# oscarknagg/voicemap

Measured on AMD Instinct MI355X. Metric: audio-sec/s embedded, 3s@16kHz siamese batch (training step), higher is better.
Workload: dtype f16; 1 GPU; siamese cfg-A train step (filters 128, embed 64, contrastive loss), 128 pairs/GPU of 3 s @ 16 kHz decimated x4 (L=12000), Adam(clipnorm 1), f16 storage; global_pairs=128, parallelism=dp1

## Files before the change

include/voicemap_hip.h:

```cpp
#ifndef VOICEMAP_HIP_H
#define VOICEMAP_HIP_H

#include <stdint.h>

#ifdef __cplusplus
extern "C" {
#endif

enum { VM_F32 = 0, VM_BF16 = 1, VM_F32S = 2, VM_F16 = 3 };
enum { VM_OK = 0, VM_ERR_ARG = -1, VM_ERR_LAUNCH = -2, VM_ERR_UNSUPPORTED = -3 };
enum { VM_LOSS_CONTRASTIVE = 0, VM_LOSS_BCE = 1 };
enum { VM_HEAD_UNIFORM_EUCLIDEAN = 0, VM_HEAD_WEIGHTED_L1 = 1 };
enum { VM_DIST_EUCLIDEAN = 0, VM_DIST_COSINE = 1, VM_DIST_DOT = 2 };
enum { VM_SCORE_WEIGHTED_L1 = 3, VM_SCORE_NEG_EUCLIDEAN = 4 };

const char* vm_last_error(void);
int vm_abi_version(void);
int vm_check_device(void);

int vm_fill_zero(void* ptr, int64_t bytes, void* stream);
int vm_event_create(void** event_out);
int vm_event_destroy(void* event);
int vm_event_record(void* event, void* stream);
int vm_stream_wait_event(void* stream, void* event);
// ... 19 lines not shown
                                    int noise_is_i16, const int64_t* noise_offsets, int K, const float* snr_lin, const float* gain,
                                    const float* rirs, int n_rirs, int R, const int32_t* rir_id, float* out, void* ws, void* stream);

int64_t vm_conv1_stat_rows(int64_t L);
int vm_conv1_fwd(const float* x, const float* w, const float* bias, int64_t n_windows, int64_t L, int F,
                 int dtype, void* z, float* stat_sum, float* stat_sq, void* stream);
int64_t vm_conv1_wgrad_workspace_bytes(int64_t n_windows, int F);
int vm_conv1_wgrad(const float* x, const void* du, int64_t n_windows, int64_t L, int F, int dtype,
                   float* ws, float* grad_w, void* stream);

int vm_conv1_fused_fwd(const float* x, const float* w, const float* bias, const float* gamma_or_scale, const float* shift,
                       int64_t n_windows, int64_t L, int F, int pool, int inference, int dtype, void* out, float* stat_sum,
                       float* stat_sq, void* stream);
int vm_conv1_fused_fwd_varlen(const float* x, const float* w, const float* bias, const float* scale, const float* shift,
                              const int32_t* lens, int64_t n_windows, int64_t L, int F, int pool, int dtype, void* out, void* stream);
int64_t vm_conv1_fused_bwd_workspace_bytes(int64_t n_windows, int64_t L, int F);
int vm_conv1_fused_bwd(const float* x, const float* w, const float* bias, const void* dp, const float* scale,
                       const float* mean, const float* invstd, const float* drop, const float* c1, const float* c2,
                       int64_t n_windows, int64_t windows_per_tower, int64_t L, int F, int pool, int dtype, void* ws,
                       float* grad_w, float* grad_b, void* stream);

int64_t vm_conv_stat_rows(int64_t L);
int vm_conv_fwd(const void* in, const void* wf, const float* bias, int64_t n_windows, int64_t L, int c_in,
                int c_out, int dtype, void* z, float* stat_sum, float* stat_sq, void* stream);
int64_t vm_conv_flat_stat_rows(int64_t n_windows, int64_t L);
int vm_conv_fwd_flat(const void* in, const void* wf, const float* bias, int64_t n_windows, int64_t L, int c_in, int c_out, int dtype,
                     void* z, float* stat_sum, float* stat_sq, void* stream);
int vm_conv_fwd_e_supported(int64_t n_windows, int64_t L, int c_in, int c_out, int dtype);
int vm_conv_fwd_e(const void* in, const void* wf, const float* bias, const float* gamma, int64_t n_windows, int64_t L,
                  int c_in, int c_out, int dtype, void* z, float* stat_sum, float* stat_sq, void* e, void* stream);
int vm_fold_bn_weights(const float* wt, const float* scale, const float* shift, const float* bias, int towers, int c_in, int c_out,
                       int dtype, void* wf_folded, void* wf_packed, float* hb, float* ctr_out, void* stream);
int vm_conv_fwd_fold_supported(int64_t n_windows, int64_t L, int c_in, int c_out, int dtype, int with_e);
int vm_conv_fwd_fold(const void* in_e, const void* wf_folded, const float* bias, const float* hb, const float* gamma,
                     int64_t n_windows, int64_t windows_per_tower, int64_t L, int c_in, int c_out, int dtype, void* z, float* stat_sum,
                     float* stat_sq, void* e, void* o, const void* wf_packed, const float* e_center, void* stream);
int vm_pack_nt_weights_supported(int n_rows, int a_c, int dtype);
int vm_pack_nt_weights(const void* bt, int towers, int n_rows, int a_c, int dtype, void* packed, void* stream);
int vm_pack_nt_weights_batch(int n, const void* const* bt, const int* towers, const int* n_rows, const int* a_c, int dtype,
                             void* const* packed, void* stream);
int vm_conv_fwd_pool_supported(int64_t n_windows, int64_t L, int c_in, int c_out, int dtype);
int vm_conv_fwd_pool(const void* in, const void* wf, const float* bias, const float* scale, const float* shift,
                     int64_t n_windows, int64_t L, int c_in, int c_out, int dtype, void* act, const void* wf_packed, void* stream);
int vm_conv_fwd_pool_varlen(const void* in, const void* wf, const float* bias, const float* scale, const float* shift,
                            const int32_t* lens, int64_t n_windows, int64_t L, int c_in, int c_out, int dtype, void* act,
                            const void* wf_packed, void* stream);
int vm_conv_dgrad(const void* du, const void* wd, int64_t n_windows, int64_t L, int c_in, int c_out, int dtype,
                  void* dx, void* stream);
int64_t vm_conv_dgrad_bnred_rows(int64_t L);
int vm_conv_dgrad_bnred_supported(int64_t n_windows, int64_t L, int c_in, int c_out, int dtype);
int vm_conv_dgrad_bnred(const void* du, const void* wd, int64_t n_windows, int64_t L, int c_in, int c_out, int dtype,
                        void* dx, const void* red_a, int red_a_padded, float* red_s0, float* red_s1, const void* wd_packed,
                        void* stream);
int vm_conv_wgrad_splits(int64_t n_windows, int64_t L, int c_in, int c_out);
int64_t vm_conv_wgrad_workspace_bytes(int64_t n_windows, int64_t L, int c_in, int c_out);
int vm_conv_wgrad(const void* in, const void* du, int64_t n_windows, int64_t L, int c_in, int c_out, int dtype,
                  void* ws, float* grad_w, void* stream);
int64_t vm_conv_wgrad_fold_workspace_bytes(int64_t n_windows, int64_t windows_per_tower, int64_t L, int c_in, int c_out);
int vm_conv_wgrad_fold(const void* in_e, const void* du, int64_t n_windows, int64_t windows_per_tower, int64_t L, int c_in, int c_out,
                       int dtype, const float* scale, const float* shift, const float* dsum, void* ws, float* grad_w, void* stream);
int vm_conv_wgrad_fold_finish(const void* ws, int64_t n_windows, int64_t windows_per_tower, int64_t L, int c_in, int c_out,
                              const float* scale, const float* shift, const float* dsum, float* grad_w, void* stream);
int vm_prep_conv_weights(const float* w, int c_in, int c_out, int dtype, void* wf, void* wd, void* stream);
int vm_prep_conv_weights_batch(int n_layers, const float* const* w, const int* c_in, const int* c_out, int dtype,
                               void* const* wf, void* const* wd, float* const* wt, void* stream);

// ... 69 lines not shown
int vm_bn_drop_pool_gmax_partials_e(const void* e, const float* scale, const float* shift, const float* drop, int64_t n_windows,
                                    int64_t windows_per_tower, int64_t Lq, int C, int dtype, float* part_v, int32_t* part_i,
                                    void* stream);
int vm_bn_bwd_gmax_finalize_e(const void* e, const float* dg, const int32_t* gidx, const float* scale, const float* shift,
                              const float* mean, const float* invstd, const float* drop, int64_t n_windows, int64_t windows_per_tower,
                              int64_t Lq, int C, int dtype, double count_per_tower, float* c1, float* c2, float* grad_gamma,
                              float* grad_beta, void* stream);
int vm_bn_pool_bwd_apply_pairs_gmax(const void* e, const void* o, const float* dg, const int32_t* gidx, const float* scale,
                                    const float* shift, const float* mean, const float* invstd, const float* drop, const float* c1,
                                    const float* c2, int64_t n_windows, int64_t windows_per_tower, int64_t L, int C, int dtype, void* du,
                                    float* part_du, void* stream);

int vm_global_maxpool_fwd(const void* act, int64_t n_windows, int64_t L, int C, int dtype, float* gmax,
                          int32_t* gidx, void* stream);
int vm_global_maxpool_fwd_varlen(const void* act, const int32_t* lens, int64_t n_windows, int64_t L, int C, int dtype, float* gmax,
                                 int32_t* gidx, void* ws, void* stream);
int vm_global_maxpool_bwd(const float* dg, const int32_t* gidx, int64_t n_windows, int64_t L, int C, int dtype,
                          void* dp, void* stream);
int vm_dense_fwd(const float* in, const float* w, const float* b, int64_t rows, int n_in, int n_out, float* out,
                 void* stream);
int vm_dense_bwd(const float* in, const float* w, const float* dout, int64_t rows, int n_in, int n_out,
                 float* grad_w, float* grad_b, float* din, void* stream);

int vm_siamese_head_loss(const float* emb, const float* head_w, const float* head_b, const float* y, int64_t pairs,
                         int E, int head_kind, int loss_kind, float grad_scale, float* pred, float* loss_acc, float* demb,
                         float* grad_hw, float* grad_hb, float* ws, void* stream);
int vm_siamese_head_reduce(const float* emb, const float* ws, int64_t pairs, int E, int head_kind, float* loss_acc, float* grad_hw,
                           float* grad_hb, void* stream);

int vm_tail_fwd_bwd_supported(int C, int E);
int vm_tail_fwd_bwd(const float* gmax_part_v, const int32_t* gmax_part_i, int seg_rows, float* gmax, int32_t* gidx, const float* dense_w, const float* dense_b,
                    const float* head_w, const float* head_b, const float* y, int64_t pairs, int C, int E, int head_kind,
                    int loss_kind, float grad_scale, float* emb, float* pred, float* demb, float* dgmax, float* ws, void* stream);
int vm_tail_param_grads(const float* gmax, const float* demb, const float* emb, const float* ws, int64_t pairs, int C, int E,
                        int head_kind, float* loss_acc, float* grad_dense_w, float* grad_dense_b, float* grad_hw, float* grad_hb,
                        void* stream);

int vm_softmax_cce(const float* logits, const int32_t* labels, int64_t rows, int n_classes, float grad_scale, float* prob,
                   float* loss_acc, float* dlogits, float* ws, void* stream);

int64_t vm_sqnorm_workspace_bytes(int64_t n);
int vm_grad_sqnorm(const float* g, int64_t n, void* ws, float* sqnorm, void* stream);
int vm_adam_clip_step(float* p, const float* g, float* m, float* v, int64_t n, float lr_t, float beta1, float beta2,
                      float eps, float clipnorm, float grad_prescale, float* sqnorm, const void* sqnorm_parts, int skip_nonfinite,
                      int32_t* skipped, void* stream);

int vm_nshot_distances(const float* query, const float* support, int64_t tasks, int k, int n, int E, int dist_kind,
                       float* pred, int32_t* argmin, void* stream);

int vm_nshot_indexed(const float* emb, int64_t n_rows, const int32_t* query_idx, const int32_t* support_idx, int64_t tasks, int k,
                     int n, int E, int dist_kind, float* pred, int32_t* argmin, void* stream);
int64_t vm_pairdist_workspace_bytes(int64_t M, int64_t N);
int vm_pairdist_argmin(const float* q, const float* ref, int64_t M, int64_t N, int E, int dist_kind, int64_t q_row0, float* dist,
                       float* best_val, int32_t* best_idx, void* ws, void* stream);
int64_t vm_pair_score_hist_workspace_bytes(int64_t N, int E);
int vm_pair_score_hist(const float* emb, const int32_t* label, int64_t N, int E, int score_kind, const float* weights, int64_t row_lo,
                       int64_t row_hi, const int64_t* host_windows, int n_windows, int bins, uint64_t* hist, void* ws, void* stream);
int64_t vm_cohort_stats_workspace_bytes(int64_t M, int64_t C, int E);
int vm_cohort_topk_stats(const float* q, int64_t M, const float* cohort, int64_t C, int E, int score_kind, const float* weights,
                         int64_t self_row0, int64_t K, float* mu, float* sigma, float* rsig, int32_t* count, int32_t* topk_idx, void* ws,
                         void* stream);
int vm_pair_score_hist_norm(const float* emb, const int32_t* label, int64_t N, int E, int score_kind, const float* weights, int64_t row_lo,
                            int64_t row_hi, const int64_t* host_windows, int n_windows, int bins, const float* mu, const float* rsig,
                            uint64_t* hist, void* ws, void* stream);
int64_t vm_speaker_sums_workspace_bytes(int64_t N, int E, int64_t S);
int vm_speaker_sums(const float* emb, const int32_t* label, int64_t N, int E, int64_t S, int kind, double* sums, double* msum, int32_t* count,
// ... 53 lines not shown
```

voicemap_amd/csrc/conv_common.hpp:

```cpp
#pragma once
#include <string.h>

#include <type_traits>

#include "common.hpp"

namespace vm {

constexpr int BM = 128, BN = 128;

template <int KB>
struct Geo {
    static constexpr int PITCH = KB + 16;
    static constexpr int TILE = BM * PITCH;
    static constexpr int CH = KB / 16;
    static constexpr int NCHUNK = BM * CH / 256;
};
constexpr int OUT_PITCH = BN * 4 + 16;

template <typename T> struct Mfma;
template <> struct Mfma<bf16> {
    static constexpr int KSTEP_BYTES = 32;
    using Frag = bf16x8;
    __device__ static inline Frag load(const char* row_ptr, int s, int kh) {
// ... 113 lines not shown
        acc[0][0] = M::run(b0h, a0h, acc[0][0]);
        acc[0][1] = M::run(b1h, a0h, acc[0][1]);
        acc[1][0] = M::run(b0h, a1h, acc[1][0]);
        acc[1][1] = M::run(b1h, a1h, acc[1][1]);
    }
}

__device__ inline void zero_acc(f32x16 (&acc)[2][2]) {
#pragma unroll
    for (int i = 0; i < 2; ++i)
#pragma unroll
        for (int j = 0; j < 2; ++j)
#pragma unroll
            for (int r = 0; r < 16; ++r) acc[i][j][r] = 0.f;
}

__device__ inline void acc_to_lds(char* out_tile, int wm, int wn, int lane, const f32x16 (&acc)[2][2]) {
    const int hi = lane >> 5;
#pragma unroll
    for (int im = 0; im < 2; ++im) {
        const int m = wm * 64 + im * 32 + (lane & 31);
#pragma unroll
        for (int in = 0; in < 2; ++in) {
#pragma unroll
            for (int g = 0; g < 4; ++g) {
                const int n = wn * 64 + in * 32 + 8 * g + 4 * hi;
                f32x4 v = {acc[im][in][4 * g], acc[im][in][4 * g + 1], acc[im][in][4 * g + 2], acc[im][in][4 * g + 3]};
                *reinterpret_cast<f32x4*>(out_tile + m * OUT_PITCH + n * 4) = v;
            }
        }
    }
}

enum { EPI_FWD = 0, EPI_DGRAD = 1, EPI_FWD_POOL = 2, EPI_FWD_FOLD = 3 };

template <typename T>
struct NtArgs {
    const T* a;
    const T* bt;
    const float* bias;
    T* out;
    float* stat_sum;
    float* stat_sq;
    int64_t a_win_stride;
    int a_c;
    int L, N, Ktot;
    int tilesL, tilesN;
    const T* red_a = nullptr;
    int64_t red_a_win_stride = 0;
    int red_a_row0 = 0;
    int split = 0;
    const float* aff_scale = nullptr;
    const float* aff_shift = nullptr;
    T* pool_e = nullptr;
    int pool_e_pad = 0;
    T* pool_o = nullptr;
    const float* fold_hb = nullptr;
    const float* fold_ctr = nullptr;
    int64_t tower_windows = 0, bt_tower_stride = 0;
    int flat_period = 0, flat_valid = 0;
    const T* bt_packed = nullptr;
    const int32_t* valid_len = nullptr;
};

template <int AUX = 0>
__device__ inline void glds16(const char* gsrc, char* lds_base) {
#if defined(__HIP_DEVICE_COMPILE__)
    __builtin_amdgcn_global_load_lds(gsrc, (__attribute__((address_space(3))) void*)lds_base, 16, 0, AUX);
#endif
}

template <int KB>
__device__ inline int swz(int row, int chunk) {
    return KB == 128 ? (chunk ^ ((row >> 1) & 7)) : (chunk ^ ((row >> 2) & 3));
}

template <int N>
__device__ inline void wait_vmcnt() {
    asm volatile("s_waitcnt vmcnt(%0)" ::"n"(N) : "memory");
}

}
```

voicemap_amd/csrc/conv_gemm.hip:

```cpp
#include "conv_common.hpp"

#ifndef VM_ABL
#define VM_ABL 0
#endif

namespace vm {

template <int KB>
constexpr int nt_lds_bytes() {
    return (2 * 2 * Geo<KB>::TILE > BM * OUT_PITCH + 4096) ? 2 * 2 * Geo<KB>::TILE : BM * OUT_PITCH + 4096;
}

template <typename T, int EPI, int KB, bool SPLIT = false>
__global__ __launch_bounds__(256) void conv_nt_kernel(NtArgs<T> p, int64_t n_groups) {
    static_assert(!SPLIT || (sizeof(T) == 4 && KB == 128), "split-bf16 arithmetic: fp32 storage, 128-byte slices");
    using G = Geo<KB>;
    constexpr int VEC = Elem<T>::kVec;
    constexpr int BK = KB / (int)sizeof(T);
    __shared__ __attribute__((aligned(16))) char lds[nt_lds_bytes<KB>()];

    const int tid = threadIdx.x, lane = tid & 63, w = tid >> 6, wm = w >> 1, wn = w & 1;
    const int nk = (p.Ktot + BK - 1) / BK;

    int lds_off[G::NCHUNK], kch[G::NCHUNK], srow[G::NCHUNK];
// ... 416 lines not shown
        for (int g = 0; g < 4; ++g)
#pragma unroll
            for (int i = 0; i < 4; ++i)
#pragma unroll
                for (int e = 0; e < 4; ++e) acc[i][j][4 * g + e] = b4[j][g][e];
}
#if defined(VM_EXPERIMENT_PROFILE_EPI)
extern __device__ unsigned int g_prof[];
__device__ inline void vm_epi_mark(int k) {
    const long long t = __builtin_amdgcn_s_memtime();
    if ((threadIdx.x & 63) == 0 && blockIdx.x < 8192) g_prof[((int64_t)blockIdx.x * 4 + (threadIdx.x >> 6)) * 8 + k] = (unsigned int)t;
}
#if VM_EXPERIMENT_PROFILE_EPI + 0 == 2
#define VM_EPI_MARK(k)
#define VM_RED_MARK(k) vm_epi_mark(k)
#else
#define VM_EPI_MARK(k) vm_epi_mark(k)
#define VM_RED_MARK(k)
#endif
#else
#define VM_EPI_MARK(k)
#define VM_RED_MARK(k)
#endif
struct N2DrainSync {
    __device__ inline void sync() { __syncthreads(); }
    __device__ inline void point() {}
};

template <typename T, int EPI>
__device__ inline void n2_tile_write(const NtArgs<T>& p, char* lds, const f32x16 (&acc)[4][2], int t0, int n0, int trows, int lane, int wm, int wn,
                                     const f32x4 (&negc)[2][4]) {
    using namespace n2;
    const int r = lane & 31, kh = lane >> 5;
    constexpr bool FWD = EPI == EPI_FWD || EPI == EPI_FWD_FOLD;
    const bool red = EPI == EPI_DGRAD && p.red_a != nullptr;
    const int valid = (p.L - t0) < trows ? (p.L - t0) : trows;
    constexpr bool CAN_CENTRE = EPI == EPI_FWD_FOLD && std::is_same<T, f16>::value;
    const bool ctrd = CAN_CENTRE && p.fold_ctr != nullptr;
    auto body = [&](auto ctrd_c) {
        constexpr bool CTRD = decltype(ctrd_c)::value;
        uint32_t nc16[2][4][2];
        if constexpr (CTRD) {
            typedef _Float16 h2 __attribute__((ext_vector_type(2)));
#pragma unroll
            for (int j = 0; j < 2; ++j)
#pragma unroll
                for (int g = 0; g < 4; ++g) {
                    nc16[j][g][0] = __builtin_bit_cast(uint32_t, h2{(_Float16)negc[j][g][0], (_Float16)negc[j][g][1]});
                    nc16[j][g][1] = __builtin_bit_cast(uint32_t, h2{(_Float16)negc[j][g][2], (_Float16)negc[j][g][3]});
                }
        }
#pragma unroll
        for (int i = 0; i < 4; ++i) {
#pragma unroll
            for (int j = 0; j < 2; ++j) {
                const int mb = wm * 128 + i * 32;
                const int m = mb + r;
                const bool partial = mb + 32 > valid;
                const bool zero = (FWD || red) && partial && m >= valid;
#pragma unroll
                for (int g = 0; g < 4; ++g) {
                    const int nl = wn * 64 + j * 32 + 8 * g + 4 * kh;
                    T o[4];
#pragma unroll
                    for (int e = 0; e < 4; ++e) o[e] = Elem<T>::from_f(acc[i][j][4 * g + e]);
                    u32x2 pk = *reinterpret_cast<const u32x2*>(o);
                    if constexpr (CTRD) {
                        uint32_t lo = pk[0], hi = pk[1];
                        asm("v_pk_max_f16 %0, %1, %2" : "=v"(lo) : "v"(lo), "v"(nc16[j][g][0]));
                        asm("v_pk_max_f16 %0, %1, %2" : "=v"(hi) : "v"(hi), "v"(nc16[j][g][1]));
                        pk[0] = lo;
                        pk[1] = hi;
                    } else if constexpr (EPI != EPI_DGRAD) {
                        uint32_t lo = pk[0], hi = pk[1];
                        asm("v_pk_max_i16 %0, %1, 0" : "=v"(lo) : "v"(lo));
                        asm("v_pk_max_i16 %0, %1, 0" : "=v"(hi) : "v"(hi));
                        pk[0] = lo;
                        pk[1] = hi;
                    }
                    pk[0] = zero ? 0u : pk[0];
                    pk[1] = zero ? 0u : pk[1];
                    *reinterpret_cast<u32x2*>(lds + m * TP + nl * 2) = pk;
                }
            }
        }
    };
    if constexpr (CAN_CENTRE) {
        if (ctrd) body(std::true_type{});
        else body(std::false_type{});
    } else {
        body(std::false_type{});
    }
}

template <typename T, int EPI, typename BarT>
__device__ inline void n2_tile_drain(const NtArgs<T>& p, char* lds, int64_t n, int tl, int t0, int n0, int trows, int tid, int lane, int w,
                                     BarT& bar) {
    using namespace n2;
    using V8 = typename Mfma<T>::Frag;
    const int kh = lane >> 5;
    constexpr bool FWD = EPI == EPI_FWD || EPI == EPI_FWD_FOLD;
    const bool stats = FWD && p.stat_sum != nullptr && !(VM_ABL & 8);
    const bool red = EPI == EPI_DGRAD && p.red_a != nullptr;
    const int valid = (p.L - t0) < trows ? (p.L - t0) : trows;
    const int c8 = tid & 15, rg = tid >> 4;
    if (EPI == EPI_FWD_POOL) {
        float sc[8], sh[8];
        {
            const f32x4 s0 = *reinterpret_cast<const f32x4*>(p.aff_scale + n0 + c8 * 8), s1 = *reinterpret_cast<const f32x4*>(p.aff_scale + n0 + c8 * 8 + 4);
            const f32x4 h0 = *reinterpret_cast<const f32x4*>(p.aff_shift + n0 + c8 * 8), h1 = *reinterpret_cast<const f32x4*>(p.aff_shift + n0 + c8 * 8 + 4);
#pragma unroll
            for (int e = 0; e < 4; ++e) {
                sc[e] = s0[e];
                sc[4 + e] = s1[e];
                sh[e] = h0[e];
                sh[4 + e] = h1[e];
            }
        }
        const int vq = valid >> 1;
        int dq = vq;
        if (p.valid_len != nullptr) {
            const int d = (p.valid_len[n] >> 1) - (t0 >> 1);
            dq = d < vq ? d : vq;
        }
        T* pbase = p.out + (n * (int64_t)(p.L / 2 + 2) + 1 + (t0 >> 1)) * (int64_t)p.N + n0 + c8 * 8;
        V8 r0[8], r1[8];
#pragma unroll
        for (int jj = 0; jj < 8; ++jj) {
            const int q = rg + 16 * jj;
            r0[jj] = *reinterpret_cast<const V8*>(lds + (2 * q) * TP + c8 * 16);
            r1[jj] = *reinterpret_cast<const V8*>(lds + (2 * q + 1) * TP + c8 * 16);
        }
#pragma unroll
        for (int jj = 0; jj < 8; ++jj) {
// ... 18 lines not shown
    auto half = [&](int h, auto interior_c) {
        constexpr bool INTERIOR = decltype(interior_c)::value;
        u32x4 v[8];
#pragma unroll
        for (int jj = 0; jj < 8; ++jj) v[jj] = *reinterpret_cast<const u32x4*>(lds + (h * 128 + rg + 16 * jj) * TP + c8 * 16);
#pragma unroll
        for (int jj = 0; jj < 8; ++jj) {
            const int row = h * 128 + rg + 16 * jj;
            const bool ok = INTERIOR ? (h == 0 || jj < 7 || row < trows) : row < valid;
            if (ok && !((VM_ABL & 4) && row > 0)) *reinterpret_cast<u32x4*>(obase + (int64_t)row * p.N) = v[jj];
        }
    };
    if (FWD && p.pool_o != nullptr) {
    } else if (interior) {
        half(0, std::true_type{});
        bar.point();
        half(1, std::true_type{});
        bar.point();
    } else {
        half(0, std::false_type{});
        bar.point();
        half(1, std::false_type{});
        bar.point();
    }
    if (FWD && p.pool_e != nullptr) {
        u32x4 neg;
        {
            const f32x4 g0 = *reinterpret_cast<const f32x4*>(p.aff_scale + n0 + c8 * 8), g1 = *reinterpret_cast<const f32x4*>(p.aff_scale + n0 + c8 * 8 + 4);
            neg[0] = (g0[0] < 0.f ? 0xFFFFu : 0u) | (g0[1] < 0.f ? 0xFFFF0000u : 0u);
            neg[1] = (g0[2] < 0.f ? 0xFFFFu : 0u) | (g0[3] < 0.f ? 0xFFFF0000u : 0u);
            neg[2] = (g1[0] < 0.f ? 0xFFFFu : 0u) | (g1[1] < 0.f ? 0xFFFF0000u : 0u);
            neg[3] = (g1[2] < 0.f ? 0xFFFFu : 0u) | (g1[3] < 0.f ? 0xFFFF0000u : 0u);
        }
        constexpr bool CAN_CENTRE = EPI == EPI_FWD_FOLD && std::is_same<T, f16>::value;
        const bool ctrd = CAN_CENTRE && p.fold_ctr != nullptr;
        u32x4 c16 = {0u, 0u, 0u, 0u};
        if (CAN_CENTRE && ctrd) {
            const f32x4 q0 = *reinterpret_cast<const f32x4*>(p.fold_ctr + n0 + c8 * 8), q1 = *reinterpret_cast<const f32x4*>(p.fold_ctr + n0 + c8 * 8 + 4);
            typedef _Float16 h2 __attribute__((ext_vector_type(2)));
            c16[0] = __builtin_bit_cast(uint32_t, h2{(_Float16)q0[0], (_Float16)q0[1]});
            c16[1] = __builtin_bit_cast(uint32_t, h2{(_Float16)q0[2], (_Float16)q0[3]});
            c16[2] = __builtin_bit_cast(uint32_t, h2{(_Float16)q1[0], (_Float16)q1[1]});
            c16[3] = __builtin_bit_cast(uint32_t, h2{(_Float16)q1[2], (_Float16)q1[3]});
        }
        const int vq = valid >> 1;
        T* ebase = p.pool_e + (n * (int64_t)(p.L / 2 + 2 * p.pool_e_pad) + p.pool_e_pad + (t0 >> 1)) * (int64_t)p.N + n0 + c8 * 8;
        T* obase2 = p.pool_o + (n * (int64_t)(p.L / 2) + (t0 >> 1)) * (int64_t)p.N + n0 + c8 * 8;
        u32x4 r0[8], r1[8];
#pragma unroll
        for (int jj = 0; jj < 8; ++jj) {
            const int q = rg + 16 * jj;
            r0[jj] = *reinterpret_cast<const u32x4*>(lds + (2 * q) * TP + c8 * 16);
            r1[jj] = *reinterpret_cast<const u32x4*>(lds + (2 * q + 1) * TP + c8 * 16);
        }
        auto pairs = [&](auto ctrd_c, auto other_c) {
            constexpr bool CTRD = decltype(ctrd_c)::value, OTHER = decltype(other_c)::value;
#pragma unroll
            for (int jj = 0; jj < 8; ++jj) {
                const int q = rg + 16 * jj;
                u32x4 o, oth;
#pragma unroll
                for (int d = 0; d < 4; ++d) {
                    uint32_t a = r0[jj][d], b = r1[jj][d];
                    const uint32_t m = neg[d];
                    if constexpr (CTRD) {
                        uint32_t mx, mn;
                        asm("v_pk_max_f16 %0, %1, %2" : "=v"(mx) : "v"(a), "v"(b));
// ... 7 lines not shown
                    if constexpr (!CTRD || OTHER) {
                        const uint32_t fl = m & 0x7FFF7FFFu;
                        const uint32_t af = a ^ fl, bf = b ^ fl;
                        uint32_t mx, mn;
                        asm("v_pk_max_i16 %0, %1, %2" : "=v"(mx) : "v"(af), "v"(bf));
                        if constexpr (!CTRD) o[d] = mx ^ fl;
                        if constexpr (OTHER) {
                            uint32_t df;
                            asm("v_pk_min_i16 %0, %1, %2" : "=v"(mn) : "v"(af), "v"(bf));
                            asm("v_pk_sub_i16 %0, %1, %2" : "=v"(df) : "v"(af), "v"(bf));
                            oth[d] = (mn ^ fl) | (df & 0x80008000u);
                        }
                    }
                }
                if (q < vq) {
                    *reinterpret_cast<u32x4*>(ebase + (int64_t)q * p.N) = o;
                    if constexpr (OTHER) *reinterpret_cast<u32x4*>(obase2 + (int64_t)q * p.N) = oth;
                }
                bar.point();
            }
        };
        const bool other = p.pool_o != nullptr;
        if constexpr (CAN_CENTRE) {
            if (ctrd && other) pairs(std::true_type{}, std::true_type{});
            else if (ctrd) pairs(std::true_type{}, std::false_type{});
            else if (other) pairs(std::false_type{}, std::true_type{});
            else pairs(std::false_type{}, std::false_type{});
        } else {
            if (other) pairs(std::false_type{}, std::true_type{});
            else pairs(std::false_type{}, std::false_type{});
        }
    }
    VM_EPI_MARK(5);
    if (stats) {
#if defined(__HIP_DEVICE_COMPILE__)
        const uint32_t lds0 = (uint32_t)(uintptr_t)(__attribute__((address_space(3))) const char*)lds;
#else
        const uint32_t lds0 = 0;
#endif
        const int li = lane & 15, lg = (lane >> 4) & 1;
        const uint32_t xoff = lds0 + (4 * (li >> 2) + 2 * kh) * TP + (32 * w + 16 * lg + 4 * (li & 3)) * 2;
        const u32x2 ones = ones4<T>();
        const int srows = (p.L + 127) / 128;
        const int cn = lane & 31;
#pragma unroll
        for (int h = 0; h < 2; ++h) {
            f32x4 d1a = {0.f, 0.f, 0.f, 0.f}, d1b = d1a, d2a = d1a, d2b = d1a;
            u32x2 lo[8], hi[8];
#pragma unroll
            for (int rs = 0; rs < 8; ++rs) {
                const uint32_t a = xoff + (h * 128 + rs * 16) * TP;
                asm volatile("ds_read_b64_tr_b16 %0, %1" : "=v"(lo[rs]) : "v"(a));
                asm volatile("ds_read_b64_tr_b16 %0, %1 offset:272" : "=v"(hi[rs]) : "v"(a));
            }
#pragma unroll
            for (int rs = 0; rs < 8; ++rs) {
                if (rs == 0) {
                    asm volatile("s_waitcnt lgkmcnt(14)" : "+v"(lo[0]), "+v"(hi[0]));
                } else if (rs == 1) {
                    asm volatile("s_waitcnt lgkmcnt(12)" : "+v"(lo[1]), "+v"(hi[1]));
                } else if (rs == 2) {
                    asm volatile("s_waitcnt lgkmcnt(10)" : "+v"(lo[2]), "+v"(hi[2]));
                } else if (rs == 3) {
                    asm volatile("s_waitcnt lgkmcnt(8)" : "+v"(lo[3]), "+v"(hi[3]));
                } else if (rs == 4) {
                    asm volatile("s_waitcnt lgkmcnt(6)" : "+v"(lo[4]), "+v"(hi[4]));
                } else if (rs == 5) {
                    asm volatile("s_waitcnt lgkmcnt(4)" : "+v"(lo[5]), "+v"(hi[5]));
                } else if (rs == 6) {
                    asm volatile("s_waitcnt lgkmcnt(2)" : "+v"(lo[6]), "+v"(hi[6]));
                } else {
                    asm volatile("s_waitcnt lgkmcnt(0)" : "+v"(lo[7]), "+v"(hi[7]));
                }
                d2a = Mfma4<T>::run(lo[rs], lo[rs], d2a);
                d2b = Mfma4<T>::run(hi[rs], hi[rs], d2b);
                d1a = Mfma4<T>::run(ones, lo[rs], d1a);
                d1b = Mfma4<T>::run(ones, hi[rs], d1b);
                __builtin_amdgcn_sched_barrier(0);
            }
            float ds = d1a[0] + d1b[0], dq = 0.f;
#pragma unroll
            for (int e = 0; e < 4; ++e) dq = e == (lane & 3) ? d2a[e] + d2b[e] : dq;
            ds += __shfl_xor(ds, 32, 64);
            dq += __shfl_xor(dq, 32, 64);
            if (2 * tl + h < srows && kh == 0) {
                const int64_t srow = n * srows + 2 * tl + h;
                p.stat_sum[srow * p.N + n0 + 32 * w + cn] = ds;
                p.stat_sq[srow * p.N + n0 + 32 * w + cn] = dq;
            }
            bar.point();
        }
    }
    VM_EPI_MARK(6);
    VM_RED_MARK(1);
    if (red) {
#if defined(__HIP_DEVICE_COMPILE__)
        const uint32_t lds0 = (uint32_t)(uintptr_t)(__attribute__((address_space(3))) const char*)lds;
#else
        const uint32_t lds0 = 0;
#endif
        const int li = lane & 15, lg = (lane >> 4) & 1;
        const uint32_t xoff = lds0 + (4 * (li >> 2) + 2 * kh) * TP + (32 * w + 16 * lg + 4 * (li & 3)) * 2;
        const u32x2 ones = ones4<T>();
        u32x2 dlo[16], dhi[16];
        f32x4 d1[2][2], d2[2][2];
#pragma unroll
        for (int h = 0; h < 2; ++h)
#pragma unroll
            for (int u = 0; u < 2; ++u) d1[h][u] = d2[h][u] = f32x4{0.f, 0.f, 0.f, 0.f};
#pragma unroll
        for (int q = 0; q < 16; ++q) {
            const uint32_t a = xoff + (q * 16) * TP;
            asm volatile("ds_read_b64_tr_b16 %0, %1" : "=v"(dlo[q]) : "v"(a));
            asm volatile("ds_read_b64_tr_b16 %0, %1 offset:272" : "=v"(dhi[q]) : "v"(a));
            if (q == 7) asm volatile("s_waitcnt lgkmcnt(0)" : "+v"(dlo[0]), "+v"(dhi[0]), "+v"(dlo[1]), "+v"(dhi[1]), "+v"(dlo[2]), "+v"(dhi[2]),
                                     "+v"(dlo[3]), "+v"(dhi[3]), "+v"(dlo[4]), "+v"(dhi[4]), "+v"(dlo[5]), "+v"(dhi[5]), "+v"(dlo[6]), "+v"(dhi[6]),
                                     "+v"(dlo[7]), "+v"(dhi[7]));
        }
        asm volatile("s_waitcnt lgkmcnt(0)" : "+v"(dlo[8]), "+v"(dhi[8]), "+v"(dlo[9]), "+v"(dhi[9]), "+v"(dlo[10]), "+v"(dhi[10]), "+v"(dlo[11]),
                     "+v"(dhi[11]), "+v"(dlo[12]), "+v"(dhi[12]), "+v"(dlo[13]), "+v"(dhi[13]), "+v"(dlo[14]), "+v"(dhi[14]), "+v"(dlo[15]),
                     "+v"(dhi[15]));
        VM_RED_MARK(2);
        bar.sync();
// ... 33 lines not shown
            }
            asm volatile("s_waitcnt lgkmcnt(0)" : "+v"(alo[0]), "+v"(ahi[0]), "+v"(alo[1]), "+v"(ahi[1]), "+v"(alo[2]), "+v"(ahi[2]), "+v"(alo[3]),
                         "+v"(ahi[3]), "+v"(alo[4]), "+v"(ahi[4]), "+v"(alo[5]), "+v"(ahi[5]), "+v"(alo[6]), "+v"(ahi[6]), "+v"(alo[7]), "+v"(ahi[7]));
#pragma unroll
            for (int rs = 0; rs < 8; ++rs) {
                const int q = h * 8 + rs;
                d2[h][0] = Mfma4<T>::run(dlo[q], alo[rs], d2[h][0]);
                d2[h][1] = Mfma4<T>::run(dhi[q], ahi[rs], d2[h][1]);
            }
        }
        const int cn = lane & 31;
        const int rows2 = 2 * p.tilesL;
#pragma unroll
        for (int h = 0; h < 2; ++h) {
            float ds = d1[h][0][0] + d1[h][1][0], dq = 0.f;
#pragma unroll
            for (int e = 0; e < 4; ++e) dq = e == (lane & 3) ? d2[h][0][e] + d2[h][1][e] : dq;
            ds += __shfl_xor(ds, 32, 64);
            dq += __shfl_xor(dq, 32, 64);
            const int64_t srow = n * rows2 + 2 * tl + h;
            if (kh == 0) {
                p.stat_sum[srow * p.N + n0 + 32 * w + cn] = ds;
                p.stat_sq[srow * p.N + n0 + 32 * w + cn] = dq;
            }
        }
    }
}


template <typename T, int EPI>
__device__ inline void n2_epilogue(const NtArgs<T>& p, char* lds, const f32x16 (&acc)[4][2], int64_t n, int tl, int t0, int n0, int trows,
                                   int tid, int lane, int w, int wm, int wn) {
    f32x4 negc[2][4];
    if constexpr (EPI == EPI_FWD_FOLD && std::is_same<T, f16>::value) {
        if (p.fold_ctr != nullptr) {
#pragma unroll
            for (int j = 0; j < 2; ++j)
#pragma unroll
                for (int g = 0; g < 4; ++g) {
                    const f32x4 c = *reinterpret_cast<const f32x4*>(p.fold_ctr + n0 + (wn * 64 + j * 32) + 8 * g + 4 * (lane >> 5));
                    negc[j][g] = f32x4{-c[0], -c[1], -c[2], -c[3]};
                }
        }
    }
    VM_EPI_MARK(1);
    __syncthreads();
    VM_EPI_MARK(2);
    n2_tile_write<T, EPI>(p, lds, acc, t0, n0, trows, lane, wm, wn, negc);
    VM_EPI_MARK(3);
    __syncthreads();
    VM_EPI_MARK(4);
    N2DrainSync bar;
    n2_tile_drain<T, EPI>(p, lds, n, tl, t0, n0, trows, tid, lane, w, bar);
}

namespace n2r {
constexpr int TROWS = 254;
constexpr int A_BLK = 256 * 64, B_STG = 128 * 64;
constexpr int B0 = 3 * A_BLK;
constexpr int OPER = 3 * A_BLK + 3 * B_STG;
static_assert(OPER <= n2::LDS_BYTES, "operand rings fit under the epilogue tile");
}

__device__ inline void wait_vm_0246(int n) {
    if (n >= 6) {
        asm volatile("s_waitcnt vmcnt(6)" ::: "memory");
    } else if (n == 4) {
// ... 31 lines not shown
    }
}

template <typename T, int EPI>
__global__ __launch_bounds__(256, 2) void conv_nt2r_kernel(NtArgs<T> p, int64_t n_groups) {
    VM_PROF(const long long pt_start = __builtin_amdgcn_s_memtime(); long long pt_first = 0, pt_bar = 0;)
    using namespace n2;
    using namespace n2r;
    using V8 = typename Mfma<T>::Frag;
    __shared__ __attribute__((aligned(1024))) char lds[LDS_BYTES];
    const int tid = threadIdx.x, lane = tid & 63;
    const int w = __builtin_amdgcn_readfirstlane(tid >> 6), wm = w >> 1, wn = w & 1;
    const int chunks = p.a_c / 32, nk = chunks * 3;
    const int row_bytes = p.a_c * 2;

    unsigned group;
    int tn;
    {
        const unsigned v = blockIdx.x, tiles_n = (unsigned)p.tilesN;
        if ((n_groups & 7) == 0) {
            const unsigned j = v >> 3, q = j / tiles_n;
            tn = (int)(j - q * tiles_n);
            group = q * 8 + (v & 7);
        } else {
            group = v / tiles_n;
            tn = (int)(v - group * tiles_n);
        }
    }
    const unsigned nw = group / (unsigned)p.tilesL;
    const int tl = (int)(group - nw * (unsigned)p.tilesL);
    const int64_t n = nw;
    const int t0 = tl * TROWS, n0 = tn * TN;
    if (n2_pool_dead_tile<T, EPI>(p, n, t0, n0, tid)) return;
    if constexpr (EPI == EPI_FWD_FOLD) {
        const unsigned tw = nw / (unsigned)p.tower_windows;
        p.bt += tw * p.bt_tower_stride;
        p.fold_hb += tw * 4 * p.N;
        if (p.fold_ctr != nullptr) p.fold_ctr += tw * p.N;
    }
    f32x4 bias4[2][4];
    if constexpr (EPI == EPI_FWD_FOLD) p.bias = p.fold_hb + 3 * p.N;
    n2_load_bias<T, EPI>(p, bias4, n0 + wn * 64 + 4 * (lane >> 5));

    const int lrow = lane >> 2, lchunk = lane & 3;
    const char* a_src[4];
    const char* b_src[2];
#pragma unroll
    for (int i = 0; i < 4; ++i) {
        const int row = (w + 4 * i) * 16 + lrow;
        int pr = t0 + row;
        pr = pr < p.L + 2 ? pr : p.L + 1;
        a_src[i] = reinterpret_cast<const char*>(p.a + n * p.a_win_stride + (int64_t)pr * p.a_c) + ((lchunk ^ ((row >> 2) & 3)) << 4);
    }
#pragma unroll
    for (int i = 0; i < 2; ++i) {
        const int row = (w + 4 * i) * 16 + lrow;
        b_src[i] = reinterpret_cast<const char*>(p.bt + (int64_t)(n0 + row) * p.Ktot) + ((lchunk ^ ((row >> 2) & 3)) << 4);
    }
    auto issue_a = [&](int blk, int chunk, int i0) {
        char* base = lds + blk * A_BLK;
#pragma unroll
        for (int i = 0; i < 2; ++i) glds16(a_src[i0 + i] + chunk * KB, base + __builtin_amdgcn_readfirstlane((w + 4 * (i0 + i)) * 1024));
    };
    auto issue_b = [&](int stg, int ko) {
        char* base = lds + B0 + stg * B_STG;
#pragma unroll
        for (int i = 0; i < 2; ++i) glds16(b_src[i] + ko, base + __builtin_amdgcn_readfirstlane((w + 4 * i) * 1024));
    };

    const int r = lane & 31, kh = lane >> 5;
    int a_addr[3][2], b_addr[2];
#pragma unroll
    for (int tap = 0; tap < 3; ++tap) {
        const int row = wm * 128 + r + tap;
// ... 82 lines not shown
            VM_MM(a0[1], b0[1], 1, 1);
            __builtin_amdgcn_sched_barrier(0);
            asm volatile("s_waitcnt lgkmcnt(7)" : "+v"(a0[2]));
            VM_MM(a0[2], b0[0], 2, 0);
            VM_MM(a0[2], b0[1], 2, 1);
            __builtin_amdgcn_sched_barrier(0);
            asm volatile("s_waitcnt lgkmcnt(6)" : "+v"(a0[3]));
            VM_MM(a0[3], b0[0], 3, 0);
            VM_MM(a0[3], b0[1], 3, 1);
            __builtin_amdgcn_sched_barrier(0);
            asm volatile("s_waitcnt lgkmcnt(3)" : "+v"(b1[0]), "+v"(b1[1]), "+v"(a1[0]));
            VM_MM(a1[0], b1[0], 0, 0);
            VM_MM(a1[0], b1[1], 0, 1);
            __builtin_amdgcn_sched_barrier(0);
            asm volatile("s_waitcnt lgkmcnt(2)" : "+v"(a1[1]));
            VM_MM(a1[1], b1[0], 1, 0);
            VM_MM(a1[1], b1[1], 1, 1);
            __builtin_amdgcn_sched_barrier(0);
            asm volatile("s_waitcnt lgkmcnt(1)" : "+v"(a1[2]));
            VM_MM(a1[2], b1[0], 2, 0);
            VM_MM(a1[2], b1[1], 2, 1);
            __builtin_amdgcn_sched_barrier(0);
            asm volatile("s_waitcnt lgkmcnt(0)" : "+v"(a1[3]));
            VM_MM(a1[3], b1[0], 3, 0);
            VM_MM(a1[3], b1[1], 3, 1);
            __builtin_amdgcn_sched_barrier(0);
#undef VM_MM
            __builtin_amdgcn_sched_barrier(0);
            VM_PROF(if (kt == 0) pt_first = __builtin_amdgcn_s_memtime();)
        }
        a_blk = a_blk == 2 ? 0 : a_blk + 1;
    }
    VM_PROF(const long long pt_loop = __builtin_amdgcn_s_memtime();)
    if constexpr (EPI == EPI_FWD_FOLD) {
        const int c0 = n0 + wn * 64 + 4 * (lane >> 5), rl = p.L - 1 - t0;
        if (t0 == 0) n2_fold_edge<T>(p, acc, 0, 0, wm, lane & 31, c0);
        if (rl >= 0 && rl < TROWS) n2_fold_edge<T>(p, acc, rl, 1, wm, lane & 31, c0);
    }
    n2_epilogue<T, EPI>(p, lds, acc, n, tl, t0, n0, TROWS, tid, lane, w, wm, wn);
#if defined(VM_EXPERIMENT_PROFILE)
    {
        asm volatile("s_waitcnt vmcnt(0)" ::: "memory");
        const long long pt_end = __builtin_amdgcn_s_memtime();
        if (lane == 0 && blockIdx.x < 8192) {
            unsigned int* q = g_prof + ((int64_t)blockIdx.x * 4 + w) * 8;
            q[0] = (unsigned int)(pt_end - pt_start);
            q[1] = (unsigned int)(pt_first - pt_start);
            q[2] = (unsigned int)(pt_loop - pt_first);
            q[3] = (unsigned int)(pt_end - pt_loop);
            q[4] = (unsigned int)(pt_s2 - pt_start);
            q[5] = (unsigned int)(pt_s3 - pt_s2);
            q[6] = (unsigned int)(pt_bar - pt_s3);
            q[7] = (unsigned int)(pt_first - pt_bar);
        }
    }
#endif
}


#ifndef VM_NT3_ABL
#define VM_NT3_ABL 0
#endif
namespace n3 {
constexpr int NBLK = 4;
constexpr int A_BLK = 256 * 64;
static_assert(NBLK * A_BLK <= n2::LDS_BYTES, "the input ring fits under the epilogue tile");
constexpr int KT_BYTES = 4096;
// ... 47 lines not shown
              n3_nwait(5, 8, false) == 8, "conv_nt3_kernel wait schedule");
static_assert(n3_nwait(0, 4, true) == 8 && n3_nwait(1, 4, true) == 12 && n3_nwait(2, 4, true) == 12 && n3_nwait(3, 4, true) == 8 &&
              n3_nwait(4, 8, true) == 6 && n3_nwait(11, 4, true) == 0, "conv_nt3_kernel wait schedule (lean prologue)");

template <typename T, int EPI, int CHUNKS, bool LEAN>
__global__ __launch_bounds__(256, 2) void conv_nt3_kernel(NtArgs<T> p, int64_t n_groups) {
    VM_PROF(const long long pt_start = __builtin_amdgcn_s_memtime(); long long pt_first = 0, pt_bar = 0;)
    using namespace n2;
    using V8 = typename Mfma<T>::Frag;
    constexpr int A_BLK = n3::A_BLK, NK = 3 * CHUNKS;
    __shared__ __attribute__((aligned(1024))) char lds[LDS_BYTES];
    const int tid = threadIdx.x, lane = tid & 63;
    const int w = __builtin_amdgcn_readfirstlane(tid >> 6), wm = w >> 1, wn = w & 1;

    unsigned group;
    int tn;
    {
        const unsigned v = blockIdx.x, tiles_n = (unsigned)p.tilesN;
        if ((n_groups & 7) == 0) {
            const unsigned j = v >> 3, q = j / tiles_n;
            tn = (int)(j - q * tiles_n);
            group = q * 8 + (v & 7);
        } else {
            group = v / tiles_n;
            tn = (int)(v - group * tiles_n);
        }
    }
    const unsigned nw = group / (unsigned)p.tilesL;
    const int tl = (int)(group - nw * (unsigned)p.tilesL);
    const int64_t n = nw;
    const int t0 = tl * n2r::TROWS, n0 = tn * TN;
    if (n2_pool_dead_tile<T, EPI>(p, n, t0, n0, tid)) return;
    unsigned tw = 0;
    if constexpr (EPI == EPI_FWD_FOLD) {
        tw = nw / (unsigned)p.tower_windows;
        p.fold_hb += tw * 4 * p.N;
        if (p.fold_ctr != nullptr) p.fold_ctr += tw * p.N;
    }
    if constexpr (EPI == EPI_FWD_FOLD) p.bias = p.fold_hb + 3 * p.N;
    f32x4 bias_lo[2][4], bias_hi[2][4];
    if constexpr (EPI != EPI_DGRAD) {
        const float* bp = p.bias + n0 + wn * 64;
#pragma unroll
        for (int j = 0; j < 2; ++j)
#pragma unroll
            for (int g = 0; g < 4; ++g) {
                bias_lo[j][g] = *reinterpret_cast<const f32x4*>(bp + 32 * j + 8 * g);
                bias_hi[j][g] = *reinterpret_cast<const f32x4*>(bp + 32 * j + 8 * g + 4);
            }
    }

    const int lrow = lane >> 2, lchunk = lane & 3;
    const char* a_src[4];
#pragma unroll
    for (int i = 0; i < 4; ++i) {
        const int row = (w + 4 * i) * 16 + lrow;
        int pr = t0 + row;
        pr = pr < p.L + 2 ? pr : p.L + 1;
        a_src[i] = reinterpret_cast<const char*>(p.a + n * p.a_win_stride + (int64_t)pr * p.a_c) + ((lchunk ^ ((row >> 2) & 3)) << 4);
    }
    auto issue_a = [&](int blk, int chunk, int i0) {
        char* base = lds + blk * A_BLK;
#pragma unroll
        for (int i = 0; i < 2; ++i) glds16(a_src[i0 + i] + chunk * KB, base + __builtin_amdgcn_readfirstlane((w + 4 * (i0 + i)) * 1024));
    };
    auto issue_a1 = [&](int blk, int chunk, int i) {
        glds16(a_src[i] + chunk * KB, lds + blk * A_BLK + __builtin_amdgcn_readfirstlane((w + 4 * i) * 1024));
    };
    uint64_t bbase;
    {
        const uint64_t q = (uint64_t)(uintptr_t)p.bt_packed +
                           ((uint64_t)tw * (unsigned)(p.N >> 6) + (unsigned)((n0 >> 6) + wn)) * (uint64_t)(NK * n3::KT_BYTES);
// ... 97 lines not shown
        constexpr int kt_ = (KT), c_ = kt_ / 3, tap_ = kt_ - 3 * c_, cur_ = kt_ % 3, nxt_ = (kt_ + 2) % 3, ablk_ = c_ % 4;             \
        constexpr int nc_ = (kt_ + 1) / 3, ntap_ = (kt_ + 1) - 3 * nc_;                             \
        n3_wait_b<n3_nwait(kt_, CHUNKS, LEAN)>(bs[cur_]);                                                                             \
        if constexpr (kt_ == 0) {                                                                                                     \
            __builtin_amdgcn_s_barrier();                                                                                             \
            VM_PROF(pt_bar = __builtin_amdgcn_s_memtime();)                                                                           \
            const uint32_t a00_ = lds0 + a_addr[0][0];                                                                                \
            VM_FRAG_READ(f0[0], a00_, 0) VM_FRAG_READ(f0[1], a00_, 1) VM_FRAG_READ(f0[2], a00_, 2) VM_FRAG_READ(f0[3], a00_, 3)         \
        }                                                                                                                             \
        const uint32_t aa1_ = lds0 + ablk_ * A_BLK + a_addr[tap_][1];                                                                  \
        const uint32_t an0_ = lds0 + (nc_ % 4) * A_BLK + a_addr[ntap_][0];                                                             \
        const uint64_t sb_ = bbase + (uint64_t)((kt_ + 2) * n3::KT_BYTES);                                                            \
        __builtin_amdgcn_sched_barrier(0);                                                                                            \
        VM_P_STEP0(0) VM_P_STEP0(1) VM_P_STEP0(2) VM_P_STEP0(3)                                                                       \
        if constexpr (tap_ == 2 && kt_ + 1 < NK) {                                                                                    \
            asm volatile("s_waitcnt lgkmcnt(0)" : "+v"(f1[0]), "+v"(f1[1]), "+v"(f1[2]), "+v"(f1[3]));                                 \
            __builtin_amdgcn_s_barrier();                                                                                             \
            __builtin_amdgcn_sched_barrier(0);                                                                                        \
        }                                                                                                                             \
        VM_P_STEP1(0) VM_P_STEP1(1) VM_P_STEP1(2) VM_P_STEP1(3)                                                                       \
        VM_PROF(if (kt_ == 0) pt_first = __builtin_amdgcn_s_memtime();)                                                               \
    }
#define VM_CHUNK(C) VM_KTILE_P(3 * (C)) VM_KTILE_P(3 * (C) + 1) VM_KTILE_P(3 * (C) + 2)
    VM_CHUNK(0) VM_CHUNK(1) VM_CHUNK(2) VM_CHUNK(3) VM_CHUNK(4) VM_CHUNK(5) VM_CHUNK(6) VM_CHUNK(7)
    VM_CHUNK(8) VM_CHUNK(9) VM_CHUNK(10) VM_CHUNK(11) VM_CHUNK(12) VM_CHUNK(13) VM_CHUNK(14) VM_CHUNK(15)
    static_assert(CHUNKS <= 16, "conv_nt3_kernel: at most 16 channel chunks are written out");
#undef VM_CHUNK
#undef VM_KTILE_P
#undef VM_P_STEP0
#undef VM_P_STEP1
#undef VM_FRAG_READ
#undef VM_MM
#undef VM_LOAD_SET
    if constexpr (EPI == EPI_FWD_FOLD) {
        const int c0 = n0 + wn * 64 + 4 * (lane >> 5), rl = p.L - 1 - t0;
        if (t0 == 0) n2_fold_edge<T>(p, acc, 0, 0, wm, lane & 31, c0);
        if (rl >= 0 && rl < n2r::TROWS) n2_fold_edge<T>(p, acc, rl, 1, wm, lane & 31, c0);
    }
    VM_PROF(const long long pt_loop = __builtin_amdgcn_s_memtime();)
#if VM_NT3_ABL & 8
    if (acc[0][0][0] == 123.456f && acc[3][1][15] == 1.5f) n2_epilogue<T, EPI>(p, lds, acc, n, tl, t0, n0, n2r::TROWS, tid, lane, w, wm, wn);
#else
    n2_epilogue<T, EPI>(p, lds, acc, n, tl, t0, n0, n2r::TROWS, tid, lane, w, wm, wn);
#endif
#if defined(VM_EXPERIMENT_PROFILE)
    {
        asm volatile("s_waitcnt vmcnt(0)" ::: "memory");
        const long long pt_end = __builtin_amdgcn_s_memtime();
#if defined(VM_EXPERIMENT_PROFILE_HW)
        if (lane == 0 && blockIdx.x < 8192) {
            unsigned int* q = g_prof + ((int64_t)blockIdx.x * 4 + w) * 8;
            q[0] = (unsigned int)pt_start;
            q[1] = (unsigned int)pt_end;
            q[2] = __builtin_amdgcn_s_getreg((31 << 11) | 4);
            q[3] = __builtin_amdgcn_s_getreg((31 << 11) | 20);
            q[4] = (unsigned int)pt_bar;
            q[5] = (unsigned int)pt_loop;
            q[6] = (unsigned int)(pt_start >> 32);
            q[7] = (unsigned int)pt_s3;
        }
        (void)pt_first; (void)pt_s2;
#elif defined(VM_EXPERIMENT_PROFILE_EPI)
        if (lane == 0 && blockIdx.x < 8192) {
            unsigned int* q = g_prof + ((int64_t)blockIdx.x * 4 + w) * 8;
            q[0] = (unsigned int)pt_start;
            q[7] = (unsigned int)pt_end;
        }
// ... 87 lines not shown
}

static bool nt3_chunks(int a_c) { return a_c == 128 || a_c == 256 || a_c == 384 || a_c == 512; }

template <typename T, int EPI>
static void launch_n2r(const NtArgs<T>& a, int64_t n_windows, hipStream_t stream) {
    if constexpr (sizeof(T) == 2) {
        NtArgs<T> b = a;
        b.tilesN = a.N / n2::TN;
        b.tilesL = (a.L + n2r::TROWS - 1) / n2r::TROWS;
        const int64_t n_groups = n_windows * b.tilesL;
        if constexpr (EPI != EPI_FWD) {
            if (b.bt_packed != nullptr && (g_nt3 & (EPI == EPI_DGRAD ? 2 : 1)) && nt3_chunks(a.a_c)) {
                const dim3 grid((unsigned)(n_groups * b.tilesN));
#define VM_NT3(CH, PIPE) hipLaunchKernelGGL((conv_nt3_kernel<T, EPI, CH, PIPE>), grid, dim3(256), 0, stream, b, n_groups)
                const bool pipe = (g_nt3_lean & (EPI == EPI_DGRAD ? 2 : 1)) != 0;
                switch (a.a_c / 32) {
                    case 4: if (pipe) VM_NT3(4, true); else VM_NT3(4, false); break;
                    case 8: if (pipe) VM_NT3(8, true); else VM_NT3(8, false); break;
                    case 12: if (pipe) VM_NT3(12, true); else VM_NT3(12, false); break;
                    default: if (pipe) VM_NT3(16, true); else VM_NT3(16, false); break;
                }
#undef VM_NT3
                return;
            }
        }
        hipLaunchKernelGGL((conv_nt2r_kernel<T, EPI>), dim3((unsigned)(n_groups * b.tilesN)), dim3(256), 0, stream, b, n_groups);
    }
}

template <typename T, int EPI>
static void launch_nt(const NtArgs<T>& a, int64_t n_windows, hipStream_t stream) {
    if constexpr (sizeof(T) == 2) {
        if (!a.flat_period && (g_nt_n2 & (EPI == EPI_DGRAD ? 2 : 1)) && a.Ktot == 3 * a.a_c && n2r_shape(n_windows, a.L, a.a_c, a.N, EPI == EPI_FWD || EPI == EPI_FWD_FOLD)) {
            launch_n2r<T, EPI>(a, n_windows, stream);
            return;
        }
    }
    const int64_t n_groups = n_windows * a.tilesL;
    const int64_t grid = n_groups < g_nt_blocks ? n_groups : g_nt_blocks;
    const int64_t kbytes = (int64_t)a.Ktot * (int64_t)sizeof(T);
    if constexpr (sizeof(T) == 4) {
        if (a.split) {
            hipLaunchKernelGGL((conv_nt_kernel<T, EPI, 128, true>), dim3((unsigned)grid), dim3(256), 0, stream, a, n_groups);
            return;
        }
    }
    if (g_nt_glds && kbytes % 128 == 0) {
        hipLaunchKernelGGL((conv_nt_glds_kernel<T, EPI, 128>), dim3((unsigned)grid), dim3(256), 0, stream, a, n_groups);
    } else if (g_nt_glds && kbytes % 64 == 0) {
        hipLaunchKernelGGL((conv_nt_glds_kernel<T, EPI, 64>), dim3((unsigned)grid), dim3(256), 0, stream, a, n_groups);
    } else {
        hipLaunchKernelGGL((conv_nt_kernel<T, EPI, 128>), dim3((unsigned)grid), dim3(256), 0, stream, a, n_groups);
    }
}

template <typename T>
static NtArgs<T> fwd_args(const void* in, const void* wf, const float* bias, void* out, float* stat_sum, float* stat_sq, int64_t L,
                          int c_in, int c_out, int dtype) {
    NtArgs<T> a;
    a.a = (const T*)in;
    a.bt = (const T*)wf;
    a.bias = bias;
    a.out = (T*)out;
    a.stat_sum = stat_sum;
    a.stat_sq = stat_sq;
    a.a_win_stride = (L + 2) * (int64_t)c_in;
// ... 102 lines not shown
extern "C" int vm_conv_fwd_fold(const void* in_e, const void* wf_folded, const float* bias, const float* hb, const float* gamma,
                                int64_t n_windows, int64_t windows_per_tower, int64_t L, int c_in, int c_out, int dtype, void* z,
                                float* stat_sum, float* stat_sq, void* e, void* o, const void* wf_packed, const float* e_center,
                                void* stream) {
    VM_REQUIRE(in_e && wf_folded && bias && hb && stat_sum && stat_sq, "vm_conv_fwd_fold: null pointer");
    VM_REQUIRE(e_center == nullptr || (dtype == VM_F16 && e != nullptr && o != nullptr),
               "vm_conv_fwd_fold: a centred tile (e_center) needs VM_F16 storage and the (e, o) pair output");
    VM_REQUIRE(e == nullptr || gamma != nullptr, "vm_conv_fwd_fold: the pool extreme needs gamma (its sign picks max / min)");
    VM_REQUIRE(o == nullptr || e != nullptr, "vm_conv_fwd_fold: o (the other element of each pair) goes with e");
    VM_REQUIRE(z != nullptr || o != nullptr, "vm_conv_fwd_fold: z may only be NULL when (e, o) carry the output");
    VM_REQUIRE(n_windows > 0 && L > 0 && windows_per_tower > 0 && n_windows % windows_per_tower == 0,
               "vm_conv_fwd_fold: n_windows must be a positive multiple of windows_per_tower");
    VM_REQUIRE((L + 2) * (int64_t)c_in < (1LL << 31) && 3LL * c_in * c_out < (1LL << 31), "vm_conv_fwd_fold: window too large");
    if (!vm_conv_fwd_fold_supported(n_windows, L, c_in, c_out, dtype, e != nullptr)) {
        set_error("vm_conv_fwd_fold: shape/dtype/tuning not served by the 256 x 128 input-resident kernel (ask vm_conv_fwd_fold_supported)");
        return VM_ERR_UNSUPPORTED;
    }
    VM_DISPATCH_16(dtype, {
        NtArgs<T> a = fwd_args<T>(in_e, wf_folded, bias, z, stat_sum, stat_sq, L, c_in, c_out, dtype);
        a.fold_hb = hb;
        a.tower_windows = windows_per_tower;
        a.bt_tower_stride = 3LL * c_in * c_out;
        a.aff_scale = gamma;
        a.pool_e = (T*)e;
        a.pool_o = (T*)o;
        a.pool_e_pad = 1;
        a.bt_packed = (const T*)wf_packed;
        a.fold_ctr = e_center;
        launch_n2r<T, EPI_FWD_FOLD>(a, n_windows, (hipStream_t)stream);
    });
    return check_launch("vm_conv_fwd_fold");
}

extern "C" int vm_conv_fwd_pool_supported(int64_t n_windows, int64_t L, int c_in, int c_out, int dtype) {
    return (is16(dtype) && (g_nt_n2 & 1) && L >= 2 && !(L & 1) && n2r_shape(n_windows, L, c_in, c_out, false)) ? 1 : 0;
}

extern "C" int vm_conv_fwd_pool(const void* in, const void* wf, const float* bias, const float* scale, const float* shift,
                                int64_t n_windows, int64_t L, int c_in, int c_out, int dtype, void* act, const void* wf_packed,
                                void* stream) {
    VM_REQUIRE(in && wf && bias && scale && shift && act, "vm_conv_fwd_pool: null pointer");
    VM_REQUIRE(n_windows > 0 && L > 0, "vm_conv_fwd_pool: bad sizes");
    VM_REQUIRE((L + 2) * (int64_t)c_in < (1LL << 31) && 3LL * c_in * c_out < (1LL << 31), "vm_conv_fwd_pool: window too large");
    if (!vm_conv_fwd_pool_supported(n_windows, L, c_in, c_out, dtype)) {
        set_error("vm_conv_fwd_pool: shape/dtype/tuning not served by the 256 x 128 input-resident kernel (ask vm_conv_fwd_pool_supported)");
        return VM_ERR_UNSUPPORTED;
    }
    VM_DISPATCH_16(dtype, {
        NtArgs<T> a = fwd_args<T>(in, wf, bias, act, nullptr, nullptr, L, c_in, c_out, dtype);
        a.aff_scale = scale;
        a.aff_shift = shift;
        a.bt_packed = (const T*)wf_packed;
        launch_n2r<T, EPI_FWD_POOL>(a, n_windows, (hipStream_t)stream);
    });
    return check_launch("vm_conv_fwd_pool");
}

extern "C" int vm_conv_fwd_pool_varlen(const void* in, const void* wf, const float* bias, const float* scale, const float* shift,
                                       const int32_t* lens, int64_t n_windows, int64_t L, int c_in, int c_out, int dtype, void* act,
                                       const void* wf_packed, void* stream) {
    VM_REQUIRE(in && wf && bias && scale && shift && lens && act, "vm_conv_fwd_pool_varlen: null pointer");
    VM_REQUIRE(n_windows > 0 && L > 0, "vm_conv_fwd_pool_varlen: bad sizes");
    VM_REQUIRE((L + 2) * (int64_t)c_in < (1LL << 31) && 3LL * c_in * c_out < (1LL << 31), "vm_conv_fwd_pool_varlen: window too large");
    if (!vm_conv_fwd_pool_supported(n_windows, L, c_in, c_out, dtype)) {
        set_error("vm_conv_fwd_pool_varlen: shape/dtype/tuning not served by the 256 x 128 input-resident kernel (ask vm_conv_fwd_pool_supported)");
        return VM_ERR_UNSUPPORTED;
// ... 161 lines not shown
```

voicemap_amd/csrc/program_run.hip:

```cpp
#include <cstdint>
#include <cstring>

extern "C" {
int vm_abi_version(void);
int vm_adam_clip_step(const void*, const void*, const void*, const void*, int64_t, float, float, float, float, float, float, const void*, const void*, int, const void*, const void*);
int vm_bn_bwd_finalize(const void*, const void*, int64_t, int64_t, int, double, const void*, const void*, const void*, const void*, const void*, const void*);
int vm_bn_bwd_from_sums(const void*, const void*, int64_t, const void*, const void*, const void*, const void*, const void*, const void*, const void*, int64_t, int64_t, int64_t, int, int, int, int, const void*, const void*, const void*);
int vm_bn_bwd_from_sums_finalize(const void*, const void*, int64_t, const void*, const void*, const void*, const void*, const void*, const void*, const void*, int64_t, int64_t, int64_t, int, int, int, int, double, const void*, const void*, const void*, const void*, const void*, const void*);
int vm_bn_bwd_gmax_finalize(const void*, const void*, const void*, const void*, const void*, const void*, const void*, const void*, int64_t, int64_t, int64_t, int, int, int, double, const void*, const void*, const void*, const void*, const void*);
int vm_bn_bwd_gmax_finalize_e(const void*, const void*, const void*, const void*, const void*, const void*, const void*, const void*, int64_t, int64_t, int64_t, int, int, double, const void*, const void*, const void*, const void*, const void*);
int vm_bn_drop_pool_fwd(const void*, const void*, const void*, const void*, int64_t, int64_t, int64_t, int, int, int, const void*, const void*);
int vm_bn_drop_pool_fwd_varlen(const void*, const void*, const void*, const void*, int64_t, int64_t, int, int, int, const void*, const void*);
int vm_bn_drop_pool_gmax_fwd(const void*, const void*, const void*, const void*, int64_t, int64_t, int64_t, int, int, int, const void*, const void*, const void*, const void*);
int vm_bn_drop_pool_gmax_fwd_varlen(const void*, const void*, const void*, const void*, int64_t, int64_t, int, int, int, const void*, const void*, const void*, const void*);
int vm_bn_drop_pool_gmax_partials(const void*, const void*, const void*, const void*, int64_t, int64_t, int64_t, int, int, int, const void*, const void*, const void*);
int vm_bn_drop_pool_gmax_partials_e(const void*, const void*, const void*, const void*, int64_t, int64_t, int64_t, int, int, const void*, const void*, const void*);
int vm_bn_finalize(const void*, const void*, int64_t, int, int, double, const void*, const void*, float, float, int, const void*, const void*, const void*, const void*, const void*, const void*, const void*, const void*, float, const void*, const void*, const void*, const void*, const void*);
int vm_bn_infer_affine(const void*, const void*, const void*, const void*, float, int, const void*, const void*, const void*);
int vm_bn_part_rows(void);
int vm_bn_part_rows_used(int64_t, int, int, int);
int vm_bn_pool2d_stack_fwd(const void*, const void*, const void*, const void*, int64_t, int, int64_t, int64_t, int, int, int, const void*, const void*, const void*);
int vm_bn_pool2d_stack_fwd_split(const void*, const void*, const void*, const void*, const void*, int64_t, int, int64_t, int64_t, int, int, int, const void*, const void*, const void*);
int vm_bn_pool_bwd_apply(const void*, const void*, const void*, const void*, const void*, const void*, const void*, const void*, const void*, int64_t, int64_t, int64_t, int, int, int, const void*, const void*, const void*);
int vm_bn_pool_bwd_apply_gmax(const void*, const void*, const void*, const void*, const void*, const void*, const void*, const void*, const void*, const void*, int64_t, int64_t, int64_t, int, int, int, const void*, const void*, const void*);
int vm_bn_pool_bwd_apply_pairs(const void*, const void*, const void*, const void*, const void*, const void*, const void*, const void*, const void*, const void*, int64_t, int64_t, int64_t, int, int, const void*, const void*, const void*, const void*);
int vm_bn_pool_bwd_apply_pairs_gmax(const void*, const void*, const void*, const void*, const void*, const void*, const void*, const void*, const void*, const void*, const void*, int64_t, int64_t, int64_t, int, int, const void*, const void*, const void*);
int vm_bn_pool_bwd_reduce(const void*, const void*, const void*, const void*, const void*, const void*, const void*, int64_t, int64_t, int64_t, int, int, int, const void*, const void*, const void*);
int vm_bn_pool_bwd_reduce_gmax(const void*, const void*, const void*, const void*, const void*, const void*, const void*, const void*, int64_t, int64_t, int64_t, int, int, int, const void*, const void*, const void*);
int vm_bn_pool_bwd_reduce_pooled(const void*, const void*, const void*, const void*, const void*, const void*, const void*, const void*, int64_t, int64_t, int64_t, int, int, int, const void*, const void*, const void*);
int vm_check_device(void);
int vm_clip_max_bwd(const void*, const void*, int64_t, int, int, const void*, const void*);
int vm_clip_max_fwd(const void*, int64_t, int, int, int, const void*, const void*, const void*);
int vm_cohort_topk_stats(const void*, int64_t, const void*, int64_t, int, int, const void*, int64_t, int64_t, const void*, const void*, const void*, const void*, const void*, const void*, const void*);
int vm_colsum(const void*, int64_t, int, const void*, const void*, const void*);
int vm_colsum_strided(const void*, int64_t, int, int, const void*, const void*, const void*);
int vm_conv1_fused_bwd(const void*, const void*, const void*, const void*, const void*, const void*, const void*, const void*, const void*, const void*, int64_t, int64_t, int64_t, int, int, int, const void*, const void*, const void*, const void*);
int vm_conv1_fused_fwd(const void*, const void*, const void*, const void*, const void*, int64_t, int64_t, int, int, int, int, const void*, const void*, const void*, const void*);
int vm_conv1_fused_fwd_varlen(const void*, const void*, const void*, const void*, const void*, const void*, int64_t, int64_t, int, int, int, const void*, const void*);
int vm_conv1_fwd(const void*, const void*, const void*, int64_t, int64_t, int, int, const void*, const void*, const void*, const void*);
int vm_conv1_wgrad(const void*, const void*, int64_t, int64_t, int, int, const void*, const void*, const void*);
int vm_conv2d_first_bn_pool_stack(const void*, const void*, const void*, const void*, const void*, const void*, const void*, int64_t, int, int64_t, int64_t, int, int, int, int, const void*, const void*, const void*);
int vm_conv2d_first_fwd(const void*, const void*, const void*, int64_t, int, int64_t, int, int, int, const void*, const void*, const void*, const void*);
int vm_conv2d_first_fwd_split(const void*, const void*, const void*, const void*, int64_t, int, int64_t, int, int, int, const void*, const void*, const void*, const void*, const void*);
int vm_conv2d_first_supported(int, int);
int vm_conv2d_first_wgrad(const void*, const void*, int64_t, int, int64_t, int, int, int, const void*, const void*, const void*);
int vm_conv_dgrad(const void*, const void*, int64_t, int64_t, int, int, int, const void*, const void*);
int vm_conv_dgrad_bnred(const void*, const void*, int64_t, int64_t, int, int, int, const void*, const void*, int, const void*, const void*, const void*, const void*);
int vm_conv_dgrad_bnred_supported(int64_t, int64_t, int, int, int);
int vm_conv_fwd(const void*, const void*, const void*, int64_t, int64_t, int, int, int, const void*, const void*, const void*, const void*);
int vm_conv_fwd_e(const void*, const void*, const void*, const void*, int64_t, int64_t, int, int, int, const void*, const void*, const void*, const void*, const void*);
int vm_conv_fwd_e_supported(int64_t, int64_t, int, int, int);
int vm_conv_fwd_flat(const void*, const void*, const void*, int64_t, int64_t, int, int, int, const void*, const void*, const void*, const void*);
int vm_conv_fwd_fold(const void*, const void*, const void*, const void*, const void*, int64_t, int64_t, int64_t, int, int, int, const void*, const void*, const void*, const void*, const void*, const void*, const void*, const void*);
int vm_conv_fwd_fold_supported(int64_t, int64_t, int, int, int, int);
int vm_conv_fwd_pool(const void*, const void*, const void*, const void*, const void*, int64_t, int64_t, int, int, int, const void*, const void*, const void*);
int vm_conv_fwd_pool_supported(int64_t, int64_t, int, int, int);
int vm_conv_fwd_pool_varlen(const void*, const void*, const void*, const void*, const void*, const void*, int64_t, int64_t, int, int, int, const void*, const void*, const void*);
int vm_conv_wgrad(const void*, const void*, int64_t, int64_t, int, int, int, const void*, const void*, const void*);
int vm_conv_wgrad_fold(const void*, const void*, int64_t, int64_t, int64_t, int, int, int, const void*, const void*, const void*, const void*, const void*, const void*);
int vm_conv_wgrad_fold_finish(const void*, int64_t, int64_t, int64_t, int, int, const void*, const void*, const void*, const void*, const void*);
int vm_conv_wgrad_splits(int64_t, int64_t, int, int);
int vm_crop_augment_decimate_whiten(const void*, int, const void*, int64_t, int64_t, int, int, float, int64_t, const void*, int, const void*, int, const void*, const void*, const void*, int, int, const void*, const void*, const void*, const void*);
int vm_crop_decimate_whiten(const void*, int, const void*, int64_t, int64_t, int, int, float, int64_t, const void*, const void*, const void*);
int vm_crop_decimate_whiten_varlen(const void*, int, const void*, const void*, int64_t, int64_t, int, int, float, const void*, const void*, const void*);
int vm_decimate_whiten(const void*, int, int64_t, int64_t, int, int, float, int64_t, const void*, const void*, const void*);
int vm_dense_bwd(const void*, const void*, const void*, int64_t, int, int, const void*, const void*, const void*, const void*);
int vm_dense_fwd(const void*, const void*, const void*, int64_t, int, int, const void*, const void*);
int vm_du_tower_sums(const void*, const void*, int64_t, int64_t, int64_t, int, int, const void*, const void*, const void*, const void*);
int vm_event_destroy(const void*);
int vm_event_record(const void*, const void*);
int vm_fill_zero(const void*, int64_t, const void*);
int vm_fold_bn_weights(const void*, const void*, const void*, const void*, int, int, int, int, const void*, const void*, const void*, const void*, const void*);
int vm_fold_pool_windows_bwd(const void*, const void*, int64_t, int, int64_t, int, int, int, int, const void*, const void*, const void*, const void*);
int vm_fold_windows(const void*, int64_t, int, int64_t, int, int, int, int, const void*, const void*);
int vm_global_maxpool_bwd(const void*, const void*, int64_t, int64_t, int, int, const void*, const void*);
int vm_global_maxpool_fwd(const void*, int64_t, int64_t, int, int, const void*, const void*, const void*);
int vm_global_maxpool_fwd_varlen(const void*, const void*, int64_t, int64_t, int, int, const void*, const void*, const void*, const void*);
int vm_grad_sqnorm(const void*, int64_t, const void*, const void*, const void*);
int vm_mfma_rate_probe(int, int, const void*, const void*);
int vm_mine_pairs(const void*, const void*, int64_t, int, int, int64_t, int64_t, int, int, const void*, const void*, const void*, const void*, const void*, const void*, const void*);
int vm_nshot_distances(const void*, const void*, int64_t, int, int, int, int, const void*, const void*, const void*);
int vm_nshot_indexed(const void*, int64_t, const void*, const void*, int64_t, int, int, int, int, const void*, const void*, const void*);
int vm_pack_nt_weights(const void*, int, int, int, int, const void*, const void*);
int vm_pack_nt_weights_batch(int, const void*, const void*, const void*, const void*, int, const void*, const void*);
int vm_pack_nt_weights_supported(int, int, int);
int vm_pair_score_hist(const void*, const void*, int64_t, int, int, const void*, int64_t, int64_t, const void*, int, int, const void*, const void*, const void*);
int vm_pair_score_hist_norm(const void*, const void*, int64_t, int, int, const void*, int64_t, int64_t, const void*, int, int, const void*, const void*, const void*, const void*, const void*);
int vm_pairdist_argmin(const void*, const void*, int64_t, int64_t, int, int, int64_t, const void*, const void*, const void*, const void*, const void*);
int vm_pool_windows_bwd(const void*, const void*, int64_t, int, int64_t, int, int, const void*, const void*);
int vm_pool_windows_fwd(const void*, int64_t, int, int64_t, int, int, const void*, const void*);
int vm_prep_conv_weights(const void*, int, int, int, const void*, const void*, const void*);
int vm_prep_conv_weights_batch(int, const void*, const void*, const void*, int, const void*, const void*, const void*, const void*);
int vm_siamese_head_loss(const void*, const void*, const void*, const void*, int64_t, int, int, int, float, const void*, const void*, const void*, const void*, const void*, const void*, const void*);
int vm_siamese_head_reduce(const void*, const void*, int64_t, int, int, const void*, const void*, const void*, const void*);
int vm_softmax_cce(const void*, const void*, int64_t, int, float, const void*, const void*, const void*, const void*, const void*);
int vm_speaker_identify(const void*, const void*, int64_t, int, const void*, const void*, const void*, int64_t, int, int, const void*, const void*, const void*, const void*, const void*, const void*, const void*);
int vm_speaker_sums(const void*, const void*, int64_t, int, int64_t, int, const void*, const void*, const void*, const void*, const void*);
int vm_speaker_trial_hist(const void*, const void*, int64_t, int, const void*, const void*, const void*, int64_t, int, int, const void*, int, int, const void*, const void*, const void*);
int vm_stack_windows(const void*, int64_t, int, int64_t, int, int, int, const void*, const void*);
int vm_stft_logmel(const void*, int, int64_t, int64_t, int, int, const void*, const void*, int, float, int, const void*, const void*);
int vm_stft_logmel_f16s(const void*, int, int64_t, int64_t, int, int, const void*, const void*, int, float, int, const void*, const void*);
int vm_stft_logmel_f16s_split(const void*, int, int64_t, int64_t, int, int, const void*, const void*, int, float, int, const void*, const void*, const void*);
int vm_stft_split_basis(const void*, int, const void*, const void*);
int vm_stream_wait_event(const void*, const void*);
int vm_tail_fwd_bwd(const void*, const void*, int, const void*, const void*, const void*, const void*, const void*, const void*, const void*, int64_t, int, int, int, int, float, const void*, const void*, const void*, const void*, const void*, const void*);
int vm_tail_fwd_bwd_supported(int, int);
int vm_tail_param_grads(const void*, const void*, const void*, const void*, int64_t, int, int, int, const void*, const void*, const void*, const void*, const void*, const void*);
}

static inline float w2f(int64_t w) {
    const uint32_t u = (uint32_t)w;
    float f;
    memcpy(&f, &u, 4);
    return f;
}
static inline double w2d(int64_t w) {
    double d;
    memcpy(&d, &w, 8);
    return d;
}

extern "C" int64_t vm_program_table_hash(void) { return 1570090092LL; }

extern "C" int vm_program_run(const int64_t* w, int64_t n_words, int64_t* fail_at) {
    int64_t i = 0;
    while (i + 1 < n_words) {
        const int64_t id = w[i], argc = w[i + 1];
        const int64_t* a = w + i + 2;
        int rc = -1;
        if (argc >= 0 && i + 2 + argc <= n_words) {
            switch (id) {
                case 0: if (argc == 0) rc = vm_abi_version(); break;
                case 1: if (argc == 16) rc = vm_adam_clip_step((const void*)a[0], (const void*)a[1], (const void*)a[2], (const void*)a[3], a[4], w2f(a[5]), w2f(a[6]), w2f(a[7]), w2f(a[8]), w2f(a[9]), w2f(a[10]), (const void*)a[11], (const void*)a[12], (int)a[13], (const void*)a[14], (const void*)a[15]); break;
                case 2: if (argc == 12) rc = vm_bn_bwd_finalize((const void*)a[0], (const void*)a[1], a[2], a[3], (int)a[4], w2d(a[5]), (const void*)a[6], (const void*)a[7], (const void*)a[8], (const void*)a[9], (const void*)a[10], (const void*)a[11]); break;
                case 3: if (argc == 20) rc = vm_bn_bwd_from_sums((const void*)a[0], (const void*)a[1], a[2], (const void*)a[3], (const void*)a[4], (const void*)a[5], (const void*)a[6], (const void*)a[7], (const void*)a[8], (const void*)a[9], a[10], a[11], a[12], (int)a[13], (int)a[14], (int)a[15], (int)a[16], (const void*)a[17], (const void*)a[18], (const void*)a[19]); break;
                case 4: if (argc == 24) rc = vm_bn_bwd_from_sums_finalize((const void*)a[0], (const void*)a[1], a[2], (const void*)a[3], (const void*)a[4], (const void*)a[5], (const void*)a[6], (const void*)a[7], (const void*)a[8], (const void*)a[9], a[10], a[11], a[12], (int)a[13], (int)a[14], (int)a[15], (int)a[16], w2d(a[17]), (const void*)a[18], (const void*)a[19], (const void*)a[20], (const void*)a[21], (const void*)a[22], (const void*)a[23]); break;
                case 5: if (argc == 20) rc = vm_bn_bwd_gmax_finalize((const void*)a[0], (const void*)a[1], (const void*)a[2], (const void*)a[3], (const void*)a[4], (const void*)a[5], (const void*)a[6], (const void*)a[7], a[8], a[9], a[10], (int)a[11], (int)a[12], (int)a[13], w2d(a[14]), (const void*)a[15], (const void*)a[16], (const void*)a[17], (const void*)a[18], (const void*)a[19]); break;
                case 6: if (argc == 19) rc = vm_bn_bwd_gmax_finalize_e((const void*)a[0], (const void*)a[1], (const void*)a[2], (const void*)a[3], (const void*)a[4], (const void*)a[5], (const void*)a[6], (const void*)a[7], a[8], a[9], a[10], (int)a[11], (int)a[12], w2d(a[13]), (const void*)a[14], (const void*)a[15], (const void*)a[16], (const void*)a[17], (const void*)a[18]); break;
                case 7: if (argc == 12) rc = vm_bn_drop_pool_fwd((const void*)a[0], (const void*)a[1], (const void*)a[2], (const void*)a[3], a[4], a[5], a[6], (int)a[7], (int)a[8], (int)a[9], (const void*)a[10], (const void*)a[11]); break;
                case 8: if (argc == 11) rc = vm_bn_drop_pool_fwd_varlen((const void*)a[0], (const void*)a[1], (const void*)a[2], (const void*)a[3], a[4], a[5], (int)a[6], (int)a[7], (int)a[8], (const void*)a[9], (const void*)a[10]); break;
                case 9: if (argc == 14) rc = vm_bn_drop_pool_gmax_fwd((const void*)a[0], (const void*)a[1], (const void*)a[2], (const void*)a[3], a[4], a[5], a[6], (int)a[7], (int)a[8], (int)a[9], (const void*)a[10], (const void*)a[11], (const void*)a[12], (const void*)a[13]); break;
                case 10: if (argc == 13) rc = vm_bn_drop_pool_gmax_fwd_varlen((const void*)a[0], (const void*)a[1], (const void*)a[2], (const void*)a[3], a[4], a[5], (int)a[6], (int)a[7], (int)a[8], (const void*)a[9], (const void*)a[10], (const void*)a[11], (const void*)a[12]); break;
                case 11: if (argc == 13) rc = vm_bn_drop_pool_gmax_partials((const void*)a[0], (const void*)a[1], (const void*)a[2], (const void*)a[3], a[4], a[5], a[6], (int)a[7], (int)a[8], (int)a[9], (const void*)a[10], (const void*)a[11], (const void*)a[12]); break;
                case 12: if (argc == 12) rc = vm_bn_drop_pool_gmax_partials_e((const void*)a[0], (const void*)a[1], (const void*)a[2], (const void*)a[3], a[4], a[5], a[6], (int)a[7], (int)a[8], (const void*)a[9], (const void*)a[10], (const void*)a[11]); break;
                case 13: if (argc == 25) rc = vm_bn_finalize((const void*)a[0], (const void*)a[1], a[2], (int)a[3], (int)a[4], w2d(a[5]), (const void*)a[6], (const void*)a[7], w2f(a[8]), w2f(a[9]), (int)a[10], (const void*)a[11], (const void*)a[12], (const void*)a[13], (const void*)a[14], (const void*)a[15], (const void*)a[16], (const void*)a[17], (const void*)a[18], w2f(a[19]), (const void*)a[20], (const void*)a[21], (const void*)a[22], (const void*)a[23], (const void*)a[24]); break;
                case 14: if (argc == 9) rc = vm_bn_infer_affine((const void*)a[0], (const void*)a[1], (const void*)a[2], (const void*)a[3], w2f(a[4]), (int)a[5], (const void*)a[6], (const void*)a[7], (const void*)a[8]); break;
                case 15: if (argc == 0) rc = vm_bn_part_rows(); break;
                case 16: if (argc == 4) rc = vm_bn_part_rows_used(a[0], (int)a[1], (int)a[2], (int)a[3]); break;
                case 17: if (argc == 14) rc = vm_bn_pool2d_stack_fwd((const void*)a[0], (const void*)a[1], (const void*)a[2], (const void*)a[3], a[4], (int)a[5], a[6], a[7], (int)a[8], (int)a[9], (int)a[10], (const void*)a[11], (const void*)a[12], (const void*)a[13]); break;
                case 18: if (argc == 15) rc = vm_bn_pool2d_stack_fwd_split((const void*)a[0], (const void*)a[1], (const void*)a[2], (const void*)a[3], (const void*)a[4], a[5], (int)a[6], a[7], a[8], (int)a[9], (int)a[10], (int)a[11], (const void*)a[12], (const void*)a[13], (const void*)a[14]); break;
                case 19: if (argc == 18) rc = vm_bn_pool_bwd_apply((const void*)a[0], (const void*)a[1], (const void*)a[2], (const void*)a[3], (const void*)a[4], (const void*)a[5], (const void*)a[6], (const void*)a[7], (const void*)a[8], a[9], a[10], a[11], (int)a[12], (int)a[13], (int)a[14], (const void*)a[15], (const void*)a[16], (const void*)a[17]); break;
                case 20: if (argc == 19) rc = vm_bn_pool_bwd_apply_gmax((const void*)a[0], (const void*)a[1], (const void*)a[2], (const void*)a[3], (const void*)a[4], (const void*)a[5], (const void*)a[6], (const void*)a[7], (const void*)a[8], (const void*)a[9], a[10], a[11], a[12], (int)a[13], (int)a[14], (int)a[15], (const void*)a[16], (const void*)a[17], (const void*)a[18]); break;
                case 21: if (argc == 19) rc = vm_bn_pool_bwd_apply_pairs((const void*)a[0], (const void*)a[1], (const void*)a[2], (const void*)a[3], (const void*)a[4], (const void*)a[5], (const void*)a[6], (const void*)a[7], (const void*)a[8], (const void*)a[9], a[10], a[11], a[12], (int)a[13], (int)a[14], (const void*)a[15], (const void*)a[16], (const void*)a[17], (const void*)a[18]); break;
                case 22: if (argc == 19) rc = vm_bn_pool_bwd_apply_pairs_gmax((const void*)a[0], (const void*)a[1], (const void*)a[2], (const void*)a[3], (const void*)a[4], (const void*)a[5], (const void*)a[6], (const void*)a[7], (const void*)a[8], (const void*)a[9], (const void*)a[10], a[11], a[12], a[13], (int)a[14], (int)a[15], (const void*)a[16], (const void*)a[17], (const void*)a[18]); break;
                case 23: if (argc == 16) rc = vm_bn_pool_bwd_reduce((const void*)a[0], (const void*)a[1], (const void*)a[2], (const void*)a[3], (const void*)a[4], (const void*)a[5], (const void*)a[6], a[7], a[8], a[9], (int)a[10], (int)a[11], (int)a[12], (const void*)a[13], (const void*)a[14], (const void*)a[15]); break;
                case 24: if (argc == 17) rc = vm_bn_pool_bwd_reduce_gmax((const void*)a[0], (const void*)a[1], (const void*)a[2], (const void*)a[3], (const void*)a[4], (const void*)a[5], (const void*)a[6], (const void*)a[7], a[8], a[9], a[10], (int)a[11], (int)a[12], (int)a[13], (const void*)a[14], (const void*)a[15], (const void*)a[16]); break;
                case 25: if (argc == 17) rc = vm_bn_pool_bwd_reduce_pooled((const void*)a[0], (const void*)a[1], (const void*)a[2], (const void*)a[3], (const void*)a[4], (const void*)a[5], (const void*)a[6], (const void*)a[7], a[8], a[9], a[10], (int)a[11], (int)a[12], (int)a[13], (const void*)a[14], (const void*)a[15], (const void*)a[16]); break;
                case 26: if (argc == 0) rc = vm_check_device(); break;
                case 27: if (argc == 7) rc = vm_clip_max_bwd((const void*)a[0], (const void*)a[1], a[2], (int)a[3], (int)a[4], (const void*)a[5], (const void*)a[6]); break;
                case 28: if (argc == 8) rc = vm_clip_max_fwd((const void*)a[0], a[1], (int)a[2], (int)a[3], (int)a[4], (const void*)a[5], (const void*)a[6], (const void*)a[7]); break;
                case 29: if (argc == 16) rc = vm_cohort_topk_stats((const void*)a[0], a[1], (const void*)a[2], a[3], (int)a[4], (int)a[5], (const void*)a[6], a[7], a[8], (const void*)a[9], (const void*)a[10], (const void*)a[11], (const void*)a[12], (const void*)a[13], (const void*)a[14], (const void*)a[15]); break;
                case 30: if (argc == 6) rc = vm_colsum((const void*)a[0], a[1], (int)a[2], (const void*)a[3], (const void*)a[4], (const void*)a[5]); break;
                case 31: if (argc == 7) rc = vm_colsum_strided((const void*)a[0], a[1], (int)a[2], (int)a[3], (const void*)a[4], (const void*)a[5], (const void*)a[6]); break;
                case 32: if (argc == 20) rc = vm_conv1_fused_bwd((const void*)a[0], (const void*)a[1], (const void*)a[2], (const void*)a[3], (const void*)a[4], (const void*)a[5], (const void*)a[6], (const void*)a[7], (const void*)a[8], (const void*)a[9], a[10], a[11], a[12], (int)a[13], (int)a[14], (int)a[15], (const void*)a[16], (const void*)a[17], (const void*)a[18], (const void*)a[19]); break;
                case 33: if (argc == 15) rc = vm_conv1_fused_fwd((const void*)a[0], (const void*)a[1], (const void*)a[2], (const void*)a[3], (const void*)a[4], a[5], a[6], (int)a[7], (int)a[8], (int)a[9], (int)a[10], (const void*)a[11], (const void*)a[12], (const void*)a[13], (const void*)a[14]); break;
                case 34: if (argc == 13) rc = vm_conv1_fused_fwd_varlen((const void*)a[0], (const void*)a[1], (const void*)a[2], (const void*)a[3], (const void*)a[4], (const void*)a[5], a[6], a[7], (int)a[8], (int)a[9], (int)a[10], (const void*)a[11], (const void*)a[12]); break;
                case 35: if (argc == 11) rc = vm_conv1_fwd((const void*)a[0], (const void*)a[1], (const void*)a[2], a[3], a[4], (int)a[5], (int)a[6], (const void*)a[7], (const void*)a[8], (const void*)a[9], (const void*)a[10]); break;
                case 36: if (argc == 9) rc = vm_conv1_wgrad((const void*)a[0], (const void*)a[1], a[2], a[3], (int)a[4], (int)a[5], (const void*)a[6], (const void*)a[7], (const void*)a[8]); break;
                case 37: if (argc == 18) rc = vm_conv2d_first_bn_pool_stack((const void*)a[0], (const void*)a[1], (const void*)a[2], (const void*)a[3], (const void*)a[4], (const void*)a[5], (const void*)a[6], a[7], (int)a[8], a[9], a[10], (int)a[11], (int)a[12], (int)a[13], (int)a[14], (const void*)a[15], (const void*)a[16], (const void*)a[17]); break;
                case 38: if (argc == 13) rc = vm_conv2d_first_fwd((const void*)a[0], (const void*)a[1], (const void*)a[2], a[3], (int)a[4], a[5], (int)a[6], (int)a[7], (int)a[8], (const void*)a[9], (const void*)a[10], (const void*)a[11], (const void*)a[12]); break;
                case 39: if (argc == 15) rc = vm_conv2d_first_fwd_split((const void*)a[0], (const void*)a[1], (const void*)a[2], (const void*)a[3], a[4], (int)a[5], a[6], (int)a[7], (int)a[8], (int)a[9], (const void*)a[10], (const void*)a[11], (const void*)a[12], (const void*)a[13], (const void*)a[14]); break;
                case 40: if (argc == 2) rc = vm_conv2d_first_supported((int)a[0], (int)a[1]); break;
                case 41: if (argc == 11) rc = vm_conv2d_first_wgrad((const void*)a[0], (const void*)a[1], a[2], (int)a[3], a[4], (int)a[5], (int)a[6], (int)a[7], (const void*)a[8], (const void*)a[9], (const void*)a[10]); break;
                case 42: if (argc == 9) rc = vm_conv_dgrad((const void*)a[0], (const void*)a[1], a[2], a[3], (int)a[4], (int)a[5], (int)a[6], (const void*)a[7], (const void*)a[8]); break;
                case 43: if (argc == 14) rc = vm_conv_dgrad_bnred((const void*)a[0], (const void*)a[1], a[2], a[3], (int)a[4], (int)a[5], (int)a[6], (const void*)a[7], (const void*)a[8], (int)a[9], (const void*)a[10], (const void*)a[11], (const void*)a[12], (const void*)a[13]); break;
                case 44: if (argc == 5) rc = vm_conv_dgrad_bnred_supported(a[0], a[1], (int)a[2], (int)a[3], (int)a[4]); break;
                case 45: if (argc == 12) rc = vm_conv_fwd((const void*)a[0], (const void*)a[1], (const void*)a[2], a[3], a[4], (int)a[5], (int)a[6], (int)a[7], (const void*)a[8], (const void*)a[9], (const void*)a[10], (const void*)a[11]); break;
                case 46: if (argc == 14) rc = vm_conv_fwd_e((const void*)a[0], (const void*)a[1], (const void*)a[2], (const void*)a[3], a[4], a[5], (int)a[6], (int)a[7], (int)a[8], (const void*)a[9], (const void*)a[10], (const void*)a[11], (const void*)a[12], (const void*)a[13]); break;
                case 47: if (argc == 5) rc = vm_conv_fwd_e_supported(a[0], a[1], (int)a[2], (int)a[3], (int)a[4]); break;
                case 48: if (argc == 12) rc = vm_conv_fwd_flat((const void*)a[0], (const void*)a[1], (const void*)a[2], a[3], a[4], (int)a[5], (int)a[6], (int)a[7], (const void*)a[8], (const void*)a[9], (const void*)a[10], (const void*)a[11]); break;
                case 49: if (argc == 19) rc = vm_conv_fwd_fold((const void*)a[0], (const void*)a[1], (const void*)a[2], (const void*)a[3], (const void*)a[4], a[5], a[6], a[7], (int)a[8], (int)a[9], (int)a[10], (const void*)a[11], (const void*)a[12], (const void*)a[13], (const void*)a[14], (const void*)a[15], (const void*)a[16], (const void*)a[17], (const void*)a[18]); break;
                case 50: if (argc == 6) rc = vm_conv_fwd_fold_supported(a[0], a[1], (int)a[2], (int)a[3], (int)a[4], (int)a[5]); break;
                case 51: if (argc == 13) rc = vm_conv_fwd_pool((const void*)a[0], (const void*)a[1], (const void*)a[2], (const void*)a[3], (const void*)a[4], a[5], a[6], (int)a[7], (int)a[8], (int)a[9], (const void*)a[10], (const void*)a[11], (const void*)a[12]); break;
                case 52: if (argc == 5) rc = vm_conv_fwd_pool_supported(a[0], a[1], (int)a[2], (int)a[3], (int)a[4]); break;
                case 53: if (argc == 14) rc = vm_conv_fwd_pool_varlen((const void*)a[0], (const void*)a[1], (const void*)a[2], (const void*)a[3], (const void*)a[4], (const void*)a[5], a[6], a[7], (int)a[8], (int)a[9], (int)a[10], (const void*)a[11], (const void*)a[12], (const void*)a[13]); break;
                case 54: if (argc == 10) rc = vm_conv_wgrad((const void*)a[0], (const void*)a[1], a[2], a[3], (int)a[4], (int)a[5], (int)a[6], (const void*)a[7], (const void*)a[8], (const void*)a[9]); break;
                case 55: if (argc == 14) rc = vm_conv_wgrad_fold((const void*)a[0], (const void*)a[1], a[2], a[3], a[4], (int)a[5], (int)a[6], (int)a[7], (const void*)a[8], (const void*)a[9], (const void*)a[10], (const void*)a[11], (const void*)a[12], (const void*)a[13]); break;
                case 56: if (argc == 11) rc = vm_conv_wgrad_fold_finish((const void*)a[0], a[1], a[2], a[3], (int)a[4], (int)a[5], (const void*)a[6], (const void*)a[7], (const void*)a[8], (const void*)a[9], (const void*)a[10]); break;
                case 57: if (argc == 4) rc = vm_conv_wgrad_splits(a[0], a[1], (int)a[2], (int)a[3]); break;
                case 58: if (argc == 22) rc = vm_crop_augment_decimate_whiten((const void*)a[0], (int)a[1], (const void*)a[2], a[3], a[4], (int)a[5], (int)a[6], w2f(a[7]), a[8], (const void*)a[9], (int)a[10], (const void*)a[11], (int)a[12], (const void*)a[13], (const void*)a[14], (const void*)a[15], (int)a[16], (int)a[17], (const void*)a[18], (const void*)a[19], (const void*)a[20], (const void*)a[21]); break;
                case 59: if (argc == 12) rc = vm_crop_decimate_whiten((const void*)a[0], (int)a[1], (const void*)a[2], a[3], a[4], (int)a[5], (int)a[6], w2f(a[7]), a[8], (const void*)a[9], (const void*)a[10], (const void*)a[11]); break;
                case 60: if (argc == 12) rc = vm_crop_decimate_whiten_varlen((const void*)a[0], (int)a[1], (const void*)a[2], (const void*)a[3], a[4], a[5], (int)a[6], (int)a[7], w2f(a[8]), (const void*)a[9], (const void*)a[10], (const void*)a[11]); break;
                case 61: if (argc == 11) rc = vm_decimate_whiten((const void*)a[0], (int)a[1], a[2], a[3], (int)a[4], (int)a[5], w2f(a[6]), a[7], (const void*)a[8], (const void*)a[9], (const void*)a[10]); break;
                case 62: if (argc == 10) rc = vm_dense_bwd((const void*)a[0], (const void*)a[1], (const void*)a[2], a[3], (int)a[4], (int)a[5], (const void*)a[6], (const void*)a[7], (const void*)a[8], (const void*)a[9]); break;
                case 63: if (argc == 8) rc = vm_dense_fwd((const void*)a[0], (const void*)a[1], (const void*)a[2], a[3], (int)a[4], (int)a[5], (const void*)a[6], (const void*)a[7]); break;
                case 64: if (argc == 11) rc = vm_du_tower_sums((const void*)a[0], (const void*)a[1], a[2], a[3], a[4], (int)a[5], (int)a[6], (const void*)a[7], (const void*)a[8], (const void*)a[9], (const void*)a[10]); break;
                case 65: if (argc == 1) rc = vm_event_destroy((const void*)a[0]); break;
                case 66: if (argc == 2) rc = vm_event_record((const void*)a[0], (const void*)a[1]); break;
                case 67: if (argc == 3) rc = vm_fill_zero((const void*)a[0], a[1], (const void*)a[2]); break;
                case 68: if (argc == 13) rc = vm_fold_bn_weights((const void*)a[0], (const void*)a[1], (const void*)a[2], (const void*)a[3], (int)a[4], (int)a[5], (int)a[6], (int)a[7], (const void*)a[8], (const void*)a[9], (const void*)a[10], (const void*)a[11], (const void*)a[12]); break;
                case 69: if (argc == 13) rc = vm_fold_pool_windows_bwd((const void*)a[0], (const void*)a[1], a[2], (int)a[3], a[4], (int)a[5], (int)a[6], (int)a[7], (int)a[8], (const void*)a[9], (const void*)a[10], (const void*)a[11], (const void*)a[12]); break;
                case 70: if (argc == 10) rc = vm_fold_windows((const void*)a[0], a[1], (int)a[2], a[3], (int)a[4], (int)a[5], (int)a[6], (int)a[7], (const void*)a[8], (const void*)a[9]); break;
                case 71: if (argc == 8) rc = vm_global_maxpool_bwd((const void*)a[0], (const void*)a[1], a[2], a[3], (int)a[4], (int)a[5], (const void*)a[6], (const void*)a[7]); break;
                case 72: if (argc == 8) rc = vm_global_maxpool_fwd((const void*)a[0], a[1], a[2], (int)a[3], (int)a[4], (const void*)a[5], (const void*)a[6], (const void*)a[7]); break;
                case 73: if (argc == 10) rc = vm_global_maxpool_fwd_varlen((const void*)a[0], (const void*)a[1], a[2], a[3], (int)a[4], (int)a[5], (const void*)a[6], (const void*)a[7], (const void*)a[8], (const void*)a[9]); break;
                case 74: if (argc == 5) rc = vm_grad_sqnorm((const void*)a[0], a[1], (const void*)a[2], (const void*)a[3], (const void*)a[4]); break;
                case 75: if (argc == 4) rc = vm_mfma_rate_probe((int)a[0], (int)a[1], (const void*)a[2], (const void*)a[3]); break;
                case 76: if (argc == 16) rc = vm_mine_pairs((const void*)a[0], (const void*)a[1], a[2], (int)a[3], (int)a[4], a[5], a[6], (int)a[7], (int)a[8], (const void*)a[9], (const void*)a[10], (const void*)a[11], (const void*)a[12], (const void*)a[13], (const void*)a[14], (const void*)a[15]); break;
                case 77: if (argc == 10) rc = vm_nshot_distances((const void*)a[0], (const void*)a[1], a[2], (int)a[3], (int)a[4], (int)a[5], (int)a[6], (const void*)a[7], (const void*)a[8], (const void*)a[9]); break;
                case 78: if (argc == 12) rc = vm_nshot_indexed((const void*)a[0], a[1], (const void*)a[2], (const void*)a[3], a[4], (int)a[5], (int)a[6], (int)a[7], (int)a[8], (const void*)a[9], (const void*)a[10], (const void*)a[11]); break;
                case 79: if (argc == 7) rc = vm_pack_nt_weights((const void*)a[0], (int)a[1], (int)a[2], (int)a[3], (int)a[4], (const void*)a[5], (const void*)a[6]); break;
                case 80: if (argc == 8) rc = vm_pack_nt_weights_batch((int)a[0], (const void*)a[1], (const void*)a[2], (const void*)a[3], (const void*)a[4], (int)a[5], (const void*)a[6], (const void*)a[7]); break;
                case 81: if (argc == 3) rc = vm_pack_nt_weights_supported((int)a[0], (int)a[1], (int)a[2]); break;
                case 82: if (argc == 14) rc = vm_pair_score_hist((const void*)a[0], (const void*)a[1], a[2], (int)a[3], (int)a[4], (const void*)a[5], a[6], a[7], (const void*)a[8], (int)a[9], (int)a[10], (const void*)a[11], (const void*)a[12], (const void*)a[13]); break;
                case 83: if (argc == 16) rc = vm_pair_score_hist_norm((const void*)a[0], (const void*)a[1], a[2], (int)a[3], (int)a[4], (const void*)a[5], a[6], a[7], (const void*)a[8], (int)a[9], (int)a[10], (const void*)a[11], (const void*)a[12], (const void*)a[13], (const void*)a[14], (const void*)a[15]); break;
                case 84: if (argc == 12) rc = vm_pairdist_argmin((const void*)a[0], (const void*)a[1], a[2], a[3], (int)a[4], (int)a[5], a[6], (const void*)a[7], (const void*)a[8], (const void*)a[9], (const void*)a[10], (const void*)a[11]); break;
                case 85: if (argc == 9) rc = vm_pool_windows_bwd((const void*)a[0], (const void*)a[1], a[2], (int)a[3], a[4], (int)a[5], (int)a[6], (const void*)a[7], (const void*)a[8]); break;
                case 86: if (argc == 8) rc = vm_pool_windows_fwd((const void*)a[0], a[1], (int)a[2], a[3], (int)a[4], (int)a[5], (const void*)a[6], (const void*)a[7]); break;
                case 87: if (argc == 7) rc = vm_prep_conv_weights((const void*)a[0], (int)a[1], (int)a[2], (int)a[3], (const void*)a[4], (const void*)a[5], (const void*)a[6]); break;
                case 88: if (argc == 9) rc = vm_prep_conv_weights_batch((int)a[0], (const void*)a[1], (const void*)a[2], (const void*)a[3], (int)a[4], (const void*)a[5], (const void*)a[6], (const void*)a[7], (const void*)a[8]); break;
                case 89: if (argc == 16) rc = vm_siamese_head_loss((const void*)a[0], (const void*)a[1], (const void*)a[2], (const void*)a[3], a[4], (int)a[5], (int)a[6], (int)a[7], w2f(a[8]), (const void*)a[9], (const void*)a[10], (const void*)a[11], (const void*)a[12], (const void*)a[13], (const void*)a[14], (const void*)a[15]); break;
                case 90: if (argc == 9) rc = vm_siamese_head_reduce((const void*)a[0], (const void*)a[1], a[2], (int)a[3], (int)a[4], (const void*)a[5], (const void*)a[6], (const void*)a[7], (const void*)a[8]); break;
                case 91: if (argc == 10) rc = vm_softmax_cce((const void*)a[0], (const void*)a[1], a[2], (int)a[3], w2f(a[4]), (const void*)a[5], (const void*)a[6], (const void*)a[7], (const void*)a[8], (const void*)a[9]); break;
                case 92: if (argc == 17) rc = vm_speaker_identify((const void*)a[0], (const void*)a[1], a[2], (int)a[3], (const void*)a[4], (const void*)a[5], (const void*)a[6], a[7], (int)a[8], (int)a[9], (const void*)a[10], (const void*)a[11], (const void*)a[12], (const void*)a[13], (const void*)a[14], (const void*)a[15], (const void*)a[16]); break;
                case 93: if (argc == 11) rc = vm_speaker_sums((const void*)a[0], (const void*)a[1], a[2], (int)a[3], a[4], (int)a[5], (const void*)a[6], (const void*)a[7], (const void*)a[8], (const void*)a[9], (const void*)a[10]); break;
                case 94: if (argc == 16) rc = vm_speaker_trial_hist((const void*)a[0], (const void*)a[1], a[2], (int)a[3], (const void*)a[4], (const void*)a[5], (const void*)a[6], a[7], (int)a[8], (int)a[9], (const void*)a[10], (int)a[11], (int)a[12], (const void*)a[13], (const void*)a[14], (const void*)a[15]); break;
                case 95: if (argc == 9) rc = vm_stack_windows((const void*)a[0], a[1], (int)a[2], a[3], (int)a[4], (int)a[5], (int)a[6], (const void*)a[7], (const void*)a[8]); break;
                case 96: if (argc == 13) rc = vm_stft_logmel((const void*)a[0], (int)a[1], a[2], a[3], (int)a[4], (int)a[5], (const void*)a[6], (const void*)a[7], (int)a[8], w2f(a[9]), (int)a[10], (const void*)a[11], (const void*)a[12]); break;
                case 97: if (argc == 13) rc = vm_stft_logmel_f16s((const void*)a[0], (int)a[1], a[2], a[3], (int)a[4], (int)a[5], (const void*)a[6], (const void*)a[7], (int)a[8], w2f(a[9]), (int)a[10], (const void*)a[11], (const void*)a[12]); break;
                case 98: if (argc == 14) rc = vm_stft_logmel_f16s_split((const void*)a[0], (int)a[1], a[2], a[3], (int)a[4], (int)a[5], (const void*)a[6], (const void*)a[7], (int)a[8], w2f(a[9]), (int)a[10], (const void*)a[11], (const void*)a[12], (const void*)a[13]); break;
                case 99: if (argc == 4) rc = vm_stft_split_basis((const void*)a[0], (int)a[1], (const void*)a[2], (const void*)a[3]); break;
                case 100: if (argc == 2) rc = vm_stream_wait_event((const void*)a[0], (const void*)a[1]); break;
                case 101: if (argc == 22) rc = vm_tail_fwd_bwd((const void*)a[0], (const void*)a[1], (int)a[2], (const void*)a[3], (const void*)a[4], (const void*)a[5], (const void*)a[6], (const void*)a[7], (const void*)a[8], (const void*)a[9], a[10], (int)a[11], (int)a[12], (int)a[13], (int)a[14], w2f(a[15]), (const void*)a[16], (const void*)a[17], (const void*)a[18], (const void*)a[19], (const void*)a[20], (const void*)a[21]); break;
                case 102: if (argc == 2) rc = vm_tail_fwd_bwd_supported((int)a[0], (int)a[1]); break;
                case 103: if (argc == 14) rc = vm_tail_param_grads((const void*)a[0], (const void*)a[1], (const void*)a[2], (const void*)a[3], a[4], (int)a[5], (int)a[6], (int)a[7], (const void*)a[8], (const void*)a[9], (const void*)a[10], (const void*)a[11], (const void*)a[12], (const void*)a[13]); break;
                default: break;
            }
        }
        if (rc != 0) {
            if (fail_at != nullptr) *fail_at = i;
            return rc;
        }
        i += 2 + argc;
    }
    return 0;
}
```

voicemap_amd/csrc/tail.hip:

```cpp
#include "common.hpp"

namespace vm {

template <typename T>
__global__ __launch_bounds__(256) void global_maxpool_fwd_kernel(const T* __restrict__ act, int64_t L, int C, int P,
                                                                 float* __restrict__ gmax, int32_t* __restrict__ gidx) {
    constexpr int VEC = Elem<T>::kVec;
    __shared__ float rv[256][VEC];
    __shared__ int ri[256][VEC];
    const int tid = threadIdx.x, RP = 256 / P, pl = tid % P, rl = tid / P;
    const int CV = C / VEC;
    const int64_t n = blockIdx.x;
    for (int cvb = 0; cvb < CV; cvb += P) {
        const int cv = cvb + pl;
        const bool cok = cv < CV;
        const int c0 = cv * VEC;
        float best[VEC];
        int bi[VEC];
#pragma unroll
        for (int i = 0; i < VEC; ++i) {
            best[i] = -INFINITY;
            bi[i] = 0x7fffffff;
        }
        if (cok) {
// ... 242 lines not shown
                                                                  int64_t pairs, int E, int head_kind,
                                                                  float* __restrict__ loss_acc, float* __restrict__ grad_hw,
                                                                  float* __restrict__ grad_hb) {
    __shared__ float red[4];
    const int tid = threadIdx.x;
    float l = 0.f, h = 0.f, gb = 0.f, gw = 0.f;
    for (int64_t b = tid; b < pairs; b += 256) {
        l += pair_ws[b * 4 + 0];
        h += pair_ws[b * 4 + 1];
        gb += pair_ws[b * 4 + 2];
        gw += pair_ws[b * 4 + 3];
    }
    const float ls = block_sum_256(l, red);
    const float hs = block_sum_256(h, red);
    const float gbs = block_sum_256(gb, red);
    const float gws = block_sum_256(gw, red);
    if (tid == 0) {
        loss_acc[0] = ls / (float)pairs;
        loss_acc[1] = hs / (float)pairs;
        grad_hb[0] = gbs;
        if (head_kind == VM_HEAD_UNIFORM_EUCLIDEAN) grad_hw[0] = gws;
    }
    if (head_kind == VM_HEAD_WEIGHTED_L1) {
        for (int j = tid; j < E; j += 256) {
            float acc = 0.f;
            for (int64_t b = 0; b < pairs; ++b) acc = fmaf(pair_ws[b * 4 + 2], fabsf(emb[b * E + j] - emb[(pairs + b) * E + j]), acc);
            grad_hw[j] = acc;
        }
    }
}

constexpr int TAIL_MAX_C = 1024, TAIL_MAX_E = 256;

__global__ __launch_bounds__(64 * DENSE_KS) void tail_pair_kernel(const float* __restrict__ part_v, const int32_t* __restrict__ part_i,
                                                                  int seg_rows, float* __restrict__ gmax, int32_t* __restrict__ gidx,
                                                                  const float* __restrict__ dw, const float* __restrict__ db,
                                                                  const float* __restrict__ hw, const float* __restrict__ hb,
                                                                  const float* __restrict__ y, int64_t pairs, int C, int E, int head_kind,
                                                                  int loss_kind, float grad_scale, float* __restrict__ emb,
                                                                  float* __restrict__ pred, float* __restrict__ demb,
                                                                  float* __restrict__ dgmax, float* __restrict__ pair_ws) {
    __shared__ float g[2][TAIL_MAX_C];
    __shared__ float ev[2][TAIL_MAX_E];
    __shared__ float de[2][TAIL_MAX_E];
    __shared__ float red[DENSE_KS][64];
    const int tid = threadIdx.x;
    const int64_t b = blockIdx.x;
    const int64_t win[2] = {b, pairs + b};
    for (int idx = tid; idx < 2 * C; idx += 64 * DENSE_KS) {
        const int w = idx >= C ? 1 : 0, c = idx - w * C;
        const int64_t n = win[w];
        float bv;
        if (part_v != nullptr) {
            bv = -INFINITY;
            int k = 0x7fffffff;
            for (int s = 0; s < seg_rows; ++s) {
                const float yv = part_v[(n * seg_rows + s) * C + c];
                const int kk = part_i[(n * seg_rows + s) * C + c];
                if (kk != 0x7fffffff && (k == 0x7fffffff || yv > bv || (yv == bv && kk < k))) {
                    bv = yv;
                    k = kk;
                }
            }
            gmax[n * C + c] = bv;
            gidx[n * C + c] = k;
        } else {
            bv = gmax[n * C + c];
        }
        g[w][c] = bv;
    }
    __syncthreads();
    {
        const int ol = tid & 63, kq = tid >> 6;
        const int per = (C + DENSE_KS - 1) / DENSE_KS;
        const int i0 = kq * per, i1 = min(C, i0 + per);
        for (int w = 0; w < 2; ++w) {
            for (int ob = 0; ob * 64 < E; ++ob) {
                const int o = ob * 64 + ol;
                const float* ir = g[w];
                float a[4] = {0.f, 0.f, 0.f, 0.f};
                if (o < E) {
                    int i = i0;
                    for (; i + 8 <= i1; i += 8) {
                        float x[8], yv[8];
#pragma unroll
                        for (int u = 0; u < 8; ++u) {
// ... 296 lines not shown
    hipLaunchKernelGGL(siamese_head_reduce_kernel, dim3(1), dim3(256), 0, (hipStream_t)stream, emb, ws, pairs, E, head_kind, loss_acc,
                       grad_hw, grad_hb);
    return check_launch("vm_siamese_head_reduce");
}

extern "C" int vm_softmax_cce(const float* logits, const int32_t* labels, int64_t rows, int n_classes, float grad_scale, float* prob,
                              float* loss_acc, float* dlogits, float* ws, void* stream) {
    VM_REQUIRE(logits && prob && rows > 0 && n_classes > 0, "vm_softmax_cce: bad argument");
    VM_REQUIRE(labels == nullptr || (loss_acc && ws), "vm_softmax_cce: loss_acc and ws (2*rows floats) required with labels");
    hipLaunchKernelGGL(softmax_cce_kernel, dim3((unsigned)rows), dim3(256), 0, (hipStream_t)stream, logits, labels, rows,
                       n_classes, prob, ws, ws ? ws + rows : nullptr, dlogits, grad_scale);
    int rc = check_launch("vm_softmax_cce");
    if (rc || labels == nullptr) return rc;
    hipLaunchKernelGGL(mean2_kernel, dim3(1), dim3(256), 0, (hipStream_t)stream, (const float*)ws, (const float*)(ws + rows),
                       rows, loss_acc);
    return check_launch("vm_softmax_cce(mean)");
}

extern "C" int vm_tail_fwd_bwd_supported(int C, int E) { return C > 0 && E > 0 && C <= TAIL_MAX_C && E <= TAIL_MAX_E; }

extern "C" int vm_tail_fwd_bwd(const float* gmax_part_v, const int32_t* gmax_part_i, int seg_rows, float* gmax, int32_t* gidx, const float* dense_w, const float* dense_b,
                               const float* head_w, const float* head_b, const float* y, int64_t pairs, int C, int E, int head_kind,
                               int loss_kind, float grad_scale, float* emb, float* pred, float* demb, float* dgmax, float* ws, void* stream) {
    VM_REQUIRE(gmax && gidx && dense_w && head_w && head_b && y && emb && pred && demb && dgmax && ws, "vm_tail_fwd_bwd: null pointer");
    VM_REQUIRE(pairs > 0 && vm_tail_fwd_bwd_supported(C, E), "vm_tail_fwd_bwd: needs pairs > 0, 0 < C <= %d, 0 < E <= %d (got %d, %d)",
               TAIL_MAX_C, TAIL_MAX_E, C, E);
    VM_REQUIRE((gmax_part_v == nullptr) == (gmax_part_i == nullptr) && (gmax_part_v == nullptr || seg_rows > 0),
               "vm_tail_fwd_bwd: gmax_part_v / gmax_part_i go together, with seg_rows > 0");
    VM_REQUIRE(head_kind == VM_HEAD_UNIFORM_EUCLIDEAN || head_kind == VM_HEAD_WEIGHTED_L1,
               "vm_tail_fwd_bwd: head_kind %d not implemented (the reference raises NotImplementedError too)", head_kind);
    VM_REQUIRE(loss_kind == VM_LOSS_CONTRASTIVE || loss_kind == VM_LOSS_BCE, "vm_tail_fwd_bwd: unknown loss %d", loss_kind);
    const float* part_v = gmax_part_v;
    const int32_t* part_i = gmax_part_i;
    hipLaunchKernelGGL(tail_pair_kernel, dim3((unsigned)pairs), dim3(64 * DENSE_KS), 0, (hipStream_t)stream, part_v, part_i, seg_rows, gmax,
                       gidx, dense_w, dense_b, head_w, head_b, y, pairs, C, E, head_kind, loss_kind, grad_scale, emb, pred, demb, dgmax, ws);
    return check_launch("vm_tail_fwd_bwd");
}

extern "C" int vm_tail_param_grads(const float* gmax, const float* demb, const float* emb, const float* ws, int64_t pairs, int C, int E,
                                   int head_kind, float* loss_acc, float* grad_dense_w, float* grad_dense_b, float* grad_hw, float* grad_hb,
                                   void* stream) {
    VM_REQUIRE(gmax && demb && emb && ws && loss_acc && grad_dense_w && grad_dense_b && grad_hw && grad_hb, "vm_tail_param_grads: null pointer");
    VM_REQUIRE(pairs > 0 && C > 0 && E > 0 && C < 65534, "vm_tail_param_grads: bad sizes");
    VM_REQUIRE(head_kind == VM_HEAD_UNIFORM_EUCLIDEAN || head_kind == VM_HEAD_WEIGHTED_L1, "vm_tail_param_grads: head_kind %d", head_kind);
    hipLaunchKernelGGL(tail_reduce_kernel, dim3((E + 63) / 64, C + 2), dim3(64 * DENSE_KS), 0, (hipStream_t)stream, gmax, demb, emb, ws, pairs,
                       C, E, head_kind, loss_acc, grad_dense_w, grad_dense_b, grad_hw, grad_hb);
    return check_launch("vm_tail_param_grads");
}
```

voicemap_amd/engine.py:

```python
from __future__ import annotations

import ctypes
import functools
import math
from collections import OrderedDict
from typing import Dict, List, Optional, Sequence, Tuple

import numpy as np
import torch

from . import _lib
from ._lib import VM_BF16, VM_F16, VM_F32, VM_F32S
from .program import DynF, DynI, Program, ProgramStore

_DT = {"f32": VM_F32, "fp32": VM_F32, "float32": VM_F32, "bf16": VM_BF16, "bfloat16": VM_BF16, "f32s": VM_F32S,
       "f16": VM_F16, "fp16": VM_F16, "float16": VM_F16}
_TORCH_DT = {VM_F32: torch.float32, VM_BF16: torch.bfloat16, VM_F32S: torch.float32, VM_F16: torch.float16}
DEFAULT_F16_LOSS_SCALE = 4096.0
DEFAULT_DTYPE = "f16"
HEADS = {"uniform_euclidean": _lib.VM_HEAD_UNIFORM_EUCLIDEAN, "weighted_l1": _lib.VM_HEAD_WEIGHTED_L1}
LOSSES = {"contrastive": _lib.VM_LOSS_CONTRASTIVE, "contrastive_loss": _lib.VM_LOSS_CONTRASTIVE,
          "bce": _lib.VM_LOSS_BCE, "binary_crossentropy": _lib.VM_LOSS_BCE}
CONV1_HALO_L, CONV1_HALO = 15, 31

# ... 35 lines not shown
    for i, (_, c, _) in enumerate(blocks):
        nt_off[f"bn{i+1}.moving_mean"] = (off, c)
        off += _align(c)
        nt_off[f"bn{i+1}.moving_variance"] = (off, c)
        off += _align(c)
    return spec, offsets, n_flat, nt_off, off


class FlatState:

    def __init__(self, blocks, embedding_dimension, head, num_classes, device):
        self.spec, self.offsets, self.n_flat, self.nt_off, n_nt = flat_layout(blocks, embedding_dimension, head, num_classes)
        self.n_params = sum(n for _, n, _ in self.offsets.values())
        self.P = torch.zeros(self.n_flat, dtype=torch.float32, device=device)
        self.G = torch.zeros_like(self.P)
        self.M = torch.zeros_like(self.P)
        self.V = torch.zeros_like(self.P)
        self.NT = torch.zeros(n_nt, dtype=torch.float32, device=device)
        self.iterations = 0

    def view(self, name: str, buf: Optional[torch.Tensor] = None) -> torch.Tensor:
        if name in self.nt_off:
            o, n = self.nt_off[name]
            return self.NT[o:o + n]
        o, n, shape = self.offsets[name]
        return (self.P if buf is None else buf)[o:o + n].view(shape)

    def refresh_weights(self):
        pass


_TIMED_AS = {"vm_conv_dgrad_bnred": ("vm_conv_dgrad", ()), "vm_conv_fwd_e": ("vm_conv_fwd", (3,)),
             "vm_conv_fwd_fold": ("vm_conv_fwd", (3, 4, 6, 15)), "vm_conv_wgrad_fold": ("vm_conv_wgrad", (3,)),
             "vm_bn_pool_bwd_apply_pairs": ("vm_bn_pool_bwd_apply", (1,))}


try:
    _raw_stream = torch._C._cuda_getCurrentRawStream
except AttributeError:
    def _raw_stream(index):
        return torch.cuda.current_stream(index).cuda_stream


_SHARED_STREAMS: Dict[tuple, "torch.cuda.Stream"] = {}


def _shared_stream(device: torch.device, role: str) -> "torch.cuda.Stream":
    idx = device.index if device.index is not None else torch.cuda.current_device()
    st = _SHARED_STREAMS.get((idx, role))
    if st is None:
        st = _SHARED_STREAMS[(idx, role)] = torch.cuda.Stream(device=device)
    return st


class HipEncoderEngine:

    _rec = None
    _stream_stack = ()
    replay = False
    native_replay = True
    fused_tail = False
    _packed_weights = False

    def __init__(self, blocks: Sequence[Tuple[int, int, int]], embedding_dimension: int, dropout: float = 0.05,
                 head: Optional[str] = None, num_classes: int = 0, dtype: str = DEFAULT_DTYPE, device="cuda",
                 bn_eps: float = 1e-3, bn_momentum: float = 0.99, unbiased_moving_variance: bool = True,
                 seed: Optional[int] = None):
# ... 41 lines not shown
            if self.is16 and self.nb - 1 <= 8:
                self.wt[i] = torch.empty(cout * 3 * cin, dtype=torch.float32, device=dev)
        self.packed_weights = self.is16
        self.wfp: Dict[int, torch.Tensor] = {}
        self.wdp: Dict[int, torch.Tensor] = {}
        for i in range(1, self.nb):
            cin, cout = self.blocks[i - 1][1], self.blocks[i][1]
            if self.is16 and self.lib.query("vm_pack_nt_weights_supported", cout, cin, self.dtype):
                self.wfp[i] = torch.empty(cout * 3 * cin, dtype=self.tdt, device=dev)
            if self.is16 and self.lib.query("vm_pack_nt_weights_supported", cin, cout, self.dtype):
                self.wdp[i] = torch.empty(cin * 3 * cout, dtype=self.tdt, device=dev)
        self._sq_ws = torch.empty(self.lib.query("vm_sqnorm_workspace_bytes", self.n_flat) // 8, dtype=torch.float64, device=dev)
        self._sqnorm = torch.zeros(1, dtype=torch.float32, device=dev)
        self.lr, self.beta_1, self.beta_2, self.adam_eps, self.decay, self.clipnorm = 1e-3, 0.9, 0.999, 1e-7, 0.0, 1.0
        self.iterations = 0
        self.last_infer_l0 = 0
        self.overlap_wgrad = True
        self.pooled_reduce = self.is16
        self.fused_bn_reduce = self.is16
        self.fused_sums_finalize = True
        self.wgrad_after_dgrad = False
        self.defer_wgrad_tail = 0
        self.misc_stream = _shared_stream(self.device, "misc")
        self.fused_pool_extreme = False
        self.fold_affine = self.is16
        self.fold_pairs = True
        self.center_blocks = (1,)
        import os as _os
        if _os.environ.get("VOICEMAP_CENTER_BLOCKS") is not None:
            self.center_blocks = tuple(int(v) for v in _os.environ["VOICEMAP_CENTER_BLOCKS"].split(",") if v.strip())
        self._fold = {}
        self.fused_infer_pool = self.is16
        self.last_pairs = False
        self.tower_swap = False
        self.tower_stagger = 0
        self.side_stream = _shared_stream(self.device, "tower")
        self._side_priority = 0
        self.split_towers = True
        self.tower_stream = _shared_stream(self.device, "tower")
        self.pre_overlap = True
        self.fused_tail = True
        self._seg_rows = self.lib.query("vm_bn_part_rows")
        self.defer_head_reduce = True
        self.grad_sync = None
        self.grad_prescale = 1.0
        self.sync_bn = False
        self.sync_bn_world = 1
        self._sync_bufs = {}
        self._plans: Dict[Tuple, dict] = {}
        self.replay = True
        self._rec: Optional[Program] = None
        self._programs = ProgramStore(self.lib, functools.partial(torch.cuda.synchronize, self.device))
        self._stream_stack: List[int] = []
        self._drop_bufs: Dict[int, tuple] = {}
        self.init_params(seed)

    def _init_loss_scale(self):
        self.loss_scaled = (self.dtype == VM_F16)
        self.loss_scale = DEFAULT_F16_LOSS_SCALE if self.loss_scaled else 1.0
        self._skipped = torch.zeros(1, dtype=torch.int32, device=self.device)
        self._skip_seen, self._clean_checks = 0, 0
        self.scale_poll_every, self.scale_poll_lag = 16, 8
        self.scale_grow_after, self.scale_max, self.scale_min = 2000, 2.0 ** 24, 1.0
        self.scale_norm_low = 64.0
        self.scale_norm_hold_polls, self._norm_growth_hold = 8, 0
        self._opt_calls, self._clean_steps, self._poll = 0, 0, None
# ... 475 lines not shown

    def _fold_plan(self, pl: dict):
        if "fold_ready" in pl:
            return
        n, ls, wpt = pl["n"], pl["L"], pl["wpt"]
        for i in range(self.nb - 1 if not (self.last_pairs and self.nb > 1) else self.nb):
            c = self.blocks[i][1]
            pl[i]["ep"] = torch.zeros(n, ls[i + 1] + 2, c, dtype=self.tdt, device=self.device)
            if i > 0:
                pl[i]["o"] = torch.empty(n, ls[i + 1], c, dtype=self.tdt, device=self.device)
        for i in range(1, self.nb):
            cin, c = self.blocks[i - 1][1], self.blocks[i][1]
            pl[i]["dsum"] = torch.empty(2, 3, c, dtype=torch.float32, device=self.device)
            ws = self.lib.query("vm_conv_wgrad_fold_workspace_bytes", n, wpt, ls[i], cin, c)
            pl[i]["wgrad_ws_fold"] = torch.empty(ws // 4 + 16, dtype=torch.float32, device=self.device)
        pl["fold_ready"] = wpt

    def forward(self, pl: dict, windows_per_tower: int, drop_masks: Optional[Sequence[Optional[torch.Tensor]]] = None,
                defer_tail: bool = False):
        n = pl["n"]
        training = pl["training"]
        n_towers = n // windows_per_tower if training else 1
        assert (not training) or n % windows_per_tower == 0
        assert n_towers <= 2 or not training, "at most two towers per call"
        wpt = windows_per_tower if training else n
        pl["wpt"], pl["drop"] = wpt, drop_masks
        split = training and n_towers == 2 and self.split_towers
        fold = training and self._fold_ok(pl, wpt, drop_masks)
        pl["fold_now"] = fold
        cl = self.blocks[-1][1]
        tail = bool(defer_tail and training and n_towers == 2 and self.fused_tail and self.head in HEADS
                    and self.lib.query("vm_tail_fwd_bwd_supported", cl, self.E))
        pl["tail_pending"] = tail
        pl["tail_parts"] = tail
        if fold:
            if pl.get("fold_ready", wpt) != wpt:
                del pl["fold_ready"]
                self._programs.drop_all()
            self._fold_plan(pl)
        if training:
            self.bn_steps += 1
            self._bn_t = self.bn_steps
        else:
            self._ensure_wfp()
        if split:
            if "cr_ws_t2" not in pl:
                pl["cr_ws_t2"] = torch.empty_like(pl["cr_ws"])
                pl["gmax_ws_t2"] = torch.empty_like(pl["gmax_ws"])
                pl["mov_scratch"] = torch.empty(2 * max(b[1] for b in self.blocks), dtype=torch.float32, device=self.device)
                pl["tower_ev"] = [torch.cuda.Event() for _ in self.blocks]
            cur = torch.cuda.current_stream(self.device)
            self._join(self.tower_stream, cur)
            pl["t2_stream"] = cur if self.tower_swap else self.tower_stream
            if self.tower_swap:
                with self._on(self.tower_stream):
                    self._forward_range(pl, 0, wpt, 0, 1, wpt, drop_masks, pl["cr_ws"], pl["gmax_ws"], first_of_two=True, fold=fold)
                self._forward_range(pl, wpt, wpt, 1, 1, wpt, drop_masks, pl["cr_ws_t2"], pl["gmax_ws_t2"], second_of_two=True, fold=fold)
            else:
                self._forward_range(pl, 0, wpt, 0, 1, wpt, drop_masks, pl["cr_ws"], pl["gmax_ws"], first_of_two=True, fold=fold)
                if self.tower_stagger and "stagger_ev" in pl:
                    self._wait(self.tower_stream, pl["stagger_ev"])
                with self._on(self.tower_stream):
                    self._forward_range(pl, wpt, wpt, 1, 1, wpt, drop_masks, pl["cr_ws_t2"], pl["gmax_ws_t2"], second_of_two=True, fold=fold)
            self._join(cur, self.tower_stream)
        else:
            self._forward_range(pl, 0, n, 0, n_towers, wpt, drop_masks, pl["cr_ws"], pl["gmax_ws"], fold=fold)
# ... 64 lines not shown
                    if first_of_two and self.tower_stagger == 2:
                        if "stagger_ev" not in pl:
                            pl["stagger_ev"] = torch.cuda.Event()
                        self._record(pl["stagger_ev"])
                else:
                    self._call("vm_bn_infer_affine", gam, bet, mm, mv, self.bn_eps, c, _p(b["scale"]), _p(b["shift"]), st)
                    self._call("vm_conv1_fused_fwd", W(pl["x0"]), w1, bias, _p(b["scale"]), _p(b["shift"]), nw, L, c, pool, 1, dt,
                               W(b["act"]), None, None, st)
                continue
            if i == 0:
                self._call("vm_conv1_fwd", W(pl["x0"]), _p(self.view("conv1.kernel")), bias, nw, L, c, dt, W(b["z"]), ssum, ssq, st)
            else:
                cin = self.blocks[i - 1][1]
                if (not training and self.fused_infer_pool and pool == 2
                        and self.lib.query("vm_conv_fwd_pool_supported", nw, L, cin, c, dt)):
                    self._call("vm_bn_infer_affine", gam, bet, mm, mv, self.bn_eps, c, _p(b["scale"]), _p(b["shift"]), st)
                    self._call("vm_conv_fwd_pool", W(pl[i - 1]["act"]), _p(self.wf[i]), bias, _p(b["scale"]), _p(b["shift"]), nw, L, cin,
                               c, dt, W(b["act"]), _p(self.wfp.get(i)) if self.packed_weights else None, st)
                    continue
                b["e_now"] = b["pairs_now"] = b["ctr_now"] = False
                if fold:
                    lo = pl[i - 1]
                    wfo, hbo, wfp = self._fold_bufs(i)
                    last_pairs = (i == self.nb - 1 and self.last_pairs and self.fold_pairs and pool == 2 and L % 2 == 0 and c % 8 == 0
                                  and bool(pl.get("tail_parts")) and self.fused_sums_finalize and not self.sync_bn and "o" in b)
                    with_e = i < self.nb - 1 or last_pairs
                    use_packed = wfp is not None and self.packed_weights
                    lo_c = (i == 1 and self.fuse_block1) or bool(lo.get("ctr_now"))
                    pairs = with_e and self.fold_pairs
                    ctr = T(b["ctr"]) if (pairs and dt == VM_F16 and i in self.center_blocks) else None
                    self._call("vm_fold_bn_weights", _p(self.wt[i]), T(lo["scale"]), T(lo["shift_c" if lo_c else "shift"]),
                               bias, ntw, cin, c, dt,
                               wfo[tw0].data_ptr(), wfp[tw0].data_ptr() if use_packed else None, hbo[tw0].data_ptr(), ctr, st)
                    self._call("vm_conv_fwd_fold", W(lo["ep"]), wfo[tw0].data_ptr(), bias, hbo[tw0].data_ptr(), gam if with_e else None,
                               nw, wpt, L, cin, c, dt, None if pairs else W(b["z"]), ssum, ssq, W(b["ep"]) if with_e else None,
                               W(b["o"]) if pairs else None, wfp[tw0].data_ptr() if use_packed else None, ctr, st)
                    b["e_now"], b["pairs_now"], b["ctr_now"] = with_e, pairs, ctr is not None
                    if last_pairs:
                        finalize()
                        parts, seg = pl["gmax_ws"], self._seg_rows
                        self._call("vm_bn_drop_pool_gmax_partials_e", W(b["ep"]), T(b["scale"]), T(b["shift"]), dm, nw, wpt, L // 2, c, dt,
                                   parts.data_ptr() + w0 * seg * c * 4, parts.data_ptr() + (pl["n"] + w0) * seg * c * 4, st)
                        fused_tail = True
                        continue
                    if with_e:
                        finalize()
                        continue
                elif (training and self.fused_pool_extreme and pool == 2 and i < self.nb - 1
                        and self.lib.query("vm_conv_fwd_e_supported", nw, L, cin, c, dt)):
                    if "e" not in b:
                        b["e"] = torch.empty(pl["n"], L // 2, c, dtype=self.tdt, device=self.device)
                    self._call("vm_conv_fwd_e", W(pl[i - 1]["act"]), _p(self.wf[i]), bias, gam, nw, L, cin, c, dt, W(b["z"]), ssum, ssq,
                               W(b["e"]), st)
                    finalize()
                    self._call("vm_bn_drop_pool_fwd", W(b["e"]), T(b["scale"]), T(b["shift"]), dm, nw, wpt, L // 2, c, 1, dt,
                               W(b["act"]), st)
                    b["e_now"] = True
                    continue
                else:
                    self._call("vm_conv_fwd", W(pl[i - 1]["act"]), _p(self.wf[i]), bias, nw, L, cin, c, dt, W(b["z"]), ssum, ssq, st)
            if training:
                finalize()
            else:
                self._call("vm_bn_infer_affine", gam, bet, mm, mv, self.bn_eps, c, _p(b["scale"]), _p(b["shift"]), st)
            sc, sh = (T(b["scale"]), T(b["shift"])) if training else (_p(b["scale"]), _p(b["shift"]))
            if i == self.nb - 1:
# ... 194 lines not shown
                else:
                    self._call("vm_conv_dgrad", _p(b["du"]), _p(self.wd[i]), n, L, cin, c, dt, _p(lo["dp"]), st)
                if late:
                    side_wgrad()
        if self.overlap_wgrad:
            self._join(torch.cuda.current_stream(self.device), self.side_stream)

    def _bnred_plan(self, pl: dict, i: int) -> bool:
        if not self.fused_bn_reduce or i < 1:
            return False
        lo, n, L = pl[i - 1], pl["n"], pl["L"][i]
        cin, c = self.blocks[i - 1][1], self.blocks[i][1]
        if not (i == 1 and self.fuse_block1) and not lo.get("e_now"):
            if not (self.pooled_reduce and pl["L"][i - 1] % self.blocks[i - 1][2] == 0):
                return False
        if not self.lib.query("vm_conv_dgrad_bnred_supported", n, L, cin, c, self.dtype):
            return False
        if "rs0" not in lo:
            lo["rs_rows"] = self.lib.query("vm_conv_dgrad_bnred_rows", L)
            for nm in ("rs0", "rs1"):
                lo[nm] = torch.empty(n * lo["rs_rows"], cin, dtype=torch.float32, device=self.device)
        return True

    def siamese_head(self, pl: dict, y: Optional[torch.Tensor], loss: str = "contrastive"):
        assert self.head in HEADS, "engine was built without a siamese head"
        pairs = pl["n"] // 2
        G = self.G
        train = y is not None
        if pl.get("tail_pending"):
            assert train, "forward(defer_tail=True) must be followed by siamese_head with labels"
            cl, parts, seg = self.blocks[-1][1], pl["gmax_ws"], self._seg_rows
            pv = parts.data_ptr() if pl["tail_parts"] else None
            pi = parts.data_ptr() + pl["n"] * seg * cl * 4 if pl["tail_parts"] else None
            self._call("vm_tail_fwd_bwd", pv, pi, seg, _p(pl["gmax"]), _p(pl["gidx"]), _p(self.view("dense.kernel")), _p(self.view("dense.bias")),
                       _p(self.view("head.kernel")), _p(self.view("head.bias")), self._dyn("y", _p(y)), pairs, cl, self.E, HEADS[self.head],
                       LOSSES[loss], self._dyn("loss_scale", float(self.loss_scale)), _p(pl["emb"]), _p(pl["pred"]), _p(pl["demb"]), _p(pl["dgmax"]), _p(pl["head_ws"]), self.stream())
            pl["tail_pending"], pl["tail_grads_pending"], pl["head_pending"] = False, True, False
            return pl["pred"][:pairs]
        defer = train and self.overlap_wgrad and pl["training"] and getattr(self, "defer_head_reduce", False)
        self._call("vm_siamese_head_loss", _p(pl["emb"]), _p(self.view("head.kernel")), _p(self.view("head.bias")),
                      self._dyn("y", _p(y)), pairs, self.E, HEADS[self.head], LOSSES[loss], self._dyn("loss_scale", float(self.loss_scale)),
                      _p(pl["pred"]),
                      _p(pl["loss_acc"]) if (train and not defer) else None, _p(pl["demb"]) if train else None,
                      _p(self.view("head.kernel", G)) if train else None, _p(self.view("head.bias", G)) if train else None,
                      _p(pl["head_ws"]), self.stream())
        pl["head_pending"] = defer
        return pl["pred"][:pairs]

    def classifier_head(self, pl: dict, labels: Optional[torch.Tensor]):
        assert self.head == "classifier"
        lib, st, n = self.lib, self.stream(), pl["n"]
        self._call("vm_dense_fwd", _p(pl["emb"]), _p(self.view("head.kernel")), _p(self.view("head.bias")), n, self.E,
                 self.num_classes, _p(pl["logits"]), st)
        train = labels is not None
        self._call("vm_softmax_cce", _p(pl["logits"]), self._dyn("y", _p(labels)), n, self.num_classes,
                 self._dyn("loss_scale", float(self.loss_scale)), _p(pl["prob"]),
                 _p(pl["loss_acc"]) if train else None, _p(pl["dlogits"]) if train else None, _p(pl["cce_ws"]), st)
        if train:
            G = self.G
            self._call("vm_dense_bwd", _p(pl["emb"]), _p(self.view("head.kernel")), _p(pl["dlogits"]), n, self.E,
                     self.num_classes, _p(self.view("head.kernel", G)), _p(self.view("head.bias", G)), _p(pl["demb"]), st)
        return pl["prob"]

    def _adam_scalars(self):
        lr = self.lr
        if self.decay > 0:
# ... 17 lines not shown
        self.iterations = t
        if skip and self._rec is None:
            self._poll_loss_scale()
        self.refresh_weights()
        if skip and self._rec is not None:
            self._poll_loss_scale()

    def make_drop_masks(self, n_windows: int, generator: Optional[torch.Generator] = None):
        if self.dropout <= 0.0:
            return None
        if generator is None:
            bufs = self._drop_bufs.get(n_windows)
            if bufs is None:
                tot = sum(n_windows * c for (_, c, _) in self.blocks)
                u = torch.empty(tot, dtype=torch.float32, device=self.device)
                m = torch.empty_like(u)
                views, o = [], 0
                for (_, c, _) in self.blocks:
                    views.append(m[o:o + n_windows * c].view(n_windows, c))
                    o += n_windows * c
                bufs = self._drop_bufs[n_windows] = (u, torch.empty(tot, dtype=torch.bool, device=self.device), m, views)
            u, keep, m, views = bufs
            u.uniform_(generator=self._drop_gen)
            torch.ge(u, self.dropout, out=keep)
            torch.mul(keep, 1.0 / (1.0 - self.dropout), out=m)
            return views
        out = []
        for (_, c, _) in self.blocks:
            u = torch.rand(n_windows, c, device=self.device, generator=generator)
            out.append((u >= self.dropout).to(torch.float32) / (1.0 - self.dropout))
        return out

    def _step_flags(self):
        return (self.fold_affine, self.fuse_block1, self.fused_bn_reduce, self.fused_sums_finalize, self.split_towers, self.tower_stagger, self.tower_swap, self.last_pairs,
                self.overlap_wgrad, self.wgrad_after_dgrad, self.defer_wgrad_tail, self.fused_pool_extreme, self.fold_pairs, self.pooled_reduce,
                self.packed_weights, self.fused_tail, self.defer_head_reduce, self.unbiased, self.clipnorm, self.loss_scaled,
                self.bn_zero_debias, self.bn_eps, self.bn_momentum, self.beta_1, self.beta_2, self.adam_eps, self._side_priority,
                self.grad_prescale, self.fused_infer_pool, self.center_blocks, self.pre_overlap, id(self.grad_sync), self.lib.tuning_epoch, id(self.side_stream), id(self.tower_stream), id(self.misc_stream))

    def _train_step(self, pl: dict, wpt: int, target: torch.Tensor, loss: Optional[str], drop_masks, apply_update: bool, pre,
                    input_ready: bool = False, aug: Optional[dict] = None):
        usable = (self.replay and (self.grad_sync is None or getattr(self.grad_sync, "replayable", False)) and not self.timed
                  and not self.sync_bn)
        prog = key = None
        if usable:
            sig = None if pre is None else ((pre[0], pre[1].dtype, tuple(pre[1].shape)) + tuple(pre[-2:]) if pre[0] == "raw"
                                            else (pre[0], pre[1].dtype, pre[3]) + tuple(pre[-2:]))
            if aug is not None:
                sig = sig + ("aug", int(aug["K"]), aug["noise"].dtype if aug["K"] else None,
                             None if aug.get("rirs") is None else (aug["rirs"].data_ptr(), tuple(aug["rirs"].shape)))
            masks = None if drop_masks is None else tuple(m is not None for m in drop_masks)
            key = (id(pl), wpt, loss, apply_update, self.stream(), sig, masks, bool(input_ready), self._step_flags())
            prog = self._programs.sight(key)
            if prog is not None and prog.finished:
                self._x0_handover(pl, prog)
                self._replay_step(prog, pl, wpt, target, drop_masks, apply_update, pre, aug)
                return
            self._rec = prog
        self._x0_handover(pl, "eager")
        try:
            if pre is not None:
                ahead = bool(input_ready and self.pre_overlap and not self.timed and pl["training"])
                if ahead:
                    cur = torch.cuda.current_stream(self.device)
                    if "x0_free_ev" not in pl:
                        pl["x0_free_ev"] = torch.cuda.Event()
                    pre_cm = self._on(self.tower_stream)
# ... 390 lines not shown
```

Measured before the change: 295,100 audio-s/s.

## Fuse global max/min pool extremes into last folded conv forward epilogue

Adds a new epilogue variant to the last block's folded-BN conv forward that computes per-tile per-channel max and min raw values with row indices, packed into uint32. The tail kernel then resolves the global max pool from these per-tile extremes, applying the BN scale and shift sign to pick max or min. This removes the separate pairs/pool output pass and the gmax partial reduction over the last block's activations. In exchange it adds packed-integer min/max work and LDS re-reads in the GEMM epilogue, which may raise register pressure.

After: 297,600 audio-s/s, median of 6. No clear change (+0.8%).

```diff
diff --git a/include/voicemap_hip.h b/include/voicemap_hip.h
--- a/include/voicemap_hip.h
+++ b/include/voicemap_hip.h
@@ -75,6 +75,10 @@
 int vm_fold_bn_weights(const float* wt, const float* scale, const float* shift, const float* bias, int towers, int c_in, int c_out,
                        int dtype, void* wf_folded, void* wf_packed, float* hb, float* ctr_out, void* stream);
 int vm_conv_fwd_fold_supported(int64_t n_windows, int64_t L, int c_in, int c_out, int dtype, int with_e);
+int64_t vm_conv_fwd_fold_gmax_rows(int64_t L);
+int vm_conv_fwd_fold_gmax(const void* in_e, const void* wf_folded, const float* bias, const float* hb, int64_t n_windows,
+                          int64_t windows_per_tower, int64_t L, int c_in, int c_out, int dtype, void* z, float* stat_sum,
+                          float* stat_sq, uint32_t* ext_max, uint32_t* ext_min, const void* wf_packed, void* stream);
 int vm_conv_fwd_fold(const void* in_e, const void* wf_folded, const float* bias, const float* hb, const float* gamma,
                      int64_t n_windows, int64_t windows_per_tower, int64_t L, int c_in, int c_out, int dtype, void* z, float* stat_sum,
                      float* stat_sq, void* e, void* o, const void* wf_packed, const float* e_center, void* stream);
@@ -210,6 +214,10 @@
 int vm_tail_fwd_bwd(const float* gmax_part_v, const int32_t* gmax_part_i, int seg_rows, float* gmax, int32_t* gidx, const float* dense_w, const float* dense_b,
                     const float* head_w, const float* head_b, const float* y, int64_t pairs, int C, int E, int head_kind,
                     int loss_kind, float grad_scale, float* emb, float* pred, float* demb, float* dgmax, float* ws, void* stream);
+int vm_tail_fwd_bwd_ext(const uint32_t* ext_max, const uint32_t* ext_min, const float* scale, const float* shift, int64_t L, int dtype,
+                        float* gmax, int32_t* gidx, const float* dense_w, const float* dense_b, const float* head_w,
+                        const float* head_b, const float* y, int64_t pairs, int C, int E, int head_kind, int loss_kind,
+                        float grad_scale, float* emb, float* pred, float* demb, float* dgmax, float* ws, void* stream);
 int vm_tail_param_grads(const float* gmax, const float* demb, const float* emb, const float* ws, int64_t pairs, int C, int E,
                         int head_kind, float* loss_acc, float* grad_dense_w, float* grad_dense_b, float* grad_hw, float* grad_hb,
                         void* stream);
diff --git a/voicemap_amd/csrc/conv_common.hpp b/voicemap_amd/csrc/conv_common.hpp
--- a/voicemap_amd/csrc/conv_common.hpp
+++ b/voicemap_amd/csrc/conv_common.hpp
@@ -169,7 +169,8 @@
     }
 }
 
-enum { EPI_FWD = 0, EPI_DGRAD = 1, EPI_FWD_POOL = 2, EPI_FWD_FOLD = 3 };
+enum { EPI_FWD = 0, EPI_DGRAD = 1, EPI_FWD_POOL = 2, EPI_FWD_FOLD = 3, EPI_FWD_FOLD_GMAX = 4 };
+constexpr bool epi_fold(int epi) { return epi == EPI_FWD_FOLD || epi == EPI_FWD_FOLD_GMAX; }
 
 template <typename T>
 struct NtArgs {
@@ -198,6 +199,8 @@
     int flat_period = 0, flat_valid = 0;
     const T* bt_packed = nullptr;
     const int32_t* valid_len = nullptr;
+    uint32_t* ext_max = nullptr;
+    uint32_t* ext_min = nullptr;
 };
 
 template <int AUX = 0>
diff --git a/voicemap_amd/csrc/conv_gemm.hip b/voicemap_amd/csrc/conv_gemm.hip
--- a/voicemap_amd/csrc/conv_gemm.hip
+++ b/voicemap_amd/csrc/conv_gemm.hip
@@ -472,10 +472,10 @@
                                      const f32x4 (&negc)[2][4]) {
     using namespace n2;
     const int r = lane & 31, kh = lane >> 5;
-    constexpr bool FWD = EPI == EPI_FWD || EPI == EPI_FWD_FOLD;
+    constexpr bool FWD = EPI == EPI_FWD || epi_fold(EPI);
     const bool red = EPI == EPI_DGRAD && p.red_a != nullptr;
     const int valid = (p.L - t0) < trows ? (p.L - t0) : trows;
-    constexpr bool CAN_CENTRE = EPI == EPI_FWD_FOLD && std::is_same<T, f16>::value;
+    constexpr bool CAN_CENTRE = epi_fold(EPI) && std::is_same<T, f16>::value;
     const bool ctrd = CAN_CENTRE && p.fold_ctr != nullptr;
     auto body = [&](auto ctrd_c) {
         constexpr bool CTRD = decltype(ctrd_c)::value;
@@ -539,7 +539,7 @@
     using namespace n2;
     using V8 = typename Mfma<T>::Frag;
     const int kh = lane >> 5;
-    constexpr bool FWD = EPI == EPI_FWD || EPI == EPI_FWD_FOLD;
+    constexpr bool FWD = EPI == EPI_FWD || epi_fold(EPI);
     const bool stats = FWD && p.stat_sum != nullptr && !(VM_ABL & 8);
     const bool red = EPI == EPI_DGRAD && p.red_a != nullptr;
     const int valid = (p.L - t0) < trows ? (p.L - t0) : trows;
@@ -624,7 +624,7 @@
             neg[2] = (g1[0] < 0.f ? 0xFFFFu : 0u) | (g1[1] < 0.f ? 0xFFFF0000u : 0u);
             neg[3] = (g1[2] < 0.f ? 0xFFFFu : 0u) | (g1[3] < 0.f ? 0xFFFF0000u : 0u);
         }
-        constexpr bool CAN_CENTRE = EPI == EPI_FWD_FOLD && std::is_same<T, f16>::value;
+        constexpr bool CAN_CENTRE = epi_fold(EPI) && std::is_same<T, f16>::value;
         const bool ctrd = CAN_CENTRE && p.fold_ctr != nullptr;
         u32x4 c16 = {0u, 0u, 0u, 0u};
         if (CAN_CENTRE && ctrd) {
@@ -698,6 +698,9 @@
         }
     }
     VM_EPI_MARK(5);
+    constexpr bool GMAX = EPI == EPI_FWD_FOLD_GMAX;
+    [[maybe_unused]] const int glim = valid < (p.L & ~1) - t0 ? valid : (p.L & ~1) - t0;
+    [[maybe_unused]] uint32_t gx = 0u, gn = 0xFFFFFFFFu;
     if (stats) {
 #if defined(__HIP_DEVICE_COMPILE__)
         const uint32_t lds0 = (uint32_t)(uintptr_t)(__attribute__((address_space(3))) const char*)lds;
@@ -744,6 +747,31 @@
                 d1b = Mfma4<T>::run(ones, hi[rs], d1b);
                 __builtin_amdgcn_sched_barrier(0);
             }
+            if constexpr (GMAX) {
+                auto steps = [&](auto interior_c) {
+                    constexpr bool INTERIOR = decltype(interior_c)::value;
+#pragma unroll
+                    for (int rs = 0; rs < 8; ++rs) {
+                        const int s = h * 8 + rs;
+                        if (INTERIOR ? s < 15 : s * 16 + 16 <= glim) {
+                            uint32_t a, b, mx, mn;
+                            asm("v_pk_max_u16 %0, %1, %2" : "=v"(a) : "v"(lo[rs][0]), "v"(lo[rs][1]));
+                            asm("v_pk_max_u16 %0, %1, %2" : "=v"(b) : "v"(hi[rs][0]), "v"(hi[rs][1]));
+                            asm("v_pk_max_u16 %0, %1, %2" : "=v"(mx) : "v"(a), "v"(b));
+                            asm("v_pk_min_u16 %0, %1, %2" : "=v"(a) : "v"(lo[rs][0]), "v"(lo[rs][1]));
+                            asm("v_pk_min_u16 %0, %1, %2" : "=v"(b) : "v"(hi[rs][0]), "v"(hi[rs][1]));
+                            asm("v_pk_min_u16 %0, %1, %2" : "=v"(mn) : "v"(a), "v"(b));
+                            const uint32_t x0 = (mx << 16) | (uint32_t)(16 - s), x1 = (mx & 0xFFFF0000u) | (uint32_t)(16 - s);
+                            const uint32_t m0 = (mn << 16) | (uint32_t)s, m1 = (mn & 0xFFFF0000u) | (uint32_t)s;
+                            const uint32_t xm = x0 > x1 ? x0 : x1, mm = m0 < m1 ? m0 : m1;
+                            gx = gx > xm ? gx : xm;
+                            gn = gn < mm ? gn : mm;
+                        }
+                    }
+                };
+                if (glim == 254) steps(std::true_type{});
+                else steps(std::false_type{});
+            }
             float ds = d1a[0] + d1b[0], dq = 0.f;
 #pragma unroll
             for (int e = 0; e < 4; ++e) dq = e == (lane & 3) ? d2a[e] + d2b[e] : dq;
@@ -755,6 +783,46 @@
                 p.stat_sq[srow * p.N + n0 + 32 * w + cn] = dq;
             }
             bar.point();
+        }
+        if constexpr (GMAX) {
+            const int cn = lane & 31;
+            const char* col = lds + (2 * kh) * TP + (32 * w + cn) * 2;
+            auto at = [&](int s, int i) { return s * 16 + 2 * kh + 4 * (i >> 1) + (i & 1); };
+            auto rd = [&](int s, int i) { return (uint32_t) * reinterpret_cast<const uint16_t*>(col + (s * 16 + 4 * (i >> 1) + (i & 1)) * TP); };
+            if (glim > 0 && (glim & 15) != 0) {
+                const int s = glim >> 4;
+#pragma unroll
+                for (int i = 0; i < 8; ++i) {
+                    const uint32_t v = rd(s, i) << 16;
+                    const bool ok = at(s, i) < glim;
+                    const uint32_t xk = ok ? (v | (uint32_t)(16 - s)) : 0u, mk = ok ? (v | (uint32_t)s) : 0xFFFFFFFFu;
+                    gx = gx > xk ? gx : xk;
+                    gn = gn < mk ? gn : mk;
+                }
+            }
+            uint32_t fx = 0u, fn = 0xFFFFFFFFu;
+            if (gx != 0u) {
+                const int s = 16 - (int)(gx & 0xFFFFu);
+                int best = 0;
+#pragma unroll
+                for (int i = 7; i >= 0; --i) best = (rd(s, i) == (gx >> 16) && at(s, i) < glim) ? at(s, i) : best;
+                fx = (gx & 0xFFFF0000u) | (uint32_t)(255 - best);
+            }
+            if (gn != 0xFFFFFFFFu) {
+                const int s = (int)(gn & 0xFFFFu);
+                int best = 0;
+#pragma unroll
+                for (int i = 7; i >= 0; --i) best = (rd(s, i) == (gn >> 16) && at(s, i) < glim) ? at(s, i) : best;
+                fn = (gn & 0xFFFF0000u) | (uint32_t)best;
+            }
+            const uint32_t ox = (uint32_t)__shfl_xor((int)fx, 32, 64), on = (uint32_t)__shfl_xor((int)fn, 32, 64);
+            fx = fx > ox ? fx : ox;
+            fn = fn < on ? fn : on;
+            if (kh == 0) {
+                const int64_t o = (n * p.tilesL + tl) * (int64_t)p.N + n0 + 32 * w + cn;
+                p.ext_max[o] = fx != 0u ? ((fx & 0xFFFF0000u) | (255u - (fx & 0xFFFFu))) : 0u;
+                p.ext_min[o] = fn != 0xFFFFFFFFu ? fn : 0u;
+            }
         }
     }
     VM_EPI_MARK(6);
@@ -854,7 +922,7 @@
 __device__ inline void n2_epilogue(const NtArgs<T>& p, char* lds, const f32x16 (&acc)[4][2], int64_t n, int tl, int t0, int n0, int trows,
                                    int tid, int lane, int w, int wm, int wn) {
     f32x4 negc[2][4];
-    if constexpr (EPI == EPI_FWD_FOLD && std::is_same<T, f16>::value) {
+    if constexpr (epi_fold(EPI) && std::is_same<T, f16>::value) {
         if (p.fold_ctr != nullptr) {
 #pragma unroll
             for (int j = 0; j < 2; ++j)
@@ -952,14 +1020,14 @@
     const int64_t n = nw;
     const int t0 = tl * TROWS, n0 = tn * TN;
     if (n2_pool_dead_tile<T, EPI>(p, n, t0, n0, tid)) return;
-    if constexpr (EPI == EPI_FWD_FOLD) {
+    if constexpr (epi_fold(EPI)) {
         const unsigned tw = nw / (unsigned)p.tower_windows;
         p.bt += tw * p.bt_tower_stride;
         p.fold_hb += tw * 4 * p.N;
         if (p.fold_ctr != nullptr) p.fold_ctr += tw * p.N;
     }
     f32x4 bias4[2][4];
-    if constexpr (EPI == EPI_FWD_FOLD) p.bias = p.fold_hb + 3 * p.N;
+    if constexpr (epi_fold(EPI)) p.bias = p.fold_hb + 3 * p.N;
     n2_load_bias<T, EPI>(p, bias4, n0 + wn * 64 + 4 * (lane >> 5));
 
     const int lrow = lane >> 2, lchunk = lane & 3;
@@ -1108,7 +1176,7 @@
         a_blk = a_blk == 2 ? 0 : a_blk + 1;
     }
     VM_PROF(const long long pt_loop = __builtin_amdgcn_s_memtime();)
-    if constexpr (EPI == EPI_FWD_FOLD) {
+    if constexpr (epi_fold(EPI)) {
         const int c0 = n0 + wn * 64 + 4 * (lane >> 5), rl = p.L - 1 - t0;
         if (t0 == 0) n2_fold_edge<T>(p, acc, 0, 0, wm, lane & 31, c0);
         if (rl >= 0 && rl < TROWS) n2_fold_edge<T>(p, acc, rl, 1, wm, lane & 31, c0);
@@ -1222,12 +1290,12 @@
     const int t0 = tl * n2r::TROWS, n0 = tn * TN;
     if (n2_pool_dead_tile<T, EPI>(p, n, t0, n0, tid)) return;
     unsigned tw = 0;
-    if constexpr (EPI == EPI_FWD_FOLD) {
+    if constexpr (epi_fold(EPI)) {
         tw = nw / (unsigned)p.tower_windows;
         p.fold_hb += tw * 4 * p.N;
         if (p.fold_ctr != nullptr) p.fold_ctr += tw * p.N;
     }
-    if constexpr (EPI == EPI_FWD_FOLD) p.bias = p.fold_hb + 3 * p.N;
+    if constexpr (epi_fold(EPI)) p.bias = p.fold_hb + 3 * p.N;
     f32x4 bias_lo[2][4], bias_hi[2][4];
     if constexpr (EPI != EPI_DGRAD) {
         const float* bp = p.bias + n0 + wn * 64;
@@ -1391,7 +1459,7 @@
 #undef VM_FRAG_READ
 #undef VM_MM
 #undef VM_LOAD_SET
-    if constexpr (EPI == EPI_FWD_FOLD) {
+    if constexpr (epi_fold(EPI)) {
         const int c0 = n0 + wn * 64 + 4 * (lane >> 5), rl = p.L - 1 - t0;
         if (t0 == 0) n2_fold_edge<T>(p, acc, 0, 0, wm, lane & 31, c0);
         if (rl >= 0 && rl < n2r::TROWS) n2_fold_edge<T>(p, acc, rl, 1, wm, lane & 31, c0);
@@ -1545,7 +1613,7 @@
 template <typename T, int EPI>
 static void launch_nt(const NtArgs<T>& a, int64_t n_windows, hipStream_t stream) {
     if constexpr (sizeof(T) == 2) {
-        if (!a.flat_period && (g_nt_n2 & (EPI == EPI_DGRAD ? 2 : 1)) && a.Ktot == 3 * a.a_c && n2r_shape(n_windows, a.L, a.a_c, a.N, EPI == EPI_FWD || EPI == EPI_FWD_FOLD)) {
+        if (!a.flat_period && (g_nt_n2 & (EPI == EPI_DGRAD ? 2 : 1)) && a.Ktot == 3 * a.a_c && n2r_shape(n_windows, a.L, a.a_c, a.N, EPI == EPI_FWD || epi_fold(EPI))) {
             launch_n2r<T, EPI>(a, n_windows, stream);
             return;
         }
@@ -1714,6 +1782,32 @@
     return check_launch("vm_conv_fwd_fold");
 }
 
+extern "C" int64_t vm_conv_fwd_fold_gmax_rows(int64_t L) { return L > 0 ? (L + n2r::TROWS - 1) / n2r::TROWS : 0; }
+
+extern "C" int vm_conv_fwd_fold_gmax(const void* in_e, const void* wf_folded, const float* bias, const float* hb, int64_t n_windows,
+                                     int64_t windows_per_tower, int64_t L, int c_in, int c_out, int dtype, void* z, float* stat_sum,
+                                     float* stat_sq, uint32_t* ext_max, uint32_t* ext_min, const void* wf_packed, void* stream) {
+    VM_REQUIRE(in_e && wf_folded && bias && hb && z && stat_sum && stat_sq && ext_max && ext_min, "vm_conv_fwd_fold_gmax: null pointer");
+    VM_REQUIRE(n_windows > 0 && L > 0 && windows_per_tower > 0 && n_windows % windows_per_tower == 0,
+               "vm_conv_fwd_fold_gmax: n_windows must be a positive multiple of windows_per_tower");
+    VM_REQUIRE((L + 2) * (int64_t)c_in < (1LL << 31) && 3LL * c_in * c_out < (1LL << 31), "vm_conv_fwd_fold_gmax: window too large");
+    if (!vm_conv_fwd_fold_supported(n_windows, L, c_in, c_out, dtype, 0)) {
+        set_error("vm_conv_fwd_fold_gmax: shape/dtype/tuning not served by the 256 x 128 input-resident kernel (ask vm_conv_fwd_fold_supported)");
+        return VM_ERR_UNSUPPORTED;
+    }
+    VM_DISPATCH_16(dtype, {
+        NtArgs<T> a = fwd_args<T>(in_e, wf_folded, bias, z, stat_sum, stat_sq, L, c_in, c_out, dtype);
+        a.fold_hb = hb;
+        a.tower_windows = windows_per_tower;
+        a.bt_tower_stride = 3LL * c_in * c_out;
+        a.bt_packed = (const T*)wf_packed;
+        a.ext_max = ext_max;
+        a.ext_min = ext_min;
+        launch_n2r<T, EPI_FWD_FOLD_GMAX>(a, n_windows, (hipStream_t)stream);
+    });
+    return check_launch("vm_conv_fwd_fold_gmax");
+}
+
 extern "C" int vm_conv_fwd_pool_supported(int64_t n_windows, int64_t L, int c_in, int c_out, int dtype) {
     return (is16(dtype) && (g_nt_n2 & 1) && L >= 2 && !(L & 1) && n2r_shape(n_windows, L, c_in, c_out, false)) ? 1 : 0;
 }
diff --git a/voicemap_amd/csrc/program_run.hip b/voicemap_amd/csrc/program_run.hip
--- a/voicemap_amd/csrc/program_run.hip
+++ b/voicemap_amd/csrc/program_run.hip
@@ -52,6 +52,7 @@
 int vm_conv_fwd_e_supported(int64_t, int64_t, int, int, int);
 int vm_conv_fwd_flat(const void*, const void*, const void*, int64_t, int64_t, int, int, int, const void*, const void*, const void*, const void*);
 int vm_conv_fwd_fold(const void*, const void*, const void*, const void*, const void*, int64_t, int64_t, int64_t, int, int, int, const void*, const void*, const void*, const void*, const void*, const void*, const void*, const void*);
+int vm_conv_fwd_fold_gmax(const void*, const void*, const void*, const void*, int64_t, int64_t, int64_t, int, int, int, const void*, const void*, const void*, const void*, const void*, const void*, const void*);
 int vm_conv_fwd_fold_supported(int64_t, int64_t, int, int, int, int);
 int vm_conv_fwd_pool(const void*, const void*, const void*, const void*, const void*, int64_t, int64_t, int, int, int, const void*, const void*, const void*);
 int vm_conv_fwd_pool_supported(int64_t, int64_t, int, int, int);
@@ -104,6 +105,7 @@
 int vm_stft_split_basis(const void*, int, const void*, const void*);
 int vm_stream_wait_event(const void*, const void*);
 int vm_tail_fwd_bwd(const void*, const void*, int, const void*, const void*, const void*, const void*, const void*, const void*, const void*, int64_t, int, int, int, int, float, const void*, const void*, const void*, const void*, const void*, const void*);
+int vm_tail_fwd_bwd_ext(const void*, const void*, const void*, const void*, int64_t, int, const void*, const void*, const void*, const void*, const void*, const void*, const void*, int64_t, int, int, int, int, float, const void*, const void*, const void*, const void*, const void*, const void*);
 int vm_tail_fwd_bwd_supported(int, int);
 int vm_tail_param_grads(const void*, const void*, const void*, const void*, int64_t, int, int, int, const void*, const void*, const void*, const void*, const void*, const void*);
 }
@@ -120,7 +122,7 @@
     return d;
 }
 
-extern "C" int64_t vm_program_table_hash(void) { return 1570090092LL; }
+extern "C" int64_t vm_program_table_hash(void) { return 104152648LL; }
 
 extern "C" int vm_program_run(const int64_t* w, int64_t n_words, int64_t* fail_at) {
     int64_t i = 0;
@@ -180,60 +182,62 @@
                 case 47: if (argc == 5) rc = vm_conv_fwd_e_supported(a[0], a[1], (int)a[2], (int)a[3], (int)a[4]); break;
                 case 48: if (argc == 12) rc = vm_conv_fwd_flat((const void*)a[0], (const void*)a[1], (const void*)a[2], a[3], a[4], (int)a[5], (int)a[6], (int)a[7], (const void*)a[8], (const void*)a[9], (const void*)a[10], (const void*)a[11]); break;
                 case 49: if (argc == 19) rc = vm_conv_fwd_fold((const void*)a[0], (const void*)a[1], (const void*)a[2], (const void*)a[3], (const void*)a[4], a[5], a[6], a[7], (int)a[8], (int)a[9], (int)a[10], (const void*)a[11], (const void*)a[12], (const void*)a[13], (const void*)a[14], (const void*)a[15], (const void*)a[16], (const void*)a[17], (const void*)a[18]); break;
-                case 50: if (argc == 6) rc = vm_conv_fwd_fold_supported(a[0], a[1], (int)a[2], (int)a[3], (int)a[4], (int)a[5]); break;
-                case 51: if (argc == 13) rc = vm_conv_fwd_pool((const void*)a[0], (const void*)a[1], (const void*)a[2], (const void*)a[3], (const void*)a[4], a[5], a[6], (int)a[7], (int)a[8], (int)a[9], (const void*)a[10], (const void*)a[11], (const void*)a[12]); break;
-                case 52: if (argc == 5) rc = vm_conv_fwd_pool_supported(a[0], a[1], (int)a[2], (int)a[3], (int)a[4]); break;
-                case 53: if (argc == 14) rc = vm_conv_fwd_pool_varlen((const void*)a[0], (const void*)a[1], (const void*)a[2], (const void*)a[3], (const void*)a[4], (const void*)a[5], a[6], a[7], (int)a[8], (int)a[9], (int)a[10], (const void*)a[11], (const void*)a[12], (const void*)a[13]); break;
-                case 54: if (argc == 10) rc = vm_conv_wgrad((const void*)a[0], (const void*)a[1], a[2], a[3], (int)a[4], (int)a[5], (int)a[6], (const void*)a[7], (const void*)a[8], (const void*)a[9]); break;
-                case 55: if (argc == 14) rc = vm_conv_wgrad_fold((const void*)a[0], (const void*)a[1], a[2], a[3], a[4], (int)a[5], (int)a[6], (int)a[7], (const void*)a[8], (const void*)a[9], (const void*)a[10], (const void*)a[11], (const void*)a[12], (const void*)a[13]); break;
-                case 56: if (argc == 11) rc = vm_conv_wgrad_fold_finish((const void*)a[0], a[1], a[2], a[3], (int)a[4], (int)a[5], (const void*)a[6], (const void*)a[7], (const void*)a[8], (const void*)a[9], (const void*)a[10]); break;
-                case 57: if (argc == 4) rc = vm_conv_wgrad_splits(a[0], a[1], (int)a[2], (int)a[3]); break;
-                case 58: if (argc == 22) rc = vm_crop_augment_decimate_whiten((const void*)a[0], (int)a[1], (const void*)a[2], a[3], a[4], (int)a[5], (int)a[6], w2f(a[7]), a[8], (const void*)a[9], (int)a[10], (const void*)a[11], (int)a[12], (const void*)a[13], (const void*)a[14], (const void*)a[15], (int)a[16], (int)a[17], (const void*)a[18], (const void*)a[19], (const void*)a[20], (const void*)a[21]); break;
-                case 59: if (argc == 12) rc = vm_crop_decimate_whiten((const void*)a[0], (int)a[1], (const void*)a[2], a[3], a[4], (int)a[5], (int)a[6], w2f(a[7]), a[8], (const void*)a[9], (const void*)a[10], (const void*)a[11]); break;
-                case 60: if (argc == 12) rc = vm_crop_decimate_whiten_varlen((const void*)a[0], (int)a[1], (const void*)a[2], (const void*)a[3], a[4], a[5], (int)a[6], (int)a[7], w2f(a[8]), (const void*)a[9], (const void*)a[10], (const void*)a[11]); break;
-                case 61: if (argc == 11) rc = vm_decimate_whiten((const void*)a[0], (int)a[1], a[2], a[3], (int)a[4], (int)a[5], w2f(a[6]), a[7], (const void*)a[8], (const void*)a[9], (const void*)a[10]); break;
-                case 62: if (argc == 10) rc = vm_dense_bwd((const void*)a[0], (const void*)a[1], (const void*)a[2], a[3], (int)a[4], (int)a[5], (const void*)a[6], (const void*)a[7], (const void*)a[8], (const void*)a[9]); break;
-                case 63: if (argc == 8) rc = vm_dense_fwd((const void*)a[0], (const void*)a[1], (const void*)a[2], a[3], (int)a[4], (int)a[5], (const void*)a[6], (const void*)a[7]); break;
-                case 64: if (argc == 11) rc = vm_du_tower_sums((const void*)a[0], (const void*)a[1], a[2], a[3], a[4], (int)a[5], (int)a[6], (const void*)a[7], (const void*)a[8], (const void*)a[9], (const void*)a[10]); break;
-                case 65: if (argc == 1) rc = vm_event_destroy((const void*)a[0]); break;
-                case 66: if (argc == 2) rc = vm_event_record((const void*)a[0], (const void*)a[1]); break;
-                case 67: if (argc == 3) rc = vm_fill_zero((const void*)a[0], a[1], (const void*)a[2]); break;
-                case 68: if (argc == 13) rc = vm_fold_bn_weights((const void*)a[0], (const void*)a[1], (const void*)a[2], (const void*)a[3], (int)a[4], (int)a[5], (int)a[6], (int)a[7], (const void*)a[8], (const void*)a[9], (const void*)a[10], (const void*)a[11], (const void*)a[12]); break;
-                case 69: if (argc == 13) rc = vm_fold_pool_windows_bwd((const void*)a[0], (const void*)a[1], a[2], (int)a[3], a[4], (int)a[5], (int)a[6], (int)a[7], (int)a[8], (const void*)a[9], (const void*)a[10], (const void*)a[11], (const void*)a[12]); break;
-                case 70: if (argc == 10) rc = vm_fold_windows((const void*)a[0], a[1], (int)a[2], a[3], (int)a[4], (int)a[5], (int)a[6], (int)a[7], (const void*)a[8], (const void*)a[9]); break;
-                case 71: if (argc == 8) rc = vm_global_maxpool_bwd((const void*)a[0], (const void*)a[1], a[2], a[3], (int)a[4], (int)a[5], (const void*)a[6], (const void*)a[7]); break;
-                case 72: if (argc == 8) rc = vm_global_maxpool_fwd((const void*)a[0], a[1], a[2], (int)a[3], (int)a[4], (const void*)a[5], (const void*)a[6], (const void*)a[7]); break;
-                case 73: if (argc == 10) rc = vm_global_maxpool_fwd_varlen((const void*)a[0], (const void*)a[1], a[2], a[3], (int)a[4], (int)a[5], (const void*)a[6], (const void*)a[7], (const void*)a[8], (const void*)a[9]); break;
-                case 74: if (argc == 5) rc = vm_grad_sqnorm((const void*)a[0], a[1], (const void*)a[2], (const void*)a[3], (const void*)a[4]); break;
-                case 75: if (argc == 4) rc = vm_mfma_rate_probe((int)a[0], (int)a[1], (const void*)a[2], (const void*)a[3]); break;
-                case 76: if (argc == 16) rc = vm_mine_pairs((const void*)a[0], (const void*)a[1], a[2], (int)a[3], (int)a[4], a[5], a[6], (int)a[7], (int)a[8], (const void*)a[9], (const void*)a[10], (const void*)a[11], (const void*)a[12], (const void*)a[13], (const void*)a[14], (const void*)a[15]); break;
-                case 77: if (argc == 10) rc = vm_nshot_distances((const void*)a[0], (const void*)a[1], a[2], (int)a[3], (int)a[4], (int)a[5], (int)a[6], (const void*)a[7], (const void*)a[8], (const void*)a[9]); break;
-                case 78: if (argc == 12) rc = vm_nshot_indexed((const void*)a[0], a[1], (const void*)a[2], (const void*)a[3], a[4], (int)a[5], (int)a[6], (int)a[7], (int)a[8], (const void*)a[9], (const void*)a[10], (const void*)a[11]); break;
-                case 79: if (argc == 7) rc = vm_pack_nt_weights((const void*)a[0], (int)a[1], (int)a[2], (int)a[3], (int)a[4], (const void*)a[5], (const void*)a[6]); break;
-                case 80: if (argc == 8) rc = vm_pack_nt_weights_batch((int)a[0], (const void*)a[1], (const void*)a[2], (const void*)a[3], (const void*)a[4], (int)a[5], (const void*)a[6], (const void*)a[7]); break;
-                case 81: if (argc == 3) rc = vm_pack_nt_weights_supported((int)a[0], (int)a[1], (int)a[2]); break;
-                case 82: if (argc == 14) rc = vm_pair_score_hist((const void*)a[0], (const void*)a[1], a[2], (int)a[3], (int)a[4], (const void*)a[5], a[6], a[7], (const void*)a[8], (int)a[9], (int)a[10], (const void*)a[11], (const void*)a[12], (const void*)a[13]); break;
-                case 83: if (argc == 16) rc = vm_pair_score_hist_norm((const void*)a[0], (const void*)a[1], a[2], (int)a[3], (int)a[4], (const void*)a[5], a[6], a[7], (const void*)a[8], (int)a[9], (int)a[10], (const void*)a[11], (const void*)a[12], (const void*)a[13], (const void*)a[14], (const void*)a[15]); break;
-                case 84: if (argc == 12) rc = vm_pairdist_argmin((const void*)a[0], (const void*)a[1], a[2], a[3], (int)a[4], (int)a[5], a[6], (const void*)a[7], (const void*)a[8], (const void*)a[9], (const void*)a[10], (const void*)a[11]); break;
-                case 85: if (argc == 9) rc = vm_pool_windows_bwd((const void*)a[0], (const void*)a[1], a[2], (int)a[3], a[4], (int)a[5], (int)a[6], (const void*)a[7], (const void*)a[8]); break;
-                case 86: if (argc == 8) rc = vm_pool_windows_fwd((const void*)a[0], a[1], (int)a[2], a[3], (int)a[4], (int)a[5], (const void*)a[6], (const void*)a[7]); break;
-                case 87: if (argc == 7) rc = vm_prep_conv_weights((const void*)a[0], (int)a[1], (int)a[2], (int)a[3], (const void*)a[4], (const void*)a[5], (const void*)a[6]); break;
-                case 88: if (argc == 9) rc = vm_prep_conv_weights_batch((int)a[0], (const void*)a[1], (const void*)a[2], (const void*)a[3], (int)a[4], (const void*)a[5], (const void*)a[6], (const void*)a[7], (const void*)a[8]); break;
-                case 89: if (argc == 16) rc = vm_siamese_head_loss((const void*)a[0], (const void*)a[1], (const void*)a[2], (const void*)a[3], a[4], (int)a[5], (int)a[6], (int)a[7], w2f(a[8]), (const void*)a[9], (const void*)a[10], (const void*)a[11], (const void*)a[12], (const void*)a[13], (const void*)a[14], (const void*)a[15]); break;
-                case 90: if (argc == 9) rc = vm_siamese_head_reduce((const void*)a[0], (const void*)a[1], a[2], (int)a[3], (int)a[4], (const void*)a[5], (const void*)a[6], (const void*)a[7], (const void*)a[8]); break;
-                case 91: if (argc == 10) rc = vm_softmax_cce((const void*)a[0], (const void*)a[1], a[2], (int)a[3], w2f(a[4]), (const void*)a[5], (const void*)a[6], (const void*)a[7], (const void*)a[8], (const void*)a[9]); break;
-                case 92: if (argc == 17) rc = vm_speaker_identify((const void*)a[0], (const void*)a[1], a[2], (int)a[3], (const void*)a[4], (const void*)a[5], (const void*)a[6], a[7], (int)a[8], (int)a[9], (const void*)a[10], (const void*)a[11], (const void*)a[12], (const void*)a[13], (const void*)a[14], (const void*)a[15], (const void*)a[16]); break;
-                case 93: if (argc == 11) rc = vm_speaker_sums((const void*)a[0], (const void*)a[1], a[2], (int)a[3], a[4], (int)a[5], (const void*)a[6], (const void*)a[7], (const void*)a[8], (const void*)a[9], (const void*)a[10]); break;
-                case 94: if (argc == 16) rc = vm_speaker_trial_hist((const void*)a[0], (const void*)a[1], a[2], (int)a[3], (const void*)a[4], (const void*)a[5], (const void*)a[6], a[7], (int)a[8], (int)a[9], (const void*)a[10], (int)a[11], (int)a[12], (const void*)a[13], (const void*)a[14], (const void*)a[15]); break;
-                case 95: if (argc == 9) rc = vm_stack_windows((const void*)a[0], a[1], (int)a[2], a[3], (int)a[4], (int)a[5], (int)a[6], (const void*)a[7], (const void*)a[8]); break;
-                case 96: if (argc == 13) rc = vm_stft_logmel((const void*)a[0], (int)a[1], a[2], a[3], (int)a[4], (int)a[5], (const void*)a[6], (const void*)a[7], (int)a[8], w2f(a[9]), (int)a[10], (const void*)a[11], (const void*)a[12]); break;
-                case 97: if (argc == 13) rc = vm_stft_logmel_f16s((const void*)a[0], (int)a[1], a[2], a[3], (int)a[4], (int)a[5], (const void*)a[6], (const void*)a[7], (int)a[8], w2f(a[9]), (int)a[10], (const void*)a[11], (const void*)a[12]); break;
-                case 98: if (argc == 14) rc = vm_stft_logmel_f16s_split((const void*)a[0], (int)a[1], a[2], a[3], (int)a[4], (int)a[5], (const void*)a[6], (const void*)a[7], (int)a[8], w2f(a[9]), (int)a[10], (const void*)a[11], (const void*)a[12], (const void*)a[13]); break;
-                case 99: if (argc == 4) rc = vm_stft_split_basis((const void*)a[0], (int)a[1], (const void*)a[2], (const void*)a[3]); break;
-                case 100: if (argc == 2) rc = vm_stream_wait_event((const void*)a[0], (const void*)a[1]); break;
-                case 101: if (argc == 22) rc = vm_tail_fwd_bwd((const void*)a[0], (const void*)a[1], (int)a[2], (const void*)a[3], (const void*)a[4], (const void*)a[5], (const void*)a[6], (const void*)a[7], (const void*)a[8], (const void*)a[9], a[10], (int)a[11], (int)a[12], (int)a[13], (int)a[14], w2f(a[15]), (const void*)a[16], (const void*)a[17], (const void*)a[18], (const void*)a[19], (const void*)a[20], (const void*)a[21]); break;
-                case 102: if (argc == 2) rc = vm_tail_fwd_bwd_supported((int)a[0], (int)a[1]); break;
-                case 103: if (argc == 14) rc = vm_tail_param_grads((const void*)a[0], (const void*)a[1], (const void*)a[2], (const void*)a[3], a[4], (int)a[5], (int)a[6], (int)a[7], (const void*)a[8], (const void*)a[9], (const void*)a[10], (const void*)a[11], (const void*)a[12], (const void*)a[13]); break;
+                case 50: if (argc == 17) rc = vm_conv_fwd_fold_gmax((const void*)a[0], (const void*)a[1], (const void*)a[2], (const void*)a[3], a[4], a[5], a[6], (int)a[7], (int)a[8], (int)a[9], (const void*)a[10], (const void*)a[11], (const void*)a[12], (const void*)a[13], (const void*)a[14], (const void*)a[15], (const void*)a[16]); break;
+                case 51: if (argc == 6) rc = vm_conv_fwd_fold_supported(a[0], a[1], (int)a[2], (int)a[3], (int)a[4], (int)a[5]); break;
+                case 52: if (argc == 13) rc = vm_conv_fwd_pool((const void*)a[0], (const void*)a[1], (const void*)a[2], (const void*)a[3], (const void*)a[4], a[5], a[6], (int)a[7], (int)a[8], (int)a[9], (const void*)a[10], (const void*)a[11], (const void*)a[12]); break;
+                case 53: if (argc == 5) rc = vm_conv_fwd_pool_supported(a[0], a[1], (int)a[2], (int)a[3], (int)a[4]); break;
+                case 54: if (argc == 14) rc = vm_conv_fwd_pool_varlen((const void*)a[0], (const void*)a[1], (const void*)a[2], (const void*)a[3], (const void*)a[4], (const void*)a[5], a[6], a[7], (int)a[8], (int)a[9], (int)a[10], (const void*)a[11], (const void*)a[12], (const void*)a[13]); break;
+                case 55: if (argc == 10) rc = vm_conv_wgrad((const void*)a[0], (const void*)a[1], a[2], a[3], (int)a[4], (int)a[5], (int)a[6], (const void*)a[7], (const void*)a[8], (const void*)a[9]); break;
+                case 56: if (argc == 14) rc = vm_conv_wgrad_fold((const void*)a[0], (const void*)a[1], a[2], a[3], a[4], (int)a[5], (int)a[6], (int)a[7], (const void*)a[8], (const void*)a[9], (const void*)a[10], (const void*)a[11], (const void*)a[12], (const void*)a[13]); break;
+                case 57: if (argc == 11) rc = vm_conv_wgrad_fold_finish((const void*)a[0], a[1], a[2], a[3], (int)a[4], (int)a[5], (const void*)a[6], (const void*)a[7], (const void*)a[8], (const void*)a[9], (const void*)a[10]); break;
+                case 58: if (argc == 4) rc = vm_conv_wgrad_splits(a[0], a[1], (int)a[2], (int)a[3]); break;
+                case 59: if (argc == 22) rc = vm_crop_augment_decimate_whiten((const void*)a[0], (int)a[1], (const void*)a[2], a[3], a[4], (int)a[5], (int)a[6], w2f(a[7]), a[8], (const void*)a[9], (int)a[10], (const void*)a[11], (int)a[12], (const void*)a[13], (const void*)a[14], (const void*)a[15], (int)a[16], (int)a[17], (const void*)a[18], (const void*)a[19], (const void*)a[20], (const void*)a[21]); break;
+                case 60: if (argc == 12) rc = vm_crop_decimate_whiten((const void*)a[0], (int)a[1], (const void*)a[2], a[3], a[4], (int)a[5], (int)a[6], w2f(a[7]), a[8], (const void*)a[9], (const void*)a[10], (const void*)a[11]); break;
+                case 61: if (argc == 12) rc = vm_crop_decimate_whiten_varlen((const void*)a[0], (int)a[1], (const void*)a[2], (const void*)a[3], a[4], a[5], (int)a[6], (int)a[7], w2f(a[8]), (const void*)a[9], (const void*)a[10], (const void*)a[11]); break;
+                case 62: if (argc == 11) rc = vm_decimate_whiten((const void*)a[0], (int)a[1], a[2], a[3], (int)a[4], (int)a[5], w2f(a[6]), a[7], (const void*)a[8], (const void*)a[9], (const void*)a[10]); break;
+                case 63: if (argc == 10) rc = vm_dense_bwd((const void*)a[0], (const void*)a[1], (const void*)a[2], a[3], (int)a[4], (int)a[5], (const void*)a[6], (const void*)a[7], (const void*)a[8], (const void*)a[9]); break;
+                case 64: if (argc == 8) rc = vm_dense_fwd((const void*)a[0], (const void*)a[1], (const void*)a[2], a[3], (int)a[4], (int)a[5], (const void*)a[6], (const void*)a[7]); break;
+                case 65: if (argc == 11) rc = vm_du_tower_sums((const void*)a[0], (const void*)a[1], a[2], a[3], a[4], (int)a[5], (int)a[6], (const void*)a[7], (const void*)a[8], (const void*)a[9], (const void*)a[10]); break;
+                case 66: if (argc == 1) rc = vm_event_destroy((const void*)a[0]); break;
+                case 67: if (argc == 2) rc = vm_event_record((const void*)a[0], (const void*)a[1]); break;
+                case 68: if (argc == 3) rc = vm_fill_zero((const void*)a[0], a[1], (const void*)a[2]); break;
+                case 69: if (argc == 13) rc = vm_fold_bn_weights((const void*)a[0], (const void*)a[1], (const void*)a[2], (const void*)a[3], (int)a[4], (int)a[5], (int)a[6], (int)a[7], (const void*)a[8], (const void*)a[9], (const void*)a[10], (const void*)a[11], (const void*)a[12]); break;
+                case 70: if (argc == 13) rc = vm_fold_pool_windows_bwd((const void*)a[0], (const void*)a[1], a[2], (int)a[3], a[4], (int)a[5], (int)a[6], (int)a[7], (int)a[8], (const void*)a[9], (const void*)a[10], (const void*)a[11], (const void*)a[12]); break;
+                case 71: if (argc == 10) rc = vm_fold_windows((const void*)a[0], a[1], (int)a[2], a[3], (int)a[4], (int)a[5], (int)a[6], (int)a[7], (const void*)a[8], (const void*)a[9]); break;
+                case 72: if (argc == 8) rc = vm_global_maxpool_bwd((const void*)a[0], (const void*)a[1], a[2], a[3], (int)a[4], (int)a[5], (const void*)a[6], (const void*)a[7]); break;
+                case 73: if (argc == 8) rc = vm_global_maxpool_fwd((const void*)a[0], a[1], a[2], (int)a[3], (int)a[4], (const void*)a[5], (const void*)a[6], (const void*)a[7]); break;
+                case 74: if (argc == 10) rc = vm_global_maxpool_fwd_varlen((const void*)a[0], (const void*)a[1], a[2], a[3], (int)a[4], (int)a[5], (const void*)a[6], (const void*)a[7], (const void*)a[8], (const void*)a[9]); break;
+                case 75: if (argc == 5) rc = vm_grad_sqnorm((const void*)a[0], a[1], (const void*)a[2], (const void*)a[3], (const void*)a[4]); break;
+                case 76: if (argc == 4) rc = vm_mfma_rate_probe((int)a[0], (int)a[1], (const void*)a[2], (const void*)a[3]); break;
+                case 77: if (argc == 16) rc = vm_mine_pairs((const void*)a[0], (const void*)a[1], a[2], (int)a[3], (int)a[4], a[5], a[6], (int)a[7], (int)a[8], (const void*)a[9], (const void*)a[10], (const void*)a[11], (const void*)a[12], (const void*)a[13], (const void*)a[14], (const void*)a[15]); break;
+                case 78: if (argc == 10) rc = vm_nshot_distances((const void*)a[0], (const void*)a[1], a[2], (int)a[3], (int)a[4], (int)a[5], (int)a[6], (const void*)a[7], (const void*)a[8], (const void*)a[9]); break;
+                case 79: if (argc == 12) rc = vm_nshot_indexed((const void*)a[0], a[1], (const void*)a[2], (const void*)a[3], a[4], (int)a[5], (int)a[6], (int)a[7], (int)a[8], (const void*)a[9], (const void*)a[10], (const void*)a[11]); break;
+                case 80: if (argc == 7) rc = vm_pack_nt_weights((const void*)a[0], (int)a[1], (int)a[2], (int)a[3], (int)a[4], (const void*)a[5], (const void*)a[6]); break;
+                case 81: if (argc == 8) rc = vm_pack_nt_weights_batch((int)a[0], (const void*)a[1], (const void*)a[2], (const void*)a[3], (const void*)a[4], (int)a[5], (const void*)a[6], (const void*)a[7]); break;
+                case 82: if (argc == 3) rc = vm_pack_nt_weights_supported((int)a[0], (int)a[1], (int)a[2]); break;
+                case 83: if (argc == 14) rc = vm_pair_score_hist((const void*)a[0], (const void*)a[1], a[2], (int)a[3], (int)a[4], (const void*)a[5], a[6], a[7], (const void*)a[8], (int)a[9], (int)a[10], (const void*)a[11], (const void*)a[12], (const void*)a[13]); break;
+                case 84: if (argc == 16) rc = vm_pair_score_hist_norm((const void*)a[0], (const void*)a[1], a[2], (int)a[3], (int)a[4], (const void*)a[5], a[6], a[7], (const void*)a[8], (int)a[9], (int)a[10], (const void*)a[11], (const void*)a[12], (const void*)a[13], (const void*)a[14], (const void*)a[15]); break;
+                case 85: if (argc == 12) rc = vm_pairdist_argmin((const void*)a[0], (const void*)a[1], a[2], a[3], (int)a[4], (int)a[5], a[6], (const void*)a[7], (const void*)a[8], (const void*)a[9], (const void*)a[10], (const void*)a[11]); break;
+                case 86: if (argc == 9) rc = vm_pool_windows_bwd((const void*)a[0], (const void*)a[1], a[2], (int)a[3], a[4], (int)a[5], (int)a[6], (const void*)a[7], (const void*)a[8]); break;
+                case 87: if (argc == 8) rc = vm_pool_windows_fwd((const void*)a[0], a[1], (int)a[2], a[3], (int)a[4], (int)a[5], (const void*)a[6], (const void*)a[7]); break;
+                case 88: if (argc == 7) rc = vm_prep_conv_weights((const void*)a[0], (int)a[1], (int)a[2], (int)a[3], (const void*)a[4], (const void*)a[5], (const void*)a[6]); break;
+                case 89: if (argc == 9) rc = vm_prep_conv_weights_batch((int)a[0], (const void*)a[1], (const void*)a[2], (const void*)a[3], (int)a[4], (const void*)a[5], (const void*)a[6], (const void*)a[7], (const void*)a[8]); break;
+                case 90: if (argc == 16) rc = vm_siamese_head_loss((const void*)a[0], (const void*)a[1], (const void*)a[2], (const void*)a[3], a[4], (int)a[5], (int)a[6], (int)a[7], w2f(a[8]), (const void*)a[9], (const void*)a[10], (const void*)a[11], (const void*)a[12], (const void*)a[13], (const void*)a[14], (const void*)a[15]); break;
+                case 91: if (argc == 9) rc = vm_siamese_head_reduce((const void*)a[0], (const void*)a[1], a[2], (int)a[3], (int)a[4], (const void*)a[5], (const void*)a[6], (const void*)a[7], (const void*)a[8]); break;
+                case 92: if (argc == 10) rc = vm_softmax_cce((const void*)a[0], (const void*)a[1], a[2], (int)a[3], w2f(a[4]), (const void*)a[5], (const void*)a[6], (const void*)a[7], (const void*)a[8], (const void*)a[9]); break;
+                case 93: if (argc == 17) rc = vm_speaker_identify((const void*)a[0], (const void*)a[1], a[2], (int)a[3], (const void*)a[4], (const void*)a[5], (const void*)a[6], a[7], (int)a[8], (int)a[9], (const void*)a[10], (const void*)a[11], (const void*)a[12], (const void*)a[13], (const void*)a[14], (const void*)a[15], (const void*)a[16]); break;
+                case 94: if (argc == 11) rc = vm_speaker_sums((const void*)a[0], (const void*)a[1], a[2], (int)a[3], a[4], (int)a[5], (const void*)a[6], (const void*)a[7], (const void*)a[8], (const void*)a[9], (const void*)a[10]); break;
+                case 95: if (argc == 16) rc = vm_speaker_trial_hist((const void*)a[0], (const void*)a[1], a[2], (int)a[3], (const void*)a[4], (const void*)a[5], (const void*)a[6], a[7], (int)a[8], (int)a[9], (const void*)a[10], (int)a[11], (int)a[12], (const void*)a[13], (const void*)a[14], (const void*)a[15]); break;
+                case 96: if (argc == 9) rc = vm_stack_windows((const void*)a[0], a[1], (int)a[2], a[3], (int)a[4], (int)a[5], (int)a[6], (const void*)a[7], (const void*)a[8]); break;
+                case 97: if (argc == 13) rc = vm_stft_logmel((const void*)a[0], (int)a[1], a[2], a[3], (int)a[4], (int)a[5], (const void*)a[6], (const void*)a[7], (int)a[8], w2f(a[9]), (int)a[10], (const void*)a[11], (const void*)a[12]); break;
+                case 98: if (argc == 13) rc = vm_stft_logmel_f16s((const void*)a[0], (int)a[1], a[2], a[3], (int)a[4], (int)a[5], (const void*)a[6], (const void*)a[7], (int)a[8], w2f(a[9]), (int)a[10], (const void*)a[11], (const void*)a[12]); break;
+                case 99: if (argc == 14) rc = vm_stft_logmel_f16s_split((const void*)a[0], (int)a[1], a[2], a[3], (int)a[4], (int)a[5], (const void*)a[6], (const void*)a[7], (int)a[8], w2f(a[9]), (int)a[10], (const void*)a[11], (const void*)a[12], (const void*)a[13]); break;
+                case 100: if (argc == 4) rc = vm_stft_split_basis((const void*)a[0], (int)a[1], (const void*)a[2], (const void*)a[3]); break;
+                case 101: if (argc == 2) rc = vm_stream_wait_event((const void*)a[0], (const void*)a[1]); break;
+                case 102: if (argc == 22) rc = vm_tail_fwd_bwd((const void*)a[0], (const void*)a[1], (int)a[2], (const void*)a[3], (const void*)a[4], (const void*)a[5], (const void*)a[6], (const void*)a[7], (const void*)a[8], (const void*)a[9], a[10], (int)a[11], (int)a[12], (int)a[13], (int)a[14], w2f(a[15]), (const void*)a[16], (const void*)a[17], (const void*)a[18], (const void*)a[19], (const void*)a[20], (const void*)a[21]); break;
+                case 103: if (argc == 25) rc = vm_tail_fwd_bwd_ext((const void*)a[0], (const void*)a[1], (const void*)a[2], (const void*)a[3], a[4], (int)a[5], (const void*)a[6], (const void*)a[7], (const void*)a[8], (const void*)a[9], (const void*)a[10], (const void*)a[11], (const void*)a[12], a[13], (int)a[14], (int)a[15], (int)a[16], (int)a[17], w2f(a[18]), (const void*)a[19], (const void*)a[20], (const void*)a[21], (const void*)a[22], (const void*)a[23], (const void*)a[24]); break;
+                case 104: if (argc == 2) rc = vm_tail_fwd_bwd_supported((int)a[0], (int)a[1]); break;
+                case 105: if (argc == 14) rc = vm_tail_param_grads((const void*)a[0], (const void*)a[1], (const void*)a[2], (const void*)a[3], a[4], (int)a[5], (int)a[6], (int)a[7], (const void*)a[8], (const void*)a[9], (const void*)a[10], (const void*)a[11], (const void*)a[12], (const void*)a[13]); break;
                 default: break;
             }
         }
diff --git a/voicemap_amd/csrc/tail.hip b/voicemap_amd/csrc/tail.hip
--- a/voicemap_amd/csrc/tail.hip
+++ b/voicemap_amd/csrc/tail.hip
@@ -298,7 +298,49 @@
 
 constexpr int TAIL_MAX_C = 1024, TAIL_MAX_E = 256;
 
+struct TailExt {
+    const uint32_t* emax;
+    const uint32_t* emin;
+    const float* scale;
+    const float* shift;
+    int64_t wpt;
+    int L, tiles, f16;
+};
+constexpr int TAIL_EXT_ROWS = 254;
+
+__device__ inline float tail_ext_gmax(const TailExt& x, int64_t n, int c, int C, int* pos) {
+    const int64_t tw = n / x.wpt;
+    const float sc = x.scale[tw * C + c], sh = x.shift[tw * C + c];
+    const uint32_t* part = sc < 0.f ? x.emin : x.emax;
+    uint32_t bv = 0u;
+    int row = -1;
+    for (int t = 0; t < x.tiles; ++t) {
+        if ((x.L & ~1) - t * TAIL_EXT_ROWS <= 0) break;
+        const uint32_t k = part[(n * x.tiles + t) * C + c];
+        const uint32_t v = k >> 16;
+        if (row < 0 || (sc < 0.f ? v < bv : v > bv)) {
+            bv = v;
+            row = t * TAIL_EXT_ROWS + (int)(k & 0xFFFFu);
+        }
+    }
+    float u, y;
+    if (x.f16) {
+        u = (float)__builtin_bit_cast(f16, (uint16_t)bv);
+    } else {
+        u = __builtin_bit_cast(float, bv << 16);
+    }
+    if (sc == 0.f) {
+        row = 0;
+        u = 0.f;
+    }
+    y = fmaf(u, sc, sh) * 1.f;
+    y = x.f16 ? (float)(f16)y : (float)(bf16)y;
+    *pos = row >> 1;
+    return y;
+}
+
 __global__ __launch_bounds__(64 * DENSE_KS) void tail_pair_kernel(const float* __restrict__ part_v, const int32_t* __restrict__ part_i,
+                                                                  TailExt ext,
                                                                   int seg_rows, float* __restrict__ gmax, int32_t* __restrict__ gidx,
                                                                   const float* __restrict__ dw, const float* __restrict__ db,
                                                                   const float* __restrict__ hw, const float* __restrict__ hb,
@@ -317,7 +359,12 @@
         const int w = idx >= C ? 1 : 0, c = idx - w * C;
         const int64_t n = win[w];
         float bv;
-        if (part_v != nullptr) {
+        if (ext.emax != nullptr) {
+            int k;
+            bv = tail_ext_gmax(ext, n, c, C, &k);
+            gmax[n * C + c] = bv;
+            gidx[n * C + c] = k;
+        } else if (part_v != nullptr) {
             bv = -INFINITY;
             int k = 0x7fffffff;
             for (int s = 0; s < seg_rows; ++s) {
@@ -680,9 +727,37 @@
     VM_REQUIRE(loss_kind == VM_LOSS_CONTRASTIVE || loss_kind == VM_LOSS_BCE, "vm_tail_fwd_bwd: unknown loss %d", loss_kind);
     const float* part_v = gmax_part_v;
     const int32_t* part_i = gmax_part_i;
-    hipLaunchKernelGGL(tail_pair_kernel, dim3((unsigned)pairs), dim3(64 * DENSE_KS), 0, (hipStream_t)stream, part_v, part_i, seg_rows, gmax,
+    hipLaunchKernelGGL(tail_pair_kernel, dim3((unsigned)pairs), dim3(64 * DENSE_KS), 0, (hipStream_t)stream, part_v, part_i, TailExt{}, seg_rows, gmax,
                        gidx, dense_w, dense_b, head_w, head_b, y, pairs, C, E, head_kind, loss_kind, grad_scale, emb, pred, demb, dgmax, ws);
     return check_launch("vm_tail_fwd_bwd");
+}
+
+extern "C" int vm_tail_fwd_bwd_ext(const uint32_t* ext_max, const uint32_t* ext_min, const float* scale, const float* shift, int64_t L, int dtype,
+                                   float* gmax, int32_t* gidx, const float* dense_w, const float* dense_b, const float* head_w,
+                                   const float* head_b, const float* y, int64_t pairs, int C, int E, int head_kind, int loss_kind,
+                                   float grad_scale, float* emb, float* pred, float* demb, float* dgmax, float* ws, void* stream) {
+    VM_REQUIRE(ext_max && ext_min && scale && shift && gmax && gidx && dense_w && head_w && head_b && y && emb && pred && demb && dgmax && ws,
+               "vm_tail_fwd_bwd_ext: null pointer");
+    VM_REQUIRE(pairs > 0 && vm_tail_fwd_bwd_supported(C, E), "vm_tail_fwd_bwd_ext: needs pairs > 0, 0 < C <= %d, 0 < E <= %d (got %d, %d)",
+               TAIL_MAX_C, TAIL_MAX_E, C, E);
+    VM_REQUIRE(L >= 2 && L < (1LL << 30), "vm_tail_fwd_bwd_ext: L must hold a pool pair");
+    VM_REQUIRE(dtype == VM_BF16 || dtype == VM_F16, "vm_tail_fwd_bwd_ext: 16-bit storage only");
+    VM_REQUIRE(head_kind == VM_HEAD_UNIFORM_EUCLIDEAN || head_kind == VM_HEAD_WEIGHTED_L1,
+               "vm_tail_fwd_bwd_ext: head_kind %d not implemented (the reference raises NotImplementedError too)", head_kind);
+    VM_REQUIRE(loss_kind == VM_LOSS_CONTRASTIVE || loss_kind == VM_LOSS_BCE, "vm_tail_fwd_bwd_ext: unknown loss %d", loss_kind);
+    TailExt ext;
+    ext.emax = ext_max;
+    ext.emin = ext_min;
+    ext.scale = scale;
+    ext.shift = shift;
+    ext.wpt = pairs;
+    ext.L = (int)L;
+    ext.tiles = (int)((L + TAIL_EXT_ROWS - 1) / TAIL_EXT_ROWS);
+    ext.f16 = dtype == VM_F16;
+    hipLaunchKernelGGL(tail_pair_kernel, dim3((unsigned)pairs), dim3(64 * DENSE_KS), 0, (hipStream_t)stream, (const float*)nullptr,
+                       (const int32_t*)nullptr, ext, 0, gmax, gidx, dense_w, dense_b, head_w, head_b, y, pairs, C, E, head_kind, loss_kind, grad_scale,
+                       emb, pred, demb, dgmax, ws);
+    return check_launch("vm_tail_fwd_bwd_ext");
 }
 
 extern "C" int vm_tail_param_grads(const float* gmax, const float* demb, const float* emb, const float* ws, int64_t pairs, int C, int E,
diff --git a/voicemap_amd/engine.py b/voicemap_amd/engine.py
--- a/voicemap_amd/engine.py
+++ b/voicemap_amd/engine.py
@@ -91,7 +91,8 @@
 
 _TIMED_AS = {"vm_conv_dgrad_bnred": ("vm_conv_dgrad", ()), "vm_conv_fwd_e": ("vm_conv_fwd", (3,)),
              "vm_conv_fwd_fold": ("vm_conv_fwd", (3, 4, 6, 15)), "vm_conv_wgrad_fold": ("vm_conv_wgrad", (3,)),
-             "vm_bn_pool_bwd_apply_pairs": ("vm_bn_pool_bwd_apply", (1,))}
+             "vm_bn_pool_bwd_apply_pairs": ("vm_bn_pool_bwd_apply", (1,)),
+             "vm_conv_fwd_fold_gmax": ("vm_conv_fwd", (3, 5)), "vm_tail_fwd_bwd_ext": ("vm_tail_fwd_bwd", (3, 4, 5))}
 
 
 try:
@@ -199,6 +200,7 @@
         self._fold = {}
         self.fused_infer_pool = self.is16
         self.last_pairs = False
+        self.fused_gmax = True
         self.tower_swap = False
         self.tower_stagger = 0
         self.side_stream = _shared_stream(self.device, "tower")
@@ -740,6 +742,7 @@
         tail = bool(defer_tail and training and n_towers == 2 and self.fused_tail and self.head in HEADS
                     and self.lib.query("vm_tail_fwd_bwd_supported", cl, self.E))
         pl["tail_pending"] = tail
+        pl["tail_ext"] = False
         pl["tail_parts"] = tail
         if fold:
             if pl.get("fold_ready", wpt) != wpt:
@@ -870,6 +873,20 @@
                     self._call("vm_fold_bn_weights", _p(self.wt[i]), T(lo["scale"]), T(lo["shift_c" if lo_c else "shift"]),
                                bias, ntw, cin, c, dt,
                                wfo[tw0].data_ptr(), wfp[tw0].data_ptr() if use_packed else None, hbo[tw0].data_ptr(), ctr, st)
+                    ext = (i == self.nb - 1 and self.fused_gmax and not with_e and bool(pl.get("tail_parts")) and dm is None
+                           and pool == 2 and L >= 2 and c % 128 == 0 and not self.sync_bn)
+                    if ext:
+                        tiles = self.lib.query("vm_conv_fwd_fold_gmax_rows", L)
+                        if "ext" not in b:
+                            b["ext"] = torch.zeros(2, pl["n"] * tiles, c, dtype=torch.int32, device=self.device)
+                        self._call("vm_conv_fwd_fold_gmax", W(lo["ep"]), wfo[tw0].data_ptr(), bias, hbo[tw0].data_ptr(), nw, wpt, L, cin, c, dt,
+                                   W(b["z"]), ssum, ssq, b["ext"][0, w0 * tiles:].data_ptr(), b["ext"][1, w0 * tiles:].data_ptr(),
+                                   wfp[tw0].data_ptr() if use_packed else None, st)
+                        b["e_now"] = b["pairs_now"] = b["ctr_now"] = False
+                        finalize()
+                        pl["tail_ext"] = True
+                        fused_tail = True
+                        continue
                     self._call("vm_conv_fwd_fold", W(lo["ep"]), wfo[tw0].data_ptr(), bias, hbo[tw0].data_ptr(), gam if with_e else None,
                                nw, wpt, L, cin, c, dt, None if pairs else W(b["z"]), ssum, ssq, W(b["ep"]) if with_e else None,
                                W(b["o"]) if pairs else None, wfp[tw0].data_ptr() if use_packed else None, ctr, st)
@@ -1130,6 +1147,14 @@
             cl, parts, seg = self.blocks[-1][1], pl["gmax_ws"], self._seg_rows
             pv = parts.data_ptr() if pl["tail_parts"] else None
             pi = parts.data_ptr() + pl["n"] * seg * cl * 4 if pl["tail_parts"] else None
+            if pl.get("tail_ext"):
+                lb, Ll = pl[self.nb - 1], pl["L"][self.nb - 1]
+                self._call("vm_tail_fwd_bwd_ext", lb["ext"][0].data_ptr(), lb["ext"][1].data_ptr(), _p(lb["scale"]), _p(lb["shift"]), Ll, self.dtype,
+                           _p(pl["gmax"]), _p(pl["gidx"]), _p(self.view("dense.kernel")), _p(self.view("dense.bias")),
+                           _p(self.view("head.kernel")), _p(self.view("head.bias")), self._dyn("y", _p(y)), pairs, cl, self.E, HEADS[self.head],
+                           LOSSES[loss], self._dyn("loss_scale", float(self.loss_scale)), _p(pl["emb"]), _p(pl["pred"]), _p(pl["demb"]), _p(pl["dgmax"]), _p(pl["head_ws"]), self.stream())
+                pl["tail_pending"], pl["tail_grads_pending"], pl["head_pending"] = False, True, False
+                return pl["pred"][:pairs]
             self._call("vm_tail_fwd_bwd", pv, pi, seg, _p(pl["gmax"]), _p(pl["gidx"]), _p(self.view("dense.kernel")), _p(self.view("dense.bias")),
                        _p(self.view("head.kernel")), _p(self.view("head.bias")), self._dyn("y", _p(y)), pairs, cl, self.E, HEADS[self.head],
                        LOSSES[loss], self._dyn("loss_scale", float(self.loss_scale)), _p(pl["emb"]), _p(pl["pred"]), _p(pl["demb"]), _p(pl["dgmax"]), _p(pl["head_ws"]), self.stream())
@@ -1213,7 +1238,7 @@
         return out
 
     def _step_flags(self):
-        return (self.fold_affine, self.fuse_block1, self.fused_bn_reduce, self.fused_sums_finalize, self.split_towers, self.tower_stagger, self.tower_swap, self.last_pairs,
+        return (self.fold_affine, self.fuse_block1, self.fused_bn_reduce, self.fused_sums_finalize, self.split_towers, self.tower_stagger, self.tower_swap, self.last_pairs, self.fused_gmax,
                 self.overlap_wgrad, self.wgrad_after_dgrad, self.defer_wgrad_tail, self.fused_pool_extreme, self.fold_pairs, self.pooled_reduce,
                 self.packed_weights, self.fused_tail, self.defer_head_reduce, self.unbiased, self.clipnorm, self.loss_scaled,
                 self.bn_zero_debias, self.bn_eps, self.bn_momentum, self.beta_1, self.beta_2, self.adam_eps, self._side_priority,
```
